# pashtari/factorizer

Measured on AMD Instinct MI355X. Metric: volumes/sec fwd+bwd, Swin Factorizer 128^3, higher is better.
Workload: dtype f32

## Files before the change

factorizer_amd/_native.py:

```python
from __future__ import annotations

import ctypes
import os
import threading

import torch

_HERE = os.path.dirname(os.path.abspath(__file__))
LIB_PATH = os.environ.get("FZ_LIB_PATH") or os.path.join(_HERE, "libfactorizer_hip.so")

FZ_OK = 0
FZ_E_UNSUPPORTED = -2
ABI_VERSION = 7
SOLVER_ID = {"mu": 0, "hals": 1, "cd": 2, "smu": 3}
STORE_F32, STORE_BF16 = 0, 1
PRODUCTS_DEFAULT, PRODUCTS_SPLIT_BF16, PRODUCTS_FP32_MFMA = 0, 1, 2
_products = threading.local()


def products() -> int:
    return getattr(_products, "value", PRODUCTS_DEFAULT)


class use_products:
# ... 56 lines not shown
    "fz_abi_version": ([], _i),
    "fz_set_tile_order": ([_i], _i),
    "fz_last_error_string": ([], _c.c_char_p),
    "fz_launch_count": ([], _i64),
    "fz_swm_fwd": ([_vp, _vp] + [_i] * 10 + [_c.POINTER(_i), _i, _i, _i, _vp], _i),
    "fz_swm_inv": ([_vp, _vp] + [_i] * 10 + [_c.POINTER(_i), _i, _vp, _i, _vp], _i),
    "fz_nmf_fwd": ([_vp] * 6 + [_i64] + [_i] * 5 + [_f, _i, _vp], _i),
    "fz_nmf_bwd": ([_vp] * 7 + [_i64] + [_i] * 6 + [_f, _i, _vp], _i),
    "fz_nmf_supported": ([_i] * 5, _i),
}


class NativeError(RuntimeError):
    pass


def declared_symbols():
    return sorted(_SIGS)


def lib():
    global _lib
    if _lib is not None:
        return _lib
    with _lock:
        if _lib is not None:
            return _lib
        if not os.path.exists(LIB_PATH):
            raise NativeError(
                f"{LIB_PATH} not found: build it with `python -m factorizer_amd.build` "
                "(hipcc --offload-arch=gfx950). Device tensors have no fallback path.")
        h = ctypes.CDLL(LIB_PATH)
        try:
            h.fz_abi_version.restype = ctypes.c_int
            abi = int(h.fz_abi_version())
        except AttributeError:
            abi = None
        if abi != ABI_VERSION:
            raise NativeError(f"{LIB_PATH} has ABI revision {abi}, this binding is written against {ABI_VERSION} "
                              "(include/factorizer_hip.h: FZ_ABI_VERSION): rebuild with `python -m factorizer_amd.build`")
        for name, (args, res) in _SIGS.items():
            fn = getattr(h, name)
            fn.argtypes = args
            fn.restype = res
        _lib = h
    return _lib


def launch_count() -> int:
    return int(lib().fz_launch_count())


def check(rc: int, what: str):
    if rc != FZ_OK:
        msg = lib().fz_last_error_string().decode()
        raise NativeError(f"{what} failed (code {rc}): {msg}")


def stream_ptr(t: torch.Tensor) -> int:
    return torch.cuda.current_stream(t.device).cuda_stream


def ptr(t):
    return None if t is None else t.data_ptr()


def shifts_array(shifts):
    flat = [int(v) for s in shifts for v in s]
    return (_i * len(flat))(*flat)


_fp = _c.POINTER(_c.c_float)


class GemmDesc(_c.Structure):
    _fields_ = [("x", _vp * 4), ("nsrc", _i), ("src_mode", _i), ("c0", _i), ("Cin", _i), ("Vin", _i64),
                ("Di", _i), ("Hi", _i), ("Wi", _i), ("w", _vp), ("w_t", _i), ("ldw", _i), ("M", _i), ("K", _i),
                ("bias", _vp), ("ln", _i), ("ln_g", _vp), ("ln_b", _vp), ("ln_eps", _f), ("stats_out", _vp),
                ("bact", _i), ("bmul", _vp), ("bmul_kind", _i), ("eact", _i), ("res", _vp), ("emul", _vp), ("emul_kind", _i), ("y", _vp),
                ("Ncol", _i64), ("Ho", _i), ("Wo", _i), ("B", _i), ("loader", _i), ("epilogue", _i), ("lnb_x", _vp), ("lnb_stats", _vp), ("lnb_g", _vp),
                ("lnb_gadd", _vp), ("lnb_part", _vp), ("act_dtype", _i), ("products", _i), ("tune", _i)]


class MlpDesc(_c.Structure):
    _fields_ = [("mode", _i), ("inp", _vp), ("w1", _vp), ("w2", _vp), ("b1", _vp), ("b2", _vp), ("ln_g", _vp),
                ("ln_b", _vp), ("ln_eps", _f), ("stats", _vp), ("z1", _vp), ("gz1", _vp), ("x1", _vp), ("out", _vp),
                ("part", _vp), ("B", _i), ("C", _i), ("H", _i), ("V", _i64), ("act_dtype", _i), ("wpart", _vp),
                ("gw1", _vp), ("gb1", _vp), ("gw2", _vp), ("gb2", _vp), ("gln", _vp), ("glp", _vp), ("products", _i),
                ("pre_in", _vp), ("pre_w", _vp), ("pre_b", _vp), ("pre_res", _vp), ("pre_out", _vp),
                ("post_w", _vp), ("post_b", _vp), ("post_out", _vp), ("post_m", _i)]


class MlpDropout(_c.Structure):
    _fields_ = [("m0", _vp), ("m1", _vp), ("m2", _vp), ("s0", _f), ("s1", _f), ("s2", _f)]


class BlockPrologue(_c.Structure):
    _fields_ = [("ln_g", _vp), ("ln_b", _vp), ("ln_eps", _f), ("w", _vp), ("t", _vp), ("stats", _vp)]


class GemmDwDesc(_c.Structure):
    _fields_ = [("g", _vp), ("q", _vp), ("w", _vp), ("ln", _i), ("stats", _vp), ("ln_g", _vp), ("ln_b", _vp), ("gadd", _vp),
                ("y", _vp), ("gln", _vp), ("wpart", _vp), ("gw", _vp), ("gb", _vp), ("B", _i), ("C", _i), ("V", _i64),
                ("act_dtype", _i), ("ldgw", _i), ("ldw", _i), ("drop_m", _vp), ("drop_s", _f)]


class WgradDesc(_c.Structure):
    _fields_ = [("p", _vp), ("M", _i), ("pmul", _vp), ("pmul_kind", _i), ("q", _vp * 4), ("nsrc", _i),
                ("src_mode", _i), ("c0", _i), ("Cin", _i), ("K", _i), ("Vq", _i64), ("D", _i), ("H", _i),
                ("W", _i), ("N", _i64), ("Ho", _i), ("Wo", _i), ("stats", _vp), ("qact", _i), ("ln_g", _vp),
                ("ln_b", _vp), ("gw", _vp), ("gbias", _vp), ("accumulate", _i), ("B", _i), ("loader", _i),
                ("act_dtype", _i), ("products", _i)]


class VolGeom(_c.Structure):
    _fields_ = [("nd", _i), ("size", _i * 3), ("start", _i * 3), ("end", _i * 3), ("pad", _i * 3), ("out", _i * 3)]


class RespaceGeom(_c.Structure):
    _fields_ = [("nd", _i), ("src_size", _i * 3), ("src_axis", _i * 3), ("flip", _i * 3), ("res_size", _i * 3), ("pad", _i * 3),
                ("out", _i * 3), ("orig_size", _i * 3), ("box_start", _i * 3), ("scale", _c.c_double * 3),
                ("inv_scale", _c.c_double * 3)]


_SIGS.update({
    "fz_gcorr_supported": ([_i] * 5, _i),
    "fz_gcorr": ([_vp] * 5 + [_i] * 11 + [_f, _vp], _i),
    "fz_gcorr_wgrad_workspace_bytes": ([_i] * 10, _i64),
    "fz_gcorr_wgrad": ([_vp] * 4 + [_i] * 11 + [_vp], _i),
    "fz_gcorr_act": ([_vp] * 5 + [_i] * 11 + [_f, _i, _vp], _i),
    "fz_gcorr_wgrad_act": ([_vp] * 4 + [_i] * 12 + [_vp], _i),
    "fz_gcorr_mu_bwd": ([_vp] * 8 + [_i] * 11 + [_f, _i, _vp], _i),
    "fz_gnmf_supported": ([_i, _i64, _i, _i, _i], _i),
    "fz_gnmf_workspace_bytes": ([_i64, _i, _i64, _i, _i, _i], _i64),
    "fz_gnmf_launches": ([_i, _i, _i], _i),
    "fz_gnmf_fwd": ([_vp] * 6 + [_i64, _i, _i64, _i, _i, _i, _f, _vp, _vp], _i),
    "fz_gnmf_bwd": ([_vp] * 7 + [_i64, _i, _i64, _i, _i, _i, _i, _f, _vp, _vp], _i),
    "fz_gnmfx_supported": ([_i, _i64, _i, _i, _i], _i),
    "fz_gnmfx_workspace_bytes": ([_i64, _i, _i64, _i, _i, _i], _i64),
    "fz_gnmfx_launches": ([_i, _i64, _i, _i, _i, _i], _i),
    "fz_gnmfx_fwd": ([_vp] * 6 + [_i64, _i, _i64, _i, _i, _i, _f, _vp, _vp], _i),
    "fz_gnmfx_bwd": ([_vp] * 7 + [_i64, _i, _i64, _i, _i, _i, _i, _f, _vp, _vp], _i),
    "fz_nmf_cf_supported": ([_i] * 11, _i),
    "fz_nmf_cf_fwd": ([_vp] * 4 + [_i] * 5 + [_c.POINTER(_i)] + [_i] * 5 + [_f, _i, _vp], _i),
    "fz_nmf_cf_bwd": ([_vp] * 5 + [_i] * 5 + [_c.POINTER(_i)] + [_i] * 7 + [_f, _i, _vp], _i),
    "fz_nmf_cf_factors_supported": ([_i] * 12 + [_c.POINTER(_i)], _i),
    "fz_nmf_cf_fwd_store_factors": ([_vp] * 5 + [_i] * 5 + [_c.POINTER(_i)] + [_i] * 3 + [_f, _i, _vp], _i),
    "fz_nmf_cf_fwd_from_factors": ([_vp] * 6 + [_i] * 5 + [_c.POINTER(_i)] * 2 + [_i] * 4 + [_f, _i, _vp], _i),
    "fz_nmf_cf_bwd_factors_supported": ([_i] * 14 + [_c.POINTER(_i)], _i),
    "fz_nmf_cf_bwd_store_factors": ([_vp] * 5 + [_i] * 5 + [_c.POINTER(_i)] + [_i] * 3 + [_f, _i, _vp], _i),
    "fz_nmf_cf_bwd_from_factors": ([_vp] * 6 + [_i] * 5 + [_c.POINTER(_i)] * 2 + [_i] * 3 + [_f, _i, _vp], _i),
    "fz_nmf_pcf_supported": ([_i] * 11, _i),
    "fz_nmf_pcf_fwd": ([_vp] * 4 + [_i] * 8 + [_c.POINTER(_i)] + [_i] * 5 + [_f, _i, _vp], _i),
    "fz_nmf_pcf_bwd": ([_vp] * 5 + [_i] * 8 + [_c.POINTER(_i)] + [_i] * 7 + [_f, _i, _vp], _i),
    "fz_nmf_pcf_bwd_prefers_separate": ([_i] * 4, _i),
    "fz_act_add": ([_vp, _vp, _i64, _i, _vp], _i),
    "fz_mlp_pre_supported": ([_i, _i, _i64, _i], _i),
    "fz_mlp_drop_supported": ([_i, _i, _i64, _i], _i),
    "fz_mlp_chain_drop": ([_c.POINTER(MlpDesc), _c.POINTER(MlpDropout), _vp], _i),
    "fz_conv3_prologue_supported": ([_i] * 4, _i),
    "fz_conv3_fwd2": ([_vp] * 4 + [_i] * 8 + [_c.POINTER(BlockPrologue), _vp], _i),
    "fz_upcat2": ([_vp, _vp, _vp, _i, _vp, _vp, _vp] + [_i] * 7 + [_c.POINTER(BlockPrologue), _vp], _i),
    "fz_gemm": ([_c.POINTER(GemmDesc), _vp], _i),
    "fz_gemm_plan": ([_c.POINTER(GemmDesc), _c.c_char_p, _i], _i),
    "fz_gemm_bx_enable": ([_i], _i),
    "fz_gemm_lnbwd_partials": ([_c.POINTER(GemmDesc)], _i64),
    "fz_reduce_rows": ([_vp, _i64, _i, _vp, _vp, _vp], _i),
    "fz_adamw_step": ([_vp, _vp, _vp, _vp, _i64, _f, _f, _f, _f, _f, _i, _f, _vp], _i),
    "fz_sw_gather": ([_vp, _vp] + [_i] * 10 + [_vp], _i),
    "fz_sw_accumulate": ([_vp] * 6 + [_f] + [_i] * 10 + [_vp], _i),
    "fz_sw_finalize": ([_vp, _vp, _i, _i64, _vp], _i),
    "fz_sw_gather2": ([_vp, _vp] + [_i] * 11 + [_vp], _i),
    "fz_sw_accumulate2": ([_vp] * 6 + [_f] + [_i] * 11 + [_vp], _i),
    "fz_sw_finalize2": ([_vp, _vp, _vp, _i, _i64, _i, _vp], _i),
    "fz_mlp_supported": ([_i, _i, _i64], _i),
    "fz_mlp_partials": ([_i, _i64], _i64),
    "fz_mlp_wgrad_rows": ([_i, _i64], _i),
    "fz_gemm_dw_rows": ([_i, _i64], _i),
    "fz_gemm_dw_workspace_bytes": ([_i, _i64], _i64),
    "fz_gemm_dw": ([_c.POINTER(GemmDwDesc), _vp], _i),
    "fz_mlp_wgrad_workspace_bytes": ([_i, _i64], _i64),
    "fz_mlp_chain": ([_c.POINTER(MlpDesc), _vp], _i),
    "fz_head_bwd_rows": ([], _i),
    "fz_head_bwd_workspace_bytes": ([], _i64),
    "fz_head_bwd": ([_vp, _vp, _vp, _vp, _vp, _i, _i, _i, _i64, _i, _vp], _i),
    "fz_head_fwd": ([_vp, _vp, _vp, _vp, _i, _i, _i, _i64, _i, _vp], _i),
    "fz_upcat_supported": ([_i] * 5, _i),
    "fz_upcat_compose": ([_vp, _vp, _i, _vp, _vp, _vp, _vp, _vp, _i, _i, _i, _vp], _i),
    "fz_upcat_wgrads": ([_vp, _vp, _vp, _i, _vp, _vp, _vp, _vp, _i, _vp, _i, _i, _i, _vp], _i),
    "fz_upcat": ([_vp, _vp, _vp, _i, _vp, _vp, _vp] + [_i] * 7 + [_vp], _i),
    "fz_upcat_bwd_supported": ([_i] * 6, _i),
    "fz_upcat_bwd_workspace_bytes": ([_i] * 4, _i64),
    "fz_upcat_bwd": ([_vp, _vp, _vp, _vp, _i, _vp, _vp, _vp, _vp, _vp, _i, _vp, _vp] + [_i] * 7 + [_vp], _i),
    "fz_wgrad": ([_c.POINTER(WgradDesc), _vp, _vp], _i),
    "fz_wgrad_group": ([_c.POINTER(_c.POINTER(WgradDesc)), _c.POINTER(_vp), _i, _vp], _i),
    "fz_wgrad_workspace_bytes": ([_c.POINTER(WgradDesc)], _i64),
    "fz_conv3_fwd": ([_vp] * 4 + [_i] * 8 + [_vp], _i),
    "fz_conv3_wgrad_chunks": ([_i] * 4, _i),
    "fz_conv3_wgrad_partials": ([_vp] * 4 + [_i] * 8 + [_vp], _i),
    "fz_chunk_reduce": ([_vp, _i, _i64, _vp, _i, _vp], _i),
    "fz_chunk_reduce_ld": ([_vp, _i, _i64, _i64, _vp, _i, _vp], _i),
    "fz_finish_defer": ([_i], _i),
    "fz_finish_pending": ([], _i),
    "fz_finish_flush": ([_vp], _i),
    "fz_finish_flush_all": ([_vp], _i),
    "fz_dice_bce_chunks": ([_i64], _i),
    "fz_dice_bce_sums": ([_vp, _vp, _vp, _i, _i64, _vp], _i),
    "fz_dice_bce_grad": ([_vp, _vp, _vp, _vp, _i, _i64, _f, _f, _vp, _vp], _i),
    "fz_dice_ce_sums": ([_vp, _vp, _vp, _i, _i, _i64, _vp], _i),
    "fz_dice_ce_grad": ([_vp, _vp, _vp, _vp, _i, _i, _i64, _f, _f, _vp, _vp], _i),
    "fz_dice_ce_finish": ([_vp, _i, _i, _i64, _f, _vp, _vp, _vp], _i),
    "fz_dice_bce_ds_sums": ([_vp, _vp, _vp, _i] + [_i] * 6 + [_i, _vp], _i),
    "fz_dice_bce_ds_grad": ([_vp, _vp, _vp, _vp, _i] + [_i] * 6 + [_i, _f, _f, _vp, _vp], _i),
    "fz_dice_ce_ds_sums": ([_vp, _vp, _vp, _i, _i] + [_i] * 6 + [_i, _vp], _i),
    "fz_dice_ce_ds_grad": ([_vp, _vp, _vp, _vp, _i, _i] + [_i] * 6 + [_i, _f, _f, _vp, _vp], _i),
    "fz_rowsum_chunks": ([_i64], _i),
    "fz_rowsum": ([_vp, _vp, _vp, _i, _i, _i64, _i, _vp], _i),
    "fz_ln_fwd": ([_vp] * 5 + [_i, _i, _i64, _f, _i, _vp], _i),
    "fz_ln_bwd": ([_vp] * 8 + [_i, _i, _i64, _i, _vp], _i),
    "fz_ln_bwd_workspace_bytes": ([_i], _i64),
    "fz_ln_bwd_workspace_bytes2": ([_i, _i, _i64], _i64),
    "fz_dropout_bits_words": ([_i, _i, _i64], _i64),
    "fz_dropout_keep_bits": ([_vp, _i, _i, _i, _i64, _f, _vp, _vp], _i),
    "fz_dropout_apply": ([_i, _vp, _f, _vp, _vp, _vp, _i, _i, _i64, _i, _vp], _i),
    "fz_seg_counts_chunks": ([_i64], _i),
    "fz_seg_counts_workspace_bytes": ([_i, _i64], _i64),
    "fz_seg_counts": ([_vp, _i, _vp, _i, _f, _vp, _vp, _vp, _i, _i64, _vp], _i),
    "fz_mask_edges": ([_vp, _vp, _vp, _i, _i, _i, _i, _i, _vp], _i),
    "fz_edge_min_dist2_splits": ([_i64, _i64], _i),
    "fz_edge_min_dist2_workspace_bytes": ([_i64, _i64], _i64),
    "fz_edge_min_dist2": ([_vp, _i64, _vp, _i64, _f, _f, _f, _vp, _vp, _vp], _i),
    "fz_aug_record_floats": ([], _i),
    "fz_aug_resample": ([_vp, _vp, _i, _i, _vp, _vp, _i, _vp, _vp, _vp] + [_i] * 6 + [_vp], _i),
    "fz_aug_smooth": ([_vp, _vp, _i, _i, _vp, _vp] + [_i] * 6 + [_vp], _i),
    "fz_aug_noise_field": ([_vp, _vp, _i, _i, _i64, _vp], _i),
    "fz_aug_source_words": ([], _i),
    "fz_aug_crop_resample": ([_vp, _vp, _i, _i, _vp, _i, _vp, _vp, _vp] + [_i] * 6 + [_vp], _i),
    "fz_vol_kind_ok": ([_i, _i], _i),
    "fz_vol_bbox": ([_vp, _i, _i, _i, _i, _i, _i, _vp, _vp], _i),
    "fz_vol_workspace_bytes": ([_i, _c.POINTER(VolGeom)], _i64),
    "fz_vol_stats": ([_vp, _i, _i, _c.POINTER(VolGeom), _i, _i, _vp, _vp], _i),
    "fz_vol_write": ([_vp, _i, _vp, _i, _i, _vp, _i, _i, _c.POINTER(_i), _c.POINTER(_i), _i, _vp, _c.POINTER(VolGeom), _i, _i,
# ... 16 lines not shown
```

factorizer_amd/csrc/gemm_dw.hip:

```cpp
#include "gemm_bx.h"
#include "gemm_shared.h"
#include "finish.h"

namespace fz {


template <typename AT>
struct DwArgsT {
  const AT* g;
  const AT* q;
  const float* w;
  int ldw;
  const float* stats;
  const float* ln_g;
  const AT* gadd;
  AT* y;
  float* wpart;
  int64_t V;
  int B;
};

template <bool LNB, typename AT, typename... DropX>
__global__ __launch_bounds__(256, 2) void gemm_dw_kernel(DwArgsT<AT> p, int ntiles, DropX... dx) {
  constexpr bool DROP = sizeof...(DropX) > 0;
  const DropArgs dr = drop_of(dx...);
  constexpr int NACC = 2;
  constexpr int kWave = 64 * kTS;
  constexpr bool BXB = sizeof(AT) == 2;
  extern __shared__ __attribute__((aligned(16))) float fz_lds_dw[];
  float* As = fz_lds_dw;
  float* tB = As + 1536;
  float* red = tB + 32;
  float* R = red + 256;
  const int lane = threadIdx.x & 63, wave = threadIdx.x >> 6;
  const int j = lane & 31, h = lane >> 5;
  const int l16 = lane & 15, k4 = lane >> 4;
  float* Gb = R + wave * kWave;
  float* Qb = Gb + 32 * kTS;
  const int tiles_per_sample = (int)((p.V + 128 * NACC - 1) / (128 * NACC));

  if constexpr (BXB) {
    if (threadIdx.x < 128) {
      const int l = threadIdx.x & 63, g = threadIdx.x >> 6;
      float a8[8];
#pragma unroll
      for (int e = 0; e < 8; ++e) a8[e] = p.w[(int64_t)(2 * (8 * g + e) + (l >> 5)) * p.ldw + (l & 31)];
      bx8 t3[3];
      bx_split<3>(a8, t3);
      bx8* dst = reinterpret_cast<bx8*>(As) + (g * 3) * 64 + l;
      dst[0] = t3[0]; dst[64] = t3[1]; dst[128] = t3[2];
    }
  } else {
  for (int idx = threadIdx.x; idx < 1024; idx += 256) {
    const int l = idx & 63, a = idx >> 6;
    As[idx] = p.w[(int64_t)(2 * a + (l >> 5)) * p.ldw + (l & 31)];
  }
  }
  if (LNB && threadIdx.x < 32) tB[threadIdx.x] = p.ln_g[threadIdx.x];

  f32x4 dW[2][2];
#pragma unroll
  for (int a = 0; a < 2; ++a)
#pragma unroll
    for (int b2 = 0; b2 < 2; ++b2)
#pragma unroll
      for (int v = 0; v < 4; ++v) dW[a][b2][v] = 0.f;
  f32x16 dWx;
#pragma unroll
  for (int r = 0; r < 16; ++r) dWx[r] = 0.f;
  float db[2] = {0.f, 0.f};
  float gln = 0.f;

  int tile = blockIdx.x;
  float bv[16][NACC];
  auto fetch_tile = [&](int t) {
    const int bt = t / tiles_per_sample;
    const int64_t ct = ((int64_t)(t % tiles_per_sample) * 4 + wave) * (32 * NACC) + NACC * j;
    const unsigned lo = (unsigned)h * (unsigned)p.V + (unsigned)(ct < p.V ? ct : 0);
    const AT* xb = p.g + (int64_t)bt * 32 * p.V;
#pragma unroll
    for (int s = 0; s < 16; ++s) vload<NACC>(xb + (int64_t)(2 * s) * p.V + lo, bv[s]);
  };
  fetch_tile(tile);
  __syncthreads();

  for (; tile < ntiles; tile += gridDim.x) {
    asm volatile("" ::: "memory");
    const int b = tile / tiles_per_sample;
    const int64_t col_off = ((int64_t)(tile % tiles_per_sample) * 4 + wave) * (32 * NACC) + NACC * j;
    const bool col_ok = col_off < p.V;
    const int64_t nc = col_ok ? col_off : 0;
    const unsigned lane_row = (unsigned)(4 * h) * (unsigned)p.V + (unsigned)nc;
    const unsigned lane_par = (unsigned)h * (unsigned)p.V + (unsigned)nc;
    const int64_t sample = (int64_t)b * 32 * p.V;
    if constexpr (DROP) {
#pragma unroll
      for (int s = 0; s < 16; ++s) {
        const uint32_t dk = drop_bits(dr, 0, b, 32, 2 * s + h, nc);
        bv[s][0] = drop_f(dr, 0, dk, 0, bv[s][0]);
        bv[s][1] = drop_f(dr, 0, dk, 1, bv[s][1]);
      }
    }

    float mu[NACC] = {0.f, 0.f}, rs[NACC] = {1.f, 1.f};
    if (LNB) {
      const float* sp = p.stats + (int64_t)b * 2 * p.V;
      vload<NACC>(sp + nc, mu);
      vload<NACC>(sp + p.V + nc, rs);
    }
#pragma unroll
    for (int hf = 0; hf < 2; ++hf) {
      float xv[8][NACC];
#pragma unroll
      for (int s8 = 0; s8 < 8; ++s8) vload<NACC>(p.q + sample + (int64_t)(2 * (hf * 8 + s8)) * p.V + lane_par, xv[s8]);
#pragma unroll
      for (int s8 = 0; s8 < 8; ++s8)
        *reinterpret_cast<float2*>(Qb + (2 * (hf * 8 + s8) + h) * kTS + 2 * j) =
            make_float2(col_ok ? (xv[s8][0] - mu[0]) * rs[0] : 0.f, col_ok ? (xv[s8][1] - mu[1]) * rs[1] : 0.f);
      __builtin_amdgcn_sched_barrier(0);
    }
#pragma unroll
    for (int s = 0; s < 16; ++s)
      *reinterpret_cast<float2*>(Gb + (2 * s + h) * kTS + 2 * j) = make_float2(col_ok ? bv[s][0] : 0.f, col_ok ? bv[s][1] : 0.f);

    f32x16 acc[NACC];
#pragma unroll
    for (int q = 0; q < NACC; ++q)
#pragma unroll
      for (int r = 0; r < 16; ++r) acc[q][r] = 0.f;
    if constexpr (BXB) {
#pragma unroll
      for (int g = 0; g < 2; ++g) {
        bx8 bop[NACC][1];
#pragma unroll
        for (int q = 0; q < NACC; ++q) {
          float x8[8];
#pragma unroll
          for (int e = 0; e < 8; ++e) x8[e] = bv[8 * g + e][q];
          bx_split<1>(x8, bop[q]);
        }
#pragma unroll
        for (int t = 2; t >= 0; --t) {
          const bx8 aw = reinterpret_cast<const bx8*>(As)[(g * 3 + t) * 64 + lane];
#pragma unroll
          for (int q = 0; q < NACC; ++q) acc[q] = __builtin_amdgcn_mfma_f32_32x32x16_bf16(aw, bop[q][0], acc[q], 0, 0, 0);
        }
      }
    } else {
#pragma unroll
    for (int s = 0; s < 16; ++s) {
      const float av = As[s * 64 + lane];
#pragma unroll
      for (int q = 0; q < NACC; ++q) acc[q] = __builtin_amdgcn_mfma_f32_32x32x2f32(av, bv[s][q], acc[q], 0, 0, 0);
    }
    }
    fetch_tile(tile + gridDim.x < ntiles ? tile + gridDim.x : tile);

    if constexpr (BXB) {
      const int rowo = (lane & 31) * kTS + 8 * (lane >> 5);
#pragma unroll
      for (int gk = 0; gk < 4; ++gk) {
        float g8[8], q8[8];
#pragma unroll
        for (int e2 = 0; e2 < 4; ++e2) {
          const float2 gv = *reinterpret_cast<const float2*>(Gb + rowo + 16 * gk + 2 * e2);
          const float2 qv = *reinterpret_cast<const float2*>(Qb + rowo + 16 * gk + 2 * e2);
          g8[2 * e2] = gv.x; g8[2 * e2 + 1] = gv.y;
          q8[2 * e2] = qv.x; q8[2 * e2 + 1] = qv.y;
        }
        bx8 ga[1];
        bx_split<1>(g8, ga);
        constexpr int NTQ = LNB ? 3 : 1;
        bx8 qb[NTQ];
        bx_split<NTQ>(q8, qb);
#pragma unroll
        for (int t = NTQ - 1; t >= 0; --t) dWx = __builtin_amdgcn_mfma_f32_32x32x16_bf16(ga[0], qb[t], dWx, 0, 0, 0);
        db[0] += ((g8[0] + g8[1]) + (g8[2] + g8[3])) + ((g8[4] + g8[5]) + (g8[6] + g8[7]));
        asm volatile("" : "+v"(db[0]));
        __builtin_amdgcn_sched_barrier(0);
      }
    } else
#pragma unroll
    for (int tc = 0; tc < 2; ++tc) {
      float a0[8], a1[8], b0[8], b1[8];
#pragma unroll
      for (int u = 0; u < 8; ++u) {
        const int t = tc * 8 + u;
        a0[u] = Gb[l16 * kTS + 4 * t + k4];
        a1[u] = Gb[(16 + l16) * kTS + 4 * t + k4];
        b0[u] = Qb[l16 * kTS + 4 * t + k4];
        b1[u] = Qb[(16 + l16) * kTS + 4 * t + k4];
      }
// ... 46 lines not shown
        }
#pragma unroll
        for (int i = 0; i < 8; ++i) {
          const int r = r8 * 8 + i;
          const int rbase = (r & 3) + 8 * (r >> 2);
          const int row = rbase + 4 * h;
          const float gc = tB[row];
          const float2 xh = *reinterpret_cast<const float2*>(Qb + row * kTS + 2 * j);
          float v[NACC];
          v[0] = rs[0] * (acc[0][r] * gc - m1[0] - xh.x * m2[0]) + ga[i][0];
          v[1] = rs[1] * (acc[1][r] * gc - m1[1] - xh.y * m2[1]) + ga[i][1];
          if (col_ok) vstore<NACC>(p.y + sample + (int64_t)rbase * p.V + lane_row, v);
          float sg = col_ok ? acc[0][r] * xh.x + acc[1][r] * xh.y : 0.f;
          float sb = col_ok ? acc[0][r] + acc[1][r] : 0.f;
          sg = half_sum32(sg);
          sb = half_sum32(sb);
          if ((lane & 31) == 31) {
            red[wave * 64 + row] = sg;
            red[wave * 64 + 32 + row] = sb;
          }
          __builtin_amdgcn_sched_barrier(0);
        }
      }
      __syncthreads();
      if (threadIdx.x < 64) {
        const int e = threadIdx.x;
        gln += (red[e] + red[64 + e]) + (red[128 + e] + red[192 + e]);
      }
      __syncthreads();
    }
  }

  float* row = p.wpart + (int64_t)blockIdx.x * kDwRow;
  __syncthreads();
  if constexpr (BXB) {
#pragma unroll
    for (int r = 0; r < 16; ++r) R[(wave * 16 + r) * 64 + lane] = dWx[r];
  } else {
#pragma unroll
  for (int a = 0; a < 2; ++a)
#pragma unroll
    for (int b2 = 0; b2 < 2; ++b2)
#pragma unroll
      for (int v = 0; v < 4; ++v) R[(wave * 16 + (a * 2 + b2) * 4 + v) * 64 + lane] = dW[a][b2][v];
  }
  __syncthreads();
  for (int e = threadIdx.x; e < 1024; e += 256) {
    const int idx = e >> 6, l = e & 63;
    const float t = (R[e] + R[1024 + e]) + (R[2048 + e] + R[3072 + e]);
    if constexpr (BXB) {
      row[((idx & 3) + 8 * (idx >> 2) + 4 * (l >> 5)) * 32 + (l & 31)] = t;
    } else {
      const int a = idx >> 3, b2 = (idx >> 2) & 1, v = idx & 3;
      row[(16 * a + 4 * (l >> 4) + v) * 32 + 16 * b2 + (l & 15)] = t;
    }
  }
  __syncthreads();
  R[(wave * 2 + 0) * 64 + lane] = db[0];
  R[(wave * 2 + 1) * 64 + lane] = db[1];
  __syncthreads();
  if (threadIdx.x < 32) {
    const int e = threadIdx.x, slot = e >> 4, i16 = e & 15;
    float t = 0.f;
    if constexpr (BXB) {
      for (int w = 0; w < 4; ++w) t += R[(w * 2) * 64 + e] + R[(w * 2) * 64 + 32 + e];
    } else {
      for (int w = 0; w < 4; ++w)
        for (int kk = 0; kk < 4; ++kk) t += R[(w * 2 + slot) * 64 + kk * 16 + i16];
    }
    row[1024 + e] = t;
  }
  if (threadIdx.x < 64) row[1024 + 32 + threadIdx.x] = gln;
}


}

using namespace fz;

static int knob_gemm_dw_wgs() { return knob_pos(FZ_KNOB("FZ_GEMM_DW_WGS"), 512); }

extern "C" int fz_gemm_dw_rows(int B, int64_t V);
template <typename AT>
static int gemm_dw_launch(const fz_gemm_dw_desc* d, fz_stream_t stream) {
  DwArgsT<AT> a;
  a.g = (const AT*)d->g; a.q = (const AT*)d->q; a.w = d->w; a.ldw = d->ldw > 0 ? d->ldw : 32; a.stats = d->stats; a.ln_g = d->ln_g; a.gadd = (const AT*)d->gadd;
  a.y = (AT*)d->y; a.wpart = (float*)d->wpart; a.V = d->V; a.B = d->B;
  const int ntiles = (int)fz_mlp_partials(d->B, d->V);
  const int rows = fz_gemm_dw_rows(d->B, d->V);
  constexpr int lds = (1536 + 32 + 256 + 4 * 64 * kTS) * (int)sizeof(float);
  hipStream_t st = (hipStream_t)stream;
  if (d->drop_m) {
    auto kern = gemm_dw_kernel<false, AT, DropArgs>;
    FZ_HIP_OK(hipFuncSetAttribute(reinterpret_cast<const void*>(kern), hipFuncAttributeMaxDynamicSharedMemorySize, lds));
    hipLaunchKernelGGL(kern, dim3((unsigned)rows), dim3(256), lds, st, a, ntiles, drop_args(d->drop_m, nullptr, nullptr, d->drop_s, 1.f, 1.f, d->V));
  } else if (d->ln) {
    auto kern = gemm_dw_kernel<true, AT>;
    FZ_HIP_OK(hipFuncSetAttribute(reinterpret_cast<const void*>(kern), hipFuncAttributeMaxDynamicSharedMemorySize, lds));
    hipLaunchKernelGGL(kern, dim3((unsigned)rows), dim3(256), lds, st, a, ntiles);
  } else {
    auto kern = gemm_dw_kernel<false, AT>;
    FZ_HIP_OK(hipFuncSetAttribute(reinterpret_cast<const void*>(kern), hipFuncAttributeMaxDynamicSharedMemorySize, lds));
    hipLaunchKernelGGL(kern, dim3((unsigned)rows), dim3(256), lds, st, a, ntiles);
  }
  FZ_LAUNCH_CHECK();
  FinishJob fj = finish_job(FK_DW, kDwRow / 16);
  fj.u.dw = FinDw{(const float*)d->wpart, d->ln ? d->ln_g : (const float*)nullptr, d->ln_b, d->gw, d->gb, d->ln ? d->gln : (float*)nullptr,
                  rows, d->ldgw > 0 ? d->ldgw : 32};
  return finish_run(&fj, 1, st);
}

extern "C" int fz_gemm_dw_rows(int B, int64_t V) {
  const int64_t nt = fz_mlp_partials(B, V);
  const int wgs = knob_gemm_dw_wgs();
  return (int)(nt < wgs ? nt : wgs);
}
extern "C" int64_t fz_gemm_dw_workspace_bytes(int B, int64_t V) {
  return (int64_t)fz_gemm_dw_rows(B, V) * kDwRow * (int64_t)sizeof(float);
}

extern "C" int fz_gemm_dw(const fz_gemm_dw_desc* d, fz_stream_t stream) {
  if (!d) return fail(FZ_E_ARG, "fz_gemm_dw: null descriptor");
  if (!d->g || !d->q || !d->w || !d->y || !d->wpart || !d->gw) return fail(FZ_E_ARG, "fz_gemm_dw: null pointer");
  if (d->ln && (!d->stats || !d->ln_g || !d->ln_b || !d->gln)) return fail(FZ_E_ARG, "fz_gemm_dw: the LayerNorm form needs stats, gamma, beta, gln");
  if (!d->ln && d->gadd) return fail(FZ_E_UNSUPPORTED, "fz_gemm_dw: gadd only with the LayerNorm backward");
  if (d->drop_m && d->ln) return fail(FZ_E_UNSUPPORTED, "fz_gemm_dw: dropout on g only without the LayerNorm backward");
  if (!drop_scale_ok(d->drop_m, d->drop_s)) return fail(FZ_E_ARG, "fz_gemm_dw: the dropout scale 1 / (1 - p) must be >= 1 and finite");
  if (d->C != 32) return fail(FZ_E_UNSUPPORTED, "fz_gemm_dw: needs C == 32");
  if (d->ldgw != 0 && d->ldgw < 32) return fail(FZ_E_ARG, "fz_gemm_dw: ldgw must be 0 (= 32) or >= 32");
  if (d->ldw != 0 && d->ldw < 32) return fail(FZ_E_ARG, "fz_gemm_dw: ldw must be 0 (= 32) or >= 32");
  if (d->B < 1 || d->V < 1 || d->V % 4 != 0 || d->V > ((int64_t)1 << 27)) return fail(FZ_E_UNSUPPORTED, "fz_gemm_dw: needs B >= 1, V % 4 == 0, V <= 2^27");
  if (d->act_dtype == FZ_STORE_F32) return gemm_dw_launch<float>(d, stream);
  if (d->act_dtype == FZ_STORE_BF16) return gemm_dw_launch<bf16>(d, stream);
  return fail(FZ_E_ARG, "fz_gemm_dw: act_dtype must be FZ_STORE_F32 or FZ_STORE_BF16");
}
```

factorizer_amd/csrc/mlp_chain.h:

```cpp
#pragma once
#include "gemm_bx.h"
#include "gemm_shared.h"

namespace fz {

template <typename AT>
struct ChainArgsT {
  const float* wB;
  int wB_t, ldwB;
  const float* biasB;
  AT* side;
  const AT* preA;
  const float* preW;
  const float* preB;
  const AT* preRes;
  AT* preOut;
  const float* postW;
  const float* postB;
  AT* postOut;
  int postM;
  int stagger;
};

__device__ __forceinline__ void chain_stagger(int stagger) {
  const int n = stagger * (int)(blockIdx.x >> 8);
  for (int i = 0; i < n; ++i) __builtin_amdgcn_s_sleep(127);
}

constexpr int chain64_lds_floats(bool p512, bool pre) {
  return 2 * (p512 ? 12288 : 8192) + (pre ? 6144 + 64 : 0) + 128 + 64 + (p512 ? 2 : 1) * 512;
}
constexpr int chain_wg_lds_floats(bool bx, bool wgb) {
  return 2 * (bx ? 3072 : 2048) + 32 + 256 + 4 * (wgb ? 3072 : 48 * kTS);
}

template <typename... KArgs, typename... Args>
static int launch_lds(void (*kern)(KArgs...), dim3 grid, dim3 block, int lds_floats, hipStream_t st, Args... args) {
  const int lds = lds_floats * (int)sizeof(float);
  FZ_HIP_OK(hipFuncSetAttribute(reinterpret_cast<const void*>(kern), hipFuncAttributeMaxDynamicSharedMemorySize, lds));
  hipLaunchKernelGGL(kern, grid, block, lds, st, args...);
  FZ_LAUNCH_CHECK();
  return FZ_OK;
}

static int knob_chain64_p512() { return knob_pos(FZ_KNOB("FZ_CHAIN64_P512"), 1) == 1; }
static int knob_chain_fwd_bx() { const auto& k = FZ_KNOB("FZ_CHAIN_FWD_BX"); return k.set ? k.val : 1; }
static int knob_mlp_wgs(int dflt) { return knob_pos(FZ_KNOB("FZ_MLP_WGS"), dflt); }

template <typename AT>
int chain32_launch(const fz_mlp_desc* d, const fz_mlp_dropout* drop, const GemmArgsT<AT>& a, const ChainArgsT<AT>& c, fz_stream_t stream);
template <typename AT>
int chain64_launch(const fz_mlp_desc* d, const GemmArgsT<AT>& a, const ChainArgsT<AT>& c, fz_stream_t stream);
template <typename AT>
int chain_wg_launch(const fz_mlp_desc* d, const GemmArgsT<AT>& a, const ChainArgsT<AT>& c, fz_stream_t stream);

}
```

factorizer_amd/csrc/mlp_chain.hip:

```cpp
#include "mlp_chain.h"

using namespace fz;

static int mlp_nacc() { return 2; }

extern "C" int64_t fz_mlp_partials(int B, int64_t V) {
  const int64_t tw = 128 * mlp_nacc();
  return ((V + tw - 1) / tw) * (int64_t)B;
}

extern "C" int fz_mlp_pre_supported(int C, int H, int64_t V, int products) {
  if (!(V > 0 && (V % 4) == 0 && V <= ((int64_t)1 << 27) && products_split(products))) return 0;
  if (C == 32 && H == 64) return knob_chain_fwd_bx() ? 1 : 0;
  if (C == 64 && H == 128) return (((V + 255) / 256) % 2 == 0 && knob_chain64_p512()) ? 1 : 0;
  return 0;
}

extern "C" int fz_mlp_supported(int C, int H, int64_t V) {
  const bool shape = (C == 32 && (H == 64 || H == 128)) || (C == 64 && H == 128);
  return (shape && V > 0 && (V % 4) == 0 && V <= ((int64_t)1 << 27)) ? 1 : 0;
}

extern "C" int fz_mlp_drop_supported(int C, int H, int64_t V, int products) {
  return (C == 32 && H == 64 && fz_mlp_supported(C, H, V) && fz_mlp_pre_supported(C, H, V, products) && products_split(products)
          && knob_chain_fwd_bx()) ? 1 : 0;
}

template <typename AT>
static void forward_args(const fz_mlp_desc* d, int ldw, int ldwB, GemmArgsT<AT>& a, ChainArgsT<AT>& c) {
  a.w = d->w1; a.w_t = 0; a.ldw = ldw;
  a.bias = d->b1; a.ln = 1; a.ln_g = d->ln_g; a.ln_b = d->ln_b; a.ln_eps = d->ln_eps; a.stats_out = d->stats;
  a.res = (const AT*)d->in; a.y = (AT*)d->out;
  c.wB = d->w2; c.wB_t = 0; c.ldwB = ldwB; c.biasB = d->b2; c.side = (AT*)d->z1;
  if (d->pre_in) {
    c.preA = (const AT*)d->pre_in; c.preW = d->pre_w; c.preB = d->pre_b; c.preRes = (const AT*)d->pre_res; c.preOut = (AT*)d->pre_out;
    if (d->C == 64) a.res = (const AT*)d->pre_out;
    else { c.postW = d->post_w; c.postB = d->post_b; c.postOut = (AT*)d->post_out; c.postM = d->post_m; }
  }
}
template <typename AT>
static void backward_args(const fz_mlp_desc* d, int ldw, int ldwB, AT* side, GemmArgsT<AT>& a, ChainArgsT<AT>& c) {
  a.w = d->w2; a.w_t = 1; a.ldw = ldw;
  a.emul = (const AT*)d->z1; a.y = (AT*)d->out;
  a.lnb_x = (const AT*)d->x1; a.lnb_stats = d->stats; a.lnb_g = d->ln_g; a.lnb_gadd = (const AT*)d->in; a.lnb_part = d->part;
  c.wB = d->w1; c.wB_t = 1; c.ldwB = ldwB; c.side = side;
}

static int mlp_check(const fz_mlp_desc* d, const fz_mlp_dropout* dd, bool drop) {
  if (!fz_mlp_supported(d->C, d->H, d->V)) return fail(FZ_E_UNSUPPORTED, "fz_mlp_chain: needs (C, H) in {(32, 64), (32, 128), (64, 128)}, V % 4 == 0");
  if (drop) {
    if (!fz_mlp_drop_supported(d->C, d->H, d->V, d->products) || d->mode != 0 || !d->pre_in)
      return fail(FZ_E_UNSUPPORTED, "fz_mlp_chain: dropout needs (C, H) = (32, 64), split-bf16 products, mode 0 with pre_in (fz_mlp_drop_supported)");
    if (!drop_scale_ok(dd->m0, dd->s0) || !drop_scale_ok(dd->m1, dd->s1) || !drop_scale_ok(dd->m2, dd->s2))
      return fail(FZ_E_ARG, "fz_mlp_chain: a dropout scale 1 / (1 - p) must be >= 1 and finite");
  }
  if (d->C == 64 && d->mode == 2) return fail(FZ_E_UNSUPPORTED, "fz_mlp_chain: the fused weight gradients need C == 32, H == 64");
  if (d->B < 0) return fail(FZ_E_SHAPE, "fz_mlp_chain: negative batch");
  const bool pre = d->pre_in != nullptr;
  if (pre && (d->mode != 0 || !d->pre_w || !d->pre_res || !d->pre_out))
    return fail(FZ_E_ARG, "fz_mlp_chain: pre_in needs mode 0, pre_w, pre_res, pre_out (see fz_mlp_pre_supported)");
  if (pre && !fz_mlp_pre_supported(d->C, d->H, d->V, d->products))
    return fail(FZ_E_UNSUPPORTED, "fz_mlp_chain: the fused out-projection runs on split-bf16 products only (fz_mlp_pre_supported)");
  if (d->post_out && (!pre || d->C != 32 || !d->post_w || d->post_m < 1 || d->post_m > 4))
    return fail(FZ_E_ARG, "fz_mlp_chain: post_out needs pre_in, C == 32, post_w and 1 <= post_m <= 4");
  if ((!d->in && !pre) || !d->w1 || !d->w2 || !d->out || !d->z1 || !d->stats)
    return fail(FZ_E_ARG, "fz_mlp_chain: null pointer");
  if (d->mode == 0 && (!d->ln_g || !d->ln_b)) return fail(FZ_E_ARG, "fz_mlp_chain: forward needs the LayerNorm affine");
  if (d->mode == 1 && (!d->gz1 || !d->x1 || !d->ln_g || !d->part)) return fail(FZ_E_ARG, "fz_mlp_chain: backward needs gz1, x1, gamma, part");
  if (d->mode == 2 && (!d->x1 || !d->ln_g || !d->ln_b || !d->gln || !d->wpart || !d->gw1 || !d->gb1 || !d->gw2 || !d->gb2))
    return fail(FZ_E_ARG, "fz_mlp_chain: backward with weight gradients needs x1, gamma, beta, gln, wpart, gw1, gb1, gw2, gb2");
  if (d->mode == 2 && d->H == 128 && !d->glp) return fail(FZ_E_ARG, "fz_mlp_chain: the fused weight gradients at H == 128 need the glp buffer");
  if (d->mode < 0 || d->mode > 2) return fail(FZ_E_ARG, "fz_mlp_chain: bad mode");
  return FZ_OK;
}

template <typename AT>
static int mlp_launch(const fz_mlp_desc* d, const fz_mlp_dropout* dd, fz_stream_t stream) {
  const bool drop = dd && (dd->m0 || dd->m1 || dd->m2);
  const int rc = mlp_check(d, dd, drop);
  if (rc != FZ_OK) return rc;
  if (d->B == 0) {
    if (d->mode == 2) {
      hipStream_t s0 = (hipStream_t)stream;
      FZ_HIP_OK(hipMemsetAsync(d->gw1, 0, sizeof(float) * d->H * 32, s0));
      FZ_HIP_OK(hipMemsetAsync(d->gw2, 0, sizeof(float) * d->H * 32, s0));
      FZ_HIP_OK(hipMemsetAsync(d->gb1, 0, sizeof(float) * d->H, s0));
      FZ_HIP_OK(hipMemsetAsync(d->gb2, 0, sizeof(float) * 32, s0));
      FZ_HIP_OK(hipMemsetAsync(d->gln, 0, sizeof(float) * 64, s0));
    }
    return FZ_OK;
  }
  GemmArgsT<AT> a = {};
  ChainArgsT<AT> c = {};
  a.x[0] = (const AT*)d->in; a.nsrc = 1; a.c0 = d->C; a.Cin = d->C; a.Vin = d->V; a.M = d->H; a.K = d->C; a.Ncol = d->V; a.B = d->B;
  if (d->mode == 0) forward_args(d, d->C, d->H, a, c);
  else backward_args(d, d->H, d->C, d->mode == 1 ? (AT*)d->gz1 : (AT*)nullptr, a, c);
  if (d->C == 64) return chain64_launch(d, a, c, stream);
  if (d->mode == 2) return chain_wg_launch(d, a, c, stream);
  return chain32_launch(d, drop ? dd : nullptr, a, c, stream);
}

extern "C" int fz_mlp_chain(const fz_mlp_desc* d, fz_stream_t stream) {
  if (!d) return fail(FZ_E_ARG, "fz_mlp_chain: null descriptor");
  if (d->act_dtype == FZ_STORE_F32) return mlp_launch<float>(d, nullptr, stream);
  if (d->act_dtype == FZ_STORE_BF16) return mlp_launch<bf16>(d, nullptr, stream);
  return fail(FZ_E_ARG, "fz_mlp_chain: act_dtype must be FZ_STORE_F32 or FZ_STORE_BF16");
}

extern "C" int fz_mlp_chain_drop(const fz_mlp_desc* d, const fz_mlp_dropout* drop, fz_stream_t stream) {
  if (!d || !drop) return fail(FZ_E_ARG, "fz_mlp_chain_drop: null descriptor");
  if (d->act_dtype == FZ_STORE_F32) return mlp_launch<float>(d, drop, stream);
  if (d->act_dtype == FZ_STORE_BF16) return mlp_launch<bf16>(d, drop, stream);
  return fail(FZ_E_ARG, "fz_mlp_chain_drop: act_dtype must be FZ_STORE_F32 or FZ_STORE_BF16");
}
```

factorizer_amd/csrc/mlp_chain32.hip:

```cpp
#include "mlp_chain.h"

namespace fz {

template <bool BWD, int NACC, int HB, typename AT = float, bool BX = false, bool PRE = false, typename... DropX>
__global__ __launch_bounds__(256, (NACC == 2 && HB == 2 && !BWD && !BX) ? 3 : 2) void gemm_chain_kernel(GemmArgsT<AT> p, ChainArgsT<AT> c, int ntiles, DropX... dx) {
  constexpr bool DROP = sizeof...(DropX) > 0;
  const DropArgs dr = drop_of(dx...);
  static_assert(!DROP || (PRE && !BWD && NACC == 2), "dropout: the forward chain with the out-projection in front");
  constexpr int NW = 4;
  constexpr int HID = 32 * HB, N1 = BX ? 1536 * HB : 16 * HB * 64;
  static_assert(!BX || (!BWD && NACC == 2), "the split-bf16 form is the forward chain");
  static_assert(!PRE || (BX && HB == 2), "the out-projection in front of the chain: split-bf16 forward, hidden 64");
  __shared__ __attribute__((aligned(16))) float As1[N1];
  __shared__ __attribute__((aligned(16))) float As2[N1];
  __shared__ __attribute__((aligned(16))) float As0[PRE ? 1536 : 4];
  __shared__ float tW[HID];
  __shared__ float tB[32];
  __shared__ float tB0[32];
  __shared__ float tP[PRE ? 4 * 32 + 4 : 1];
  __shared__ float red[256];
  __shared__ __attribute__((aligned(16))) float stash[NW][32][32 * NACC];
  const int lane = threadIdx.x & 63, wave = threadIdx.x >> 6;
  const int j = lane & 31, h = lane >> 5;
  const int tiles_per_sample = (int)((p.Ncol + 32 * NW * NACC - 1) / (32 * NW * NACC));
  chain_stagger(c.stagger);

  if constexpr (BX) {
    for (int it = threadIdx.x; it < (PRE ? 4 * HB + 2 : 4 * HB) * 64; it += 64 * NW) {
      float wv[8];
      const int l = it & 63;
      __bf16* dst;
      if (PRE && it >= 4 * HB * 64) {
        const int g = (it - 4 * HB * 64) >> 6;
#pragma unroll
        for (int e = 0; e < 8; ++e) wv[e] = c.preW[(l & 31) * 32 + 2 * (8 * g + e) + (l >> 5)];
        dst = reinterpret_cast<__bf16*>(As0) + (g * 3 * 64 + l) * 8;
      } else if (it < 2 * HB * 64) {
        const int rb = (it >> 6) % HB, g = it / (64 * HB);
#pragma unroll
        for (int e = 0; e < 8; ++e) {
          const int r = 8 * g + e;
          const int kk = PRE ? (r & 3) + 8 * (r >> 2) + 4 * (l >> 5) : 2 * r + (l >> 5);
          wv[e] = weight_at(p, rb * 32 + (l & 31), kk) * p.ln_g[kk];
        }
        dst = reinterpret_cast<__bf16*>(As1) + ((g * HB + rb) * 3 * 64 + l) * 8;
      } else {
        const int g = (it - 2 * HB * 64) >> 6;
#pragma unroll
        for (int e = 0; e < 8; ++e) {
          const int s2 = 8 * g + e, r = s2 & 15, rb = s2 >> 4;
          const int kk = rb * 32 + (r & 3) + 8 * (r >> 2) + 4 * (l >> 5), m = l & 31;
          wv[e] = c.wB_t ? c.wB[(int64_t)kk * c.ldwB + m] : c.wB[(int64_t)m * c.ldwB + kk];
        }
        dst = reinterpret_cast<__bf16*>(As2) + (g * 3 * 64 + l) * 8;
      }
      bx8 t3[3];
      bx_split<3>(wv, t3);
#pragma unroll
      for (int i = 0; i < 3; ++i) *reinterpret_cast<bx8*>(dst + i * 64 * 8) = t3[i];
    }
  } else
  for (int base = threadIdx.x; base < 2 * N1; base += 256 * 8) {
    float tmp[8];
#pragma unroll
    for (int uu = 0; uu < 8; ++uu) {
      const int idx = base + uu * 256;
      float wv;
      if (idx < N1) {
        const int l = idx & 63, rb = (idx >> 6) % HB, a = idx / (64 * HB);
        const int m = rb * 32 + (l & 31), k = 2 * a + (l >> 5);
        wv = weight_at(p, m, k);
        if (!BWD) wv *= p.ln_g[k];
      } else {
        const int i2 = idx - N1;
        const int l = i2 & 63, s2 = i2 >> 6;
        const int r = s2 & 15, rb = s2 >> 4;
        const int k = rb * 32 + (r & 3) + 8 * (r >> 2) + 4 * (l >> 5), m = l & 31;
        wv = c.wB_t ? c.wB[(int64_t)k * c.ldwB + m] : c.wB[(int64_t)m * c.ldwB + k];
      }
      tmp[uu] = wv;
    }
#pragma unroll
    for (int uu = 0; uu < 8; ++uu) {
      const int idx = base + uu * 256;
      if (idx < N1) As1[idx] = tmp[uu]; else As2[idx - N1] = tmp[uu];
    }
  }
  if (BWD) {
    if (threadIdx.x < 32) tB[threadIdx.x] = p.lnb_g[threadIdx.x];
  } else {
    for (int r = threadIdx.x; r < HID; r += blockDim.x) {
      float t = 0.f;
      for (int k = 0; k < 32; ++k) t += weight_at(p, r, k) * p.ln_b[k];
      tW[r] = t + (p.bias ? p.bias[r] : 0.f);
      if (r < 32) tB[r] = c.biasB ? c.biasB[r] : 0.f;
      if (PRE && r < 32) tB0[r] = c.preB ? c.preB[r] : 0.f;
    }
    if constexpr (PRE) {
      if (c.postOut != nullptr && threadIdx.x < 4 * 32 + 4) {
        const int i = threadIdx.x;
        if (i < 128) tP[i] = (i >> 5) < c.postM ? c.postW[i] : 0.f;
        else tP[i] = ((i - 128) < c.postM && c.postB) ? c.postB[i - 128] : 0.f;
      }
    }
  }

  int tile = blockIdx.x;
  float bv[16][NACC];
  float xr[PRE ? 16 : 1][NACC];
  auto fetch_tile = [&](int t) {
    const int bt = t / tiles_per_sample;
    const int64_t ct = ((int64_t)(t % tiles_per_sample) * NW + wave) * (32 * NACC) + NACC * j;
    const unsigned lo = (unsigned)h * (unsigned)p.Ncol + (unsigned)(ct < p.Ncol ? ct : 0);
    const AT* xb = (PRE ? c.preA : p.x[0]) + (int64_t)bt * 32 * p.Ncol;
#pragma unroll
    for (int s = 0; s < 16; ++s) vload<NACC>(xb + (int64_t)(2 * s) * p.Ncol + lo, bv[s]);
    if constexpr (PRE) {
      const unsigned lr = (unsigned)(4 * h) * (unsigned)p.Ncol + (unsigned)(ct < p.Ncol ? ct : 0);
      const AT* rb0 = c.preRes + (int64_t)bt * 32 * p.Ncol;
#pragma unroll
      for (int r = 0; r < 16; ++r) vload<NACC>(rb0 + (int64_t)((r & 3) + 8 * (r >> 2)) * p.Ncol + lr, xr[PRE ? r : 0]);
    }
  };
  fetch_tile(tile);
  __syncthreads();

  for (; tile < ntiles; tile += gridDim.x) {
    asm volatile("" ::: "memory");
    const int b = tile / tiles_per_sample;
    const int64_t col_off = ((int64_t)(tile % tiles_per_sample) * NW + wave) * (32 * NACC) + NACC * j;
    const bool col_ok = col_off < p.Ncol;
    const int64_t nc = col_ok ? col_off : 0;
    const unsigned lane_row = (unsigned)(4 * h) * (unsigned)p.Ncol + (unsigned)nc;
    if constexpr (PRE) {
      f32x16 acc0[NACC];
#pragma unroll
      for (int q = 0; q < NACC; ++q)
#pragma unroll
        for (int r = 0; r < 16; ++r) acc0[q][r] = 0.f;
#pragma unroll
      for (int g = 0; g < 2; ++g) {
        bx8 aop[3];
#pragma unroll
        for (int i = 0; i < 3; ++i)
          aop[i] = *reinterpret_cast<const bx8*>(reinterpret_cast<const __bf16*>(As0) + ((g * 3 + i) * 64 + lane) * 8);
#pragma unroll
        for (int q = 0; q < NACC; ++q) {
          float x8[8];
#pragma unroll
          for (int e = 0; e < 8; ++e) x8[e] = bv[8 * g + e][q];
          bx8 bop[3];
          bx_split<3>(x8, bop);
          bx_mfma<3, 3>(acc0[q], aop, bop);
        }
      }
#pragma unroll
      for (int r = 0; r < 16; ++r) {
        const int rbase = (r & 3) + 8 * (r >> 2);
        const int row = rbase + 4 * h;
        const float add = tB0[row];
        uint32_t dk = 0;
        if constexpr (DROP) dk = drop_bits(dr, 0, b, 32, row, nc);
#pragma unroll
        for (int q = 0; q < NACC; ++q) {
          float v;
          if constexpr (DROP) v = drop_f(dr, 0, dk, q, acc0[q][r] + add) + xr[PRE ? r : 0][q];
          else v = acc0[q][r] + add + xr[PRE ? r : 0][q];
          if constexpr (sizeof(AT) == 2) v = (float)(AT)v;
          bv[r][q] = v;
        }
        vstore<NACC>(&stash[wave][row][NACC * j], bv[r]);
        if (col_ok) vstore<NACC>(c.preOut + ((int64_t)b * 32 + rbase) * p.Ncol + lane_row, bv[r]);
      }
    } else {
#pragma unroll
    for (int s = 0; s < 16; ++s) vstore<NACC>(&stash[wave][2 * s + h][NACC * j], bv[s]);
    }

    if (!BWD) {
      float mu[NACC], rs[NACC];
#pragma unroll
      for (int e = 0; e < NACC; ++e) {
        float t = 0.f;
#pragma unroll
        for (int s = 0; s < 16; ++s) t += bv[s][e];
        t += __shfl_xor(t, 32, 64);
        mu[e] = t / 32.0f;
      }
#pragma unroll
      for (int e = 0; e < NACC; ++e) {
        float t = 0.f;
#pragma unroll
        for (int s = 0; s < 16; ++s) {
          const float d = bv[s][e] - mu[e];
          t += d * d;
        }
        t += __shfl_xor(t, 32, 64);
        rs[e] = 1.0f / sqrtf(t / 32.0f + p.ln_eps);
      }
#pragma unroll
      for (int s = 0; s < 16; ++s)
#pragma unroll
        for (int e = 0; e < NACC; ++e) bv[s][e] = (bv[s][e] - mu[e]) * rs[e];
      if (p.stats_out != nullptr && h == 0 && col_ok) {
        float* so = p.stats_out + (int64_t)b * 2 * p.Vin;
        vstore<NACC>(so + col_off, mu);
        vstore<NACC>(so + p.Vin + col_off, rs);
      }
    }

    f32x16 acc1[HB][NACC];
#pragma unroll
    for (int rb = 0; rb < HB; ++rb)
#pragma unroll
      for (int q = 0; q < NACC; ++q)
#pragma unroll
        for (int r = 0; r < 16; ++r) acc1[rb][q][r] = 0.f;
// ... 82 lines not shown
        __builtin_amdgcn_sched_barrier(0);
      }
    }

    f32x16 acc2[NACC];
#pragma unroll
    for (int q = 0; q < NACC; ++q)
#pragma unroll
      for (int r = 0; r < 16; ++r) acc2[q][r] = 0.f;
    if constexpr (BX) {
#pragma unroll
      for (int g = 0; g < 2 * HB; ++g) {
        bx8 aop[3];
#pragma unroll
        for (int i = 0; i < 3; ++i)
          aop[i] = *reinterpret_cast<const bx8*>(reinterpret_cast<const __bf16*>(As2) + ((g * 3 + i) * 64 + lane) * 8);
#pragma unroll
        for (int q = 0; q < NACC; ++q) {
          float x8[8];
#pragma unroll
          for (int e = 0; e < 8; ++e) x8[e] = acc1[g >> 1][q][8 * (g & 1) + e];
          bx8 bop[3];
          bx_split<3>(x8, bop);
          bx_mfma<3, 3>(acc2[q], aop, bop);
        }
      }
    } else {
#pragma unroll
    for (int rb = 0; rb < HB; ++rb)
#pragma unroll
      for (int r = 0; r < 16; ++r) {
        const float av = As2[(rb * 16 + r) * 64 + lane];
#pragma unroll
        for (int q = 0; q < NACC; ++q) acc2[q] = __builtin_amdgcn_mfma_f32_32x32x2f32(av, acc1[rb][q][r], acc2[q], 0, 0, 0);
      }
    }

    if (BWD) {
      lnbwd_block<NACC, true, true>(p, acc2, b, col_off, col_ok, lane, wave, red, tile, tB, &stash[wave][0][0]);
      __syncthreads();
    } else if (col_ok) {
      const bool post = PRE && c.postOut != nullptr;
      float pl[4][NACC] = {};
#pragma unroll
      for (int r = 0; r < 16; ++r) {
        const int rbase = (r & 3) + 8 * (r >> 2);
        const int row = rbase + 4 * h;
        const int64_t ob = ((int64_t)b * 32 + rbase) * p.Ncol;
        const float add = tB[row];
        float e[NACC], v[NACC];
        vload<NACC>(&stash[wave][row][NACC * j], e);
        if constexpr (DROP) {
          const uint32_t dk = drop_bits(dr, 2, b, 32, row, nc);
#pragma unroll
          for (int q = 0; q < NACC; ++q) v[q] = drop_f(dr, 2, dk, q, acc2[q][r] + add) + e[q];
        } else {
#pragma unroll
        for (int q = 0; q < NACC; ++q) v[q] = acc2[q][r] + add + e[q];
        }
        vstore<NACC>(p.y + ob + lane_row, v);
        if (PRE && post) {
#pragma unroll
          for (int q = 0; q < NACC; ++q) {
            const float vs = sizeof(AT) == 2 ? (float)(AT)v[q] : v[q];
#pragma unroll
            for (int o = 0; o < 4; ++o) pl[o][q] += tP[o * 32 + row] * vs;
          }
        }
      }
      if (PRE && post) {
#pragma unroll
        for (int o = 0; o < 4; ++o) {
          float v[NACC];
#pragma unroll
          for (int q = 0; q < NACC; ++q) v[q] = pl[o][q] + __shfl_xor(pl[o][q], 32, 64) + tP[128 + o];
          if (h == 0 && o < c.postM) vstore<NACC>(c.postOut + ((int64_t)b * c.postM + o) * p.Ncol + nc, v);
        }
      }
    }
  }
}

template <typename AT>
int chain32_launch(const fz_mlp_desc* d, const fz_mlp_dropout* drop, const GemmArgsT<AT>& a, const ChainArgsT<AT>& c, fz_stream_t stream) {
  hipStream_t st = (hipStream_t)stream;
  const int ntiles = (int)fz_mlp_partials(d->B, d->V);
  const bool bwd = d->mode != 0, pre = d->pre_in != nullptr;
  const bool bx = !bwd && d->H == 64 && products_split(d->products) && knob_chain_fwd_bx();
  const int wgs = knob_mlp_wgs(d->H == 128 || bx ? 512 : 768);
  const dim3 grid((unsigned)(ntiles < wgs ? ntiles : wgs)), block(256);
  if (bwd) {
    if (d->H == 128) hipLaunchKernelGGL((gemm_chain_kernel<true, 2, 4>), grid, block, 0, st, a, c, ntiles);
    else hipLaunchKernelGGL((gemm_chain_kernel<true, 2, 2>), grid, block, 0, st, a, c, ntiles);
  } else if (d->H == 128) hipLaunchKernelGGL((gemm_chain_kernel<false, 2, 4>), grid, block, 0, st, a, c, ntiles);
  else if (!bx) hipLaunchKernelGGL((gemm_chain_kernel<false, 2, 2>), grid, block, 0, st, a, c, ntiles);
  else if (!pre) hipLaunchKernelGGL((gemm_chain_kernel<false, 2, 2, AT, true>), grid, block, 0, st, a, c, ntiles);
  else if (!drop) hipLaunchKernelGGL((gemm_chain_kernel<false, 2, 2, AT, true, true>), grid, block, 0, st, a, c, ntiles);
  else
    hipLaunchKernelGGL((gemm_chain_kernel<false, 2, 2, AT, true, true, DropArgs>), grid, block, 0, st, a, c, ntiles,
                       drop_args(drop->m0, drop->m1, drop->m2, drop->s0, drop->s1, drop->s2, d->V));
  FZ_LAUNCH_CHECK();
  return FZ_OK;
}
template int chain32_launch<float>(const fz_mlp_desc*, const fz_mlp_dropout*, const GemmArgsT<float>&, const ChainArgsT<float>&, fz_stream_t);
template int chain32_launch<bf16>(const fz_mlp_desc*, const fz_mlp_dropout*, const GemmArgsT<bf16>&, const ChainArgsT<bf16>&, fz_stream_t);

}
```

factorizer_amd/csrc/nmf_cf.h:

```cpp
#pragma once
#include <cstdlib>

#include "fz_common.h"
#include "nmf_core.h"
#include "nmf_gram.h"

namespace fz {

struct CfGeom {
  int B, C, D, H, W;
  int h;
  int G0, G1, G2;
  int s0, s1, s2;
  int accumulate;
  int divisor;
  float gscale_div;
  int64_t plane;
  int ps0, ps1, ps2;
};

enum { CF_PLAIN = 0, CF_STORE_FACTORS = 1, CF_FROM_FACTORS = 2 };
constexpr int CFG_COFAC = 88;

struct CfWave {
  using F = float;
  int lane;
  __device__ __forceinline__ int col(int j) const {
    const int jp = j >> 2, e = j & 3;
    return (((jp * 4 + (lane >> 4)) * 8 + ((lane >> 1) & 7)) * 8) + (lane & 1) * 4 + e;
  }
  __device__ __forceinline__ float sum(float v) const { return wave_sum(v); }
  __device__ __forceinline__ void sum8(float (&v)[8]) const { wave_sum8(v, lane); }
  __device__ __forceinline__ void st_priv(float* base, int idx, float v) const { base[idx * 64 + lane] = v; }
  __device__ __forceinline__ float ld_priv(const float* base, int idx) const { return base[idx * 64 + lane]; }
  __device__ __forceinline__ void st_uni(float* base, int idx, float v) const {
    if (lane == 0) base[idx] = v;
  }
  __device__ __forceinline__ float ld_uni(const float* base, int idx) const { return base[idx]; }
  __device__ __forceinline__ float ld_uni_global(const float* p, int idx) const { return p[idx]; }
  __device__ __forceinline__ float ld_v0(const float* v0, int j, int r, int R) const { return v0[col(j) * R + r]; }
  __device__ __forceinline__ float keep_col(int, float v) const { return v; }
  __device__ __forceinline__ void fence() const { __builtin_amdgcn_fence(__ATOMIC_ACQ_REL, "wavefront"); }
  static constexpr bool kDistRows = true;
  __device__ __forceinline__ float sum8_dist(const float (&v)[8]) const { return wave_sum8_dist(v, lane); }
  __device__ __forceinline__ float grp_take(float d, int m) const {
    return __int_as_float(__builtin_amdgcn_readlane(__float_as_int(d), 8 * m));
  }
  __device__ __forceinline__ bool grp_below(int n) const { return (lane >> 3) < n; }
  __device__ __forceinline__ void st_grp(float* base, int i0, int stride, float d) const {
    if ((lane & 7) == 0) base[i0 + (lane >> 3) * stride] = d;
  }
  __device__ __forceinline__ float ld_grp_global(const float* p, int i0, int stride) const { return p[i0 + (lane >> 3) * stride]; }
  __device__ __forceinline__ float ld_grp(const float* base, int i0, int stride) const { return base[i0 + (lane >> 3) * stride]; }
  __device__ __forceinline__ float grp_sum(float d) const { return wave_group_sum(d); }
  __device__ __forceinline__ float mask_rows(float d, int mreal) const { return (lane >> 3) < mreal ? d : 0.f; }
  __device__ __forceinline__ float pick_call(int c, float tot, float mine) const { return (lane & 7) == c ? tot : mine; }
  __device__ __forceinline__ void k_unrotate(float* scratch, float mine, float (&Kd)[8]) const {
    const int g = lane >> 3;
    scratch[g * 8 + ((g + lane) & 7)] = mine;
    fence();
    const float4 a = *reinterpret_cast<const float4*>(scratch + g * 8), b = *reinterpret_cast<const float4*>(scratch + g * 8 + 4);
    Kd[0] = a.x; Kd[1] = a.y; Kd[2] = a.z; Kd[3] = a.w; Kd[4] = b.x; Kd[5] = b.y; Kd[6] = b.z; Kd[7] = b.w;
    fence();
  }
};

struct CfAddr {
  int64_t base;
  int64_t off[2];
  int64_t V;
};

__device__ __forceinline__ void cf_decode(const CfGeom& q, int64_t mat, int lane, CfAddr& a) {
  unsigned t = (unsigned)mat;
  const int g2 = (int)(t % (unsigned)q.G2); t /= (unsigned)q.G2;
  const int g1 = (int)(t % (unsigned)q.G1); t /= (unsigned)q.G1;
  const int g0 = (int)(t % (unsigned)q.G0); t /= (unsigned)q.G0;
  const int hh = (int)(t % (unsigned)q.h);
  const int b = (int)(t / (unsigned)q.h);
  const int p1 = (lane >> 1) & 7, half = lane & 1;
  int z1 = g1 * 8 + p1 - q.s1; if (z1 < 0) z1 += q.H;
  int z2 = g2 * 8 + half * 4 - q.s2; if (z2 < 0) z2 += q.W;
  a.V = q.plane;
  a.base = ((int64_t)b * q.C + (int64_t)hh * 8) * a.V;
#pragma unroll
// ... 117 lines not shown
  z0 = id.g0 * 8 + (row >> 3) - q.s0; if (z0 < 0) z0 += q.D;
  z1 = id.g1 * 8 + (row & 7) - q.s1; if (z1 < 0) z1 += q.H;
  z2 = id.gq * WPB * 8 + chunk * 4 - q.s2; if (z2 < 0) z2 += q.W;
}

template <int WPB>
__device__ __forceinline__ void cf_tile_decode(const CfGeom& q, const CfTileId& id, int tid, int64_t& base, int64_t& V,
                                               unsigned (&off)[2], int (&lidx)[2], unsigned (&off2)[2]) {
  using TL = CfTile<WPB>;
  V = q.plane;
  base = ((int64_t)id.b * q.C + (int64_t)id.hh * 8) * V;
#pragma unroll
  for (int k = 0; k < 2; ++k) {
    int row, chunk, z0, z1, z2;
    cf_chunk_voxel<WPB>(q, id, tid, k, row, chunk, z0, z1, z2);
    off[k] = (unsigned)((z0 * q.H + z1) * q.W + z2);
    int z2b = z2 + 2; if (z2b >= q.W) z2b -= q.W;
    off2[k] = (unsigned)((z0 * q.H + z1) * q.W + z2b);
    lidx[k] = TL::at(row, chunk);
  }
}

template <int WPB>
__device__ __forceinline__ unsigned cf_prev_patch(const CfGeom& q, const CfTileId& id, int tid, int k) {
  int row, chunk, z0, z1, z2;
  cf_chunk_voxel<WPB>(q, id, tid, k, row, chunk, z0, z1, z2);
  z0 += q.ps0; if (z0 >= q.D) z0 -= q.D;
  z1 += q.ps1; if (z1 >= q.H) z1 -= q.H;
  z2 += q.ps2; if (z2 >= q.W) z2 -= q.W;
  return (unsigned)(((z0 >> 3) * q.G1 + (z1 >> 3)) * q.G2 + (z2 >> 3));
}

template <typename AT>
__device__ __forceinline__ float4 cf_first_window(float u, const float4& v) {
  float p0 = u * v.x, p1 = u * v.y, p2 = u * v.z, p3 = u * v.w;
  asm("" : "+v"(p0), "+v"(p1), "+v"(p2), "+v"(p3));
  const f32v4 f = {0.0f + p0, 0.0f + p1, 0.0f + p2, 0.0f + p3};
  if constexpr (sizeof(AT) == 2) {
    const f32v4 r = __builtin_convertvector(__builtin_convertvector(f, bf16v4), f32v4);
    return make_float4(r[0], r[1], r[2], r[3]);
  }
  return make_float4(f[0], f[1], f[2], f[3]);
}

template <int WPB>
__device__ __forceinline__ int cf_owner_lidx(int lane, int wave, int jp) {
  return CfTile<WPB>::at((jp * 4 + (lane >> 4)) * 8 + ((lane >> 1) & 7), wave * 2 + (lane & 1));
}

template <int WPB>
__device__ __forceinline__ void cf_to_owner(float* S, const int (&lidx)[2], int own0, int own1, float (&x)[8][8]) {
  using TL = CfTile<WPB>;
#pragma unroll
  for (int s = 0; s < 4; ++s) {
#pragma unroll
    for (int c = 0; c < 2; ++c)
#pragma unroll
      for (int k = 0; k < 2; ++k)
        *reinterpret_cast<float4*>(S + c * 64 * TL::LW + lidx[k]) =
            make_float4(x[2 * s + c][k * 4 + 0], x[2 * s + c][k * 4 + 1], x[2 * s + c][k * 4 + 2], x[2 * s + c][k * 4 + 3]);
    __syncthreads();
#pragma unroll
    for (int c = 0; c < 2; ++c) {
      const float4 a0 = *reinterpret_cast<const float4*>(S + c * 64 * TL::LW + own0);
      const float4 a1 = *reinterpret_cast<const float4*>(S + c * 64 * TL::LW + own1);
      x[2 * s + c][0] = a0.x; x[2 * s + c][1] = a0.y; x[2 * s + c][2] = a0.z; x[2 * s + c][3] = a0.w;
      x[2 * s + c][4] = a1.x; x[2 * s + c][5] = a1.y; x[2 * s + c][6] = a1.z; x[2 * s + c][7] = a1.w;
    }
    __syncthreads();
  }
}


struct CfLaunch {
  CfGeom q;
  int64_t nmat;
  int xr;
  hipStream_t st;
};

template <typename AT>
int cf_fwd_launch(const AT* t, const float* u0, const float* v0, AT* out, float* vfac, float* ufac, const CfLaunch& a, int form,
                  int R, int T, int solver, float eps);
template <typename AT>
int cf_bwd_launch(const AT* t, const float* u0, const float* v0, const AT* ga, AT* gt, const CfLaunch& a, int relu_gate, int R,
                  int T, int G, int solver, float eps);
template <typename AT>
int cf_bwd_gram_launch(const AT* t, const float* v0, const AT* ga, AT* gt, const CfLaunch& a, int T, int G, float eps);
template <typename AT>
int cf_bwd_gram_factors_launch(const AT* t, const float* v0, const AT* ga, AT* gt, float* gcfac, float* cofac, const CfLaunch& a,
                               int form, int T, int G, float eps);

}
```

factorizer_amd/csrc/nmf_cf.hip:

```cpp
#include "nmf_cf.h"

namespace fz {

static void cf_norm_shift(const int* shift, int D, int H, int W, int (&s)[3]) {
  const int S[3] = {D, H, W};
  for (int i = 0; i < 3; ++i) { s[i] = shift[i] % S[i]; if (s[i] < 0) s[i] += S[i]; }
}

static int cf_geom(CfGeom& q, int B, int C, int D, int H, int W, const int* shift, const int* prev_shift, int accumulate,
                   int divisor) {
  if (B < 0 || C < 8 || (C % 8) || D < 8 || H < 8 || W < 8 || (D % 8) || (H % 8) || (W % 8))
    return fail(FZ_E_SHAPE, "fz_nmf_cf: needs C % 8 == 0 and spatial dims multiples of 8");
  if (!shift) return fail(FZ_E_ARG, "fz_nmf_cf: shift is null");
  if ((int64_t)D * H * W >= ((int64_t)1 << 30)) return fail(FZ_E_UNSUPPORTED, "fz_nmf_cf: 2^30 or more voxels per channel plane");
  q.B = B; q.C = C; q.D = D; q.H = H; q.W = W; q.h = C / 8; q.G0 = D / 8; q.G1 = H / 8; q.G2 = W / 8;
  int s[3], ps[3] = {0, 0, 0};
  cf_norm_shift(shift, D, H, W, s);
  if (s[2] % 2) return fail(FZ_E_UNSUPPORTED, "fz_nmf_cf: W-axis shift must be even");
  if (prev_shift) cf_norm_shift(prev_shift, D, H, W, ps);
  q.s0 = s[0]; q.s1 = s[1]; q.s2 = s[2];
  q.ps0 = ps[0]; q.ps1 = ps[1]; q.ps2 = ps[2];
  q.accumulate = accumulate; q.divisor = divisor; q.gscale_div = 1.0f;
  q.plane = (int64_t)D * H * W;
#ifdef FZ_PROBE_PLANE_PAD
// ... 41 lines not shown
    using AT = decltype(at);
    CfLaunch a;
    const int rc = cf_prepare(a, B, C, D, H, W, shift, nullptr, accumulate, divisor, stream, [&](const CfGeom&) {
      if (!t || !u0 || !v0 || !out) return fail(FZ_E_ARG, "fz_nmf_cf_fwd: null pointer");
      if (R < 1 || R > 2) return fail(FZ_E_UNSUPPORTED, "fz_nmf_cf_fwd: rank 1..2");
      if (solver < FZ_SOLVER_MU || solver > FZ_SOLVER_SMU) return fail(FZ_E_ARG, "fz_nmf_cf_fwd: bad solver");
      return (int)FZ_OK;
    });
    if (rc != FZ_OK || a.nmat == 0) return rc;
    return cf_fwd_launch<AT>((const AT*)t, u0, v0, (AT*)out, nullptr, nullptr, a, CF_PLAIN, R, T, solver, eps);
  });
}

extern "C" int fz_nmf_cf_bwd(const void* t, const float* u0, const float* v0, const void* ga, void* gt, int B,
                             int C, int D, int H, int W, const int* shift, int accumulate, int nshift,
                             int relu_gate, int R, int T, int Tgrad, int solver, float eps, int act_dtype,
                             fz_stream_t stream) {
  return cf_with_dtype(act_dtype, "fz_nmf_cf_bwd: bad act_dtype", [&](auto at) {
    using AT = decltype(at);
    CfLaunch a;
    const int rc = cf_prepare(a, B, C, D, H, W, shift, nullptr, accumulate, 1, stream, [&](const CfGeom&) {
      if (!t || !u0 || !v0 || !ga || !gt) return fail(FZ_E_ARG, "fz_nmf_cf_bwd: null pointer");
      if (R < 1 || R > 2) return fail(FZ_E_UNSUPPORTED, "fz_nmf_cf_bwd: rank 1..2");
      if (solver < FZ_SOLVER_MU || solver > FZ_SOLVER_SMU) return fail(FZ_E_ARG, "fz_nmf_cf_bwd: bad solver");
      return (int)FZ_OK;
    });
    if (rc != FZ_OK || a.nmat == 0) return rc;
    a.q.gscale_div = (float)(nshift > 1 ? nshift : 1);
    const int G = Tgrad < 0 ? 0 : (Tgrad > T ? T : Tgrad);
    return cf_bwd_launch<AT>((const AT*)t, u0, v0, (const AT*)ga, (AT*)gt, a, relu_gate, R, T, G, solver, eps);
  });
}

extern "C" int fz_nmf_cf_factors_supported(int C, int D, int H, int W, int d, int pd, int ph, int pw, int R, int T, int Tgrad,
                                           int nshift, const int* shifts) {
  if (!fz_nmf_cf_supported(C, D, H, W, d, pd, ph, pw, R, T, Tgrad)) return 0;
  if (R != 1 || nshift != 2 || !shifts || (W % 64)) return 0;
  for (int w = 0; w < 2; ++w) {
    int s[3];
    cf_norm_shift(shifts + 3 * w, D, H, W, s);
    if (s[2] % 4) return 0;
  }
  return 1;
}

static int cf_fwd_factors(const void* t, const float* u0, const float* v0, void* out, float* vfac, float* ufac, int B, int C,
                          int D, int H, int W, const int* shift, const int* prev_shift, int form, int divisor, int R, int T,
                          int solver, float eps, int act_dtype, fz_stream_t stream, const char* null_msg, const char* dtype_msg) {
  return cf_with_dtype(act_dtype, dtype_msg, [&](auto at) {
    using AT = decltype(at);
    CfLaunch a;
    const int rc = cf_prepare(a, B, C, D, H, W, shift, prev_shift, form == CF_FROM_FACTORS, divisor, stream, [&](const CfGeom& q) {
      if (!t || !u0 || !v0 || !vfac || !ufac || (form == CF_FROM_FACTORS && (!out || !prev_shift))) return fail(FZ_E_ARG, null_msg);
      if (R != 1) return fail(FZ_E_UNSUPPORTED, "fz_nmf_cf_fwd factor forms: rank 1 only");
      if (W % 64) return fail(FZ_E_UNSUPPORTED, "fz_nmf_cf_fwd factor forms: W must be a multiple of 64");
      if (solver < FZ_SOLVER_MU || solver > FZ_SOLVER_SMU) return fail(FZ_E_ARG, "fz_nmf_cf_fwd factor forms: bad solver");
      if (divisor < 1) return fail(FZ_E_ARG, "fz_nmf_cf_fwd factor forms: divisor < 1");
      if ((q.s2 % 4) || (q.ps2 % 4)) return fail(FZ_E_UNSUPPORTED, "fz_nmf_cf_fwd factor forms: W-axis shift must be a multiple of 4");
      return (int)FZ_OK;
    });
    if (rc != FZ_OK || a.nmat == 0) return rc;
    return cf_fwd_launch<AT>((const AT*)t, u0, v0, (AT*)out, vfac, ufac, a, form, R, T, solver, eps);
  });
}

extern "C" int fz_nmf_cf_fwd_store_factors(const void* t, const float* u0, const float* v0, float* vfac, float* ufac, int B,
                                           int C, int D, int H, int W, const int* shift, int R, int T, int solver, float eps,
                                           int act_dtype, fz_stream_t stream) {
  return cf_fwd_factors(t, u0, v0, nullptr, vfac, ufac, B, C, D, H, W, shift, nullptr, CF_STORE_FACTORS, 1, R, T, solver, eps,
                        act_dtype, stream, "fz_nmf_cf_fwd_store_factors: null pointer (t, u0, v0, vfac or ufac)",
                        "fz_nmf_cf_fwd_store_factors: bad act_dtype");
}

extern "C" int fz_nmf_cf_fwd_from_factors(const void* t, const float* u0, const float* v0, const float* vfac,
                                          const float* ufac, void* out, int B, int C, int D, int H, int W, const int* shift,
                                          const int* prev_shift, int divisor, int R, int T, int solver, float eps, int act_dtype,
                                          fz_stream_t stream) {
  return cf_fwd_factors(t, u0, v0, out, const_cast<float*>(vfac), const_cast<float*>(ufac), B, C, D, H, W, shift, prev_shift,
                        CF_FROM_FACTORS, divisor, R, T, solver, eps, act_dtype, stream,
                        "fz_nmf_cf_fwd_from_factors: null pointer (t, u0, v0, vfac, ufac, out or prev_shift)",
                        "fz_nmf_cf_fwd_from_factors: bad act_dtype");
}

extern "C" int fz_nmf_cf_bwd_factors_supported(int C, int D, int H, int W, int d, int pd, int ph, int pw, int R, int T, int Tgrad,
                                               int solver, int relu_gate, int nshift, const int* shifts) {
  if (FZ_KNOB("FZ_CF_BWD_FACTORS").set && FZ_KNOB("FZ_CF_BWD_FACTORS").val == 0) return 0;
  if (!fz_nmf_cf_factors_supported(C, D, H, W, d, pd, ph, pw, R, T, Tgrad, nshift, shifts)) return 0;
  if (solver != FZ_SOLVER_HALS || !relu_gate) return 0;
  if (T < 1 || Tgrad < T) return 0;
  if ((C / 8) * (int64_t)(D / 8) * (H / 8) * (W / 8) >= ((int64_t)1 << 31)) return 0;
  const int lds = (CfTile<4>::STAGE_FLOATS + 4 * gram_hist_floats(T - 1) + 4 * 8 * CFG_COFAC) * (int)sizeof(float);
  return lds <= 64 * 1024 ? 1 : 0;
}

static int cf_bwd_factors(const void* t, const float* v0, const void* ga, void* gt, float* gcfac, float* cofac, int B, int C,
                          int D, int H, int W, const int* shift, const int* prev_shift, int form, int nshift, int T, int Tgrad,
                          float eps, int act_dtype, fz_stream_t stream, const char* null_msg, const char* dtype_msg) {
  return cf_with_dtype(act_dtype, dtype_msg, [&](auto at) {
    using AT = decltype(at);
    CfLaunch a;
    int rc = cf_prepare(a, B, C, D, H, W, shift, prev_shift, form == CF_FROM_FACTORS, 1, stream, [&](const CfGeom& q) {
      if (!t || !v0 || !ga || !gcfac || !cofac || (form == CF_FROM_FACTORS && (!gt || !prev_shift))) return fail(FZ_E_ARG, null_msg);
      if (W % 64) return fail(FZ_E_UNSUPPORTED, "fz_nmf_cf_bwd factor forms: W must be a multiple of 64");
      if (nshift != 2) return fail(FZ_E_UNSUPPORTED, "fz_nmf_cf_bwd factor forms: exactly two windows");
      if (T < 1 || Tgrad < T) return fail(FZ_E_UNSUPPORTED, "fz_nmf_cf_bwd factor forms: every iteration graded (1 <= T <= Tgrad)");
      if ((q.s2 % 4) || (q.ps2 % 4)) return fail(FZ_E_UNSUPPORTED, "fz_nmf_cf_bwd factor forms: W-axis shift must be a multiple of 4");
      return (int)FZ_OK;
    });
    if (rc != FZ_OK || a.nmat == 0) return rc;
    a.q.gscale_div = (float)nshift;
    rc = cf_bwd_gram_factors_launch<AT>((const AT*)t, v0, (const AT*)ga, (AT*)gt, gcfac, cofac, a, form, T, T, eps);
    if (rc == FZ_E_UNSUPPORTED) return fail(rc, "fz_nmf_cf_bwd factor forms: history exceeds the LDS budget");
    return rc;
  });
}

extern "C" int fz_nmf_cf_bwd_store_factors(const void* t, const float* v0, const void* ga, float* gcfac, float* cofac, int B,
                                           int C, int D, int H, int W, const int* shift, int nshift, int T, int Tgrad,
                                           float eps, int act_dtype, fz_stream_t stream) {
  return cf_bwd_factors(t, v0, ga, nullptr, gcfac, cofac, B, C, D, H, W, shift, nullptr, CF_STORE_FACTORS, nshift, T, Tgrad, eps,
                        act_dtype, stream, "fz_nmf_cf_bwd_store_factors: null pointer (t, v0, ga, gcfac or cofac)",
                        "fz_nmf_cf_bwd_store_factors: bad act_dtype");
}

extern "C" int fz_nmf_cf_bwd_from_factors(const void* t, const float* v0, const void* ga, const float* gcfac,
                                          const float* cofac, void* gt, int B, int C, int D, int H, int W, const int* shift,
                                          const int* prev_shift, int nshift, int T, int Tgrad, float eps, int act_dtype,
                                          fz_stream_t stream) {
  return cf_bwd_factors(t, v0, ga, gt, const_cast<float*>(gcfac), const_cast<float*>(cofac), B, C, D, H, W, shift, prev_shift,
                        CF_FROM_FACTORS, nshift, T, Tgrad, eps, act_dtype, stream,
                        "fz_nmf_cf_bwd_from_factors: null pointer (t, v0, ga, gcfac, cofac, gt or prev_shift)",
                        "fz_nmf_cf_bwd_from_factors: bad act_dtype");
}
```

factorizer_amd/csrc/nmf_cf_fwd.hip:

```cpp
#include "nmf_cf.h"

namespace fz {

template <int R, int SOLVER, typename AT>
__global__ __launch_bounds__(1024) void nmf_cf_fwd_kernel(const AT* __restrict__ t, const float* __restrict__ u0,
                                                          const float* __restrict__ v0, AT* __restrict__ out,
                                                          CfGeom q, int64_t nmat, int T, float eps, int xcd_remap) {
  const int lane = threadIdx.x & 63;
  const int64_t mat = cf_logical_block(xcd_remap) * (blockDim.x >> 6) + (threadIdx.x >> 6);
  if (mat >= nmat) return;
  CfWave w{lane};
  CfAddr a;
  cf_decode(q, mat, lane, a);
  float x[8][8], u[8][R], v[8][R];
  cf_load(t, a, x);
  nmf_forward_wave<8, 8, R, SOLVER>(w, u0, v0, x, u, v, 8, T, eps);
  const float dv = (float)q.divisor;
  const bool dv_pow2 = cf_pow2(dv);
#pragma unroll
  for (int dd = 0; dd < 8; ++dd)
#pragma unroll
    for (int jp = 0; jp < 2; ++jp) {
      AT* p = out + a.base + dd * a.V + a.off[jp];
      float4 o;
// ... 74 lines not shown
#pragma unroll
    for (int dd = 0; dd < 8; ++dd)
#pragma unroll
      for (int k = 0; k < 2; ++k) old[dd][k] = cf_ld4<HALF>(out + base + dd * V, off[k], off2[k]);
  }
#pragma unroll
  for (int s = 0; s < 4; ++s) {
#pragma unroll
    for (int c = 0; c < 2; ++c) {
      *reinterpret_cast<float4*>(S + c * 64 * TL::LW + own0) =
          make_float4(x[2 * s + c][0], x[2 * s + c][1], x[2 * s + c][2], x[2 * s + c][3]);
      *reinterpret_cast<float4*>(S + c * 64 * TL::LW + own1) =
          make_float4(x[2 * s + c][4], x[2 * s + c][5], x[2 * s + c][6], x[2 * s + c][7]);
    }
    __syncthreads();
#pragma unroll
    for (int c = 0; c < 2; ++c)
#pragma unroll
      for (int k = 0; k < 2; ++k) {
        const float4 z = *reinterpret_cast<const float4*>(S + c * 64 * TL::LW + lidx[k]);
        float4 o;
        if constexpr (FORM == CF_FROM_FACTORS) {
          o = cf_first_window<AT>(pu[k][2 * s + c], pv[k]);
          o.x += z.x; o.y += z.y; o.z += z.z; o.w += z.w;
        } else if (q.accumulate) {
          o = old[2 * s + c][k];
          o.x += z.x; o.y += z.y; o.z += z.z; o.w += z.w;
        } else {
          o = make_float4(0.0f + z.x, 0.0f + z.y, 0.0f + z.z, 0.0f + z.w);
        }
        if (q.divisor > 1) o = cf_divide4(o, dv, dv_pow2);
        cf_st4<HALF>(out + base + (2 * s + c) * V, off[k], off2[k], o);
      }
    __syncthreads();
  }
}

template <int R, int SOLVER, int WPB, bool HALF, typename AT, int FORM>
__global__ __launch_bounds__(WPB * 64, (WPB == 8 || R >= 2) ? 2 : 4) void nmf_cf_fwd_tile_kernel(const AT* __restrict__ t,
                                                                   const float* __restrict__ u0,
                                                                   const float* __restrict__ v0,
                                                                   AT* __restrict__ out, float* vfac, float* ufac,
                                                                   CfGeom q, int T, float eps, int xcd_remap) {
  extern __shared__ __attribute__((aligned(16))) float fz_lds_tile[];
  cf_fwd_tile_body<R, SOLVER, WPB, HALF, AT, FORM>(t, u0, v0, out, vfac, ufac, q, cf_tile_id<WPB>(q, cf_logical_block(xcd_remap)), T, eps,
                                                   fz_lds_tile);
}

template <typename AT>
int cf_fwd_launch(const AT* t, const float* u0, const float* v0, AT* out, float* vfac, float* ufac, const CfLaunch& a, int form,
                  int R, int T, int solver, float eps) {
  const CfGeom& q = a.q;
  const int tile = FZ_KNOB("FZ_CF_TILE").set ? FZ_KNOB("FZ_CF_TILE").val : 1;
  const bool half = (q.s2 % 4) != 0;
  const int twpb = (q.G2 % 8) == 0 ? 8 : ((q.G2 % 4) == 0 ? 4 : 1);
#define FZ_CF_TILE(RR, WW, HH, FF, SS)                                                                                  \
  hipLaunchKernelGGL((nmf_cf_fwd_tile_kernel<RR, SS, WW, HH, AT, FF>), dim3((unsigned)(a.nmat / WW)), dim3(64 * WW),    \
                     CfTile<WW>::STAGE_FLOATS * (int)sizeof(float), a.st, t, u0, v0, out, vfac, ufac, q, T, eps, a.xr)
#define FZ_CF_TILE_W(RR, SS)                                                                                            \
  do {                                                                                                                  \
    if (half) { if (twpb == 8) FZ_CF_TILE(RR, 8, true, CF_PLAIN, SS); else if (twpb == 4) FZ_CF_TILE(RR, 4, true, CF_PLAIN, SS); else FZ_CF_TILE(RR, 1, true, CF_PLAIN, SS); } \
    else FZ_CF_TILE(RR, 8, false, CF_PLAIN, SS);                                                                        \
  } while (0)
  if (form == CF_STORE_FACTORS) {
    FZ_SOLVER_CASES(FZ_CF_TILE, 1, 8, false, CF_STORE_FACTORS);
  } else if (form == CF_FROM_FACTORS) {
    FZ_SOLVER_CASES(FZ_CF_TILE, 1, 8, false, CF_FROM_FACTORS);
  } else if (half || (tile && (q.G2 % 8) == 0)) {
    if (R == 1) { FZ_SOLVER_CASES(FZ_CF_TILE_W, 1); }
    else { FZ_SOLVER_CASES(FZ_CF_TILE_W, 2); }
  } else {
    const int wpb = q.G2 < 16 ? q.G2 : 16;
    dim3 grid((unsigned)((a.nmat + wpb - 1) / wpb)), block(64 * wpb);
#define FZ_CF_FWD(RR, SS) hipLaunchKernelGGL((nmf_cf_fwd_kernel<RR, SS, AT>), grid, block, 0, a.st, t, u0, v0, out, q, a.nmat, T, eps, a.xr)
    if (R == 1) { FZ_SOLVER_CASES(FZ_CF_FWD, 1); }
    else { FZ_SOLVER_CASES(FZ_CF_FWD, 2); }
  }
  FZ_LAUNCH_CHECK();
  return FZ_OK;
}
template int cf_fwd_launch<float>(const float*, const float*, const float*, float*, float*, float*, const CfLaunch&, int, int, int, int, float);
template int cf_fwd_launch<bf16>(const bf16*, const float*, const float*, bf16*, float*, float*, const CfLaunch&, int, int, int, int, float);

}
```

factorizer_amd/functional.py:

```python
from __future__ import annotations

import ctypes
import math
import os

import torch

from . import _native as N


def _dev_guard(t: torch.Tensor):
    return torch.cuda.device(t.device)


class KernelTimer:

    def __init__(self, only=None):
        self.records = []
        self.only = None if only is None else set(only)

    def launch(self, name, nbytes, fn, cols=0, flops=0):
        if self.only is not None and name not in self.only:
            return fn()
        s = torch.cuda.Event(enable_timing=True)
# ... 279 lines not shown
    return gx


class GNMFFn(torch.autograd.Function):

    @staticmethod
    def forward(ctx, x, u0, v0, T, G, solver, eps, fam):
        x, u0, v0 = x.contiguous(), u0.contiguous(), v0.contiguous()
        y, _, _ = _gnmf_fwd_raw(x, u0, v0, T, solver, eps, fam=fam)
        ctx.save_for_backward(x, u0, v0)
        ctx.cfg = (T, G, solver, eps, fam)
        return y

    @staticmethod
    def backward(ctx, gy):
        x, u0, v0 = ctx.saved_tensors
        T, G, solver, eps, fam = ctx.cfg
        if G <= 0:
            return (torch.zeros_like(x), *[None] * 7)
        return (_gnmf_bwd_raw(x, u0, v0, gy.contiguous(), None, None, T, G, solver, eps, fam), *[None] * 7)


class GNMFDecomposeFn(torch.autograd.Function):
    @staticmethod
    def forward(ctx, x, u0, v0, T, G, solver, eps, fam):
        x, u0, v0 = x.contiguous(), u0.contiguous(), v0.contiguous()
        _, u, v = _gnmf_fwd_raw(x, u0, v0, T, solver, eps, want_uv=True, fam=fam)
        ctx.save_for_backward(x, u0, v0)
        ctx.cfg = (T, G, solver, eps, fam)
        return u, v

    @staticmethod
    def backward(ctx, gu, gv):
        x, u0, v0 = ctx.saved_tensors
        T, G, solver, eps, fam = ctx.cfg
        if G <= 0:
            return (torch.zeros_like(x), *[None] * 7)
        gx = _gnmf_bwd_raw(x, u0, v0, None, gu.contiguous(), gv.contiguous(), T, G, solver, eps, fam)
        return (gx, *[None] * 7)


def gnmf(x, u0, v0, T, G, solver, eps=1e-16):
    return GNMFFn.apply(x, u0, v0, T, G, solver, eps, "gnmf")


def gnmf_decompose(x, u0, v0, T, G, solver, eps=1e-16):
    return GNMFDecomposeFn.apply(x, u0, v0, T, G, solver, eps, "gnmf")


def gnmfx(x, u0, v0, T, G, solver, eps=1e-16):
    return GNMFFn.apply(x, u0, v0, T, G, solver, eps, "gnmfx")


def gnmfx_decompose(x, u0, v0, T, G, solver, eps=1e-16):
    return GNMFDecomposeFn.apply(x, u0, v0, T, G, solver, eps, "gnmfx")


def nmf_cf_supported(geo: Geometry, R, T, G) -> bool:
    if len(geo.spatial) != 3 or any(s[2] % 2 for s in geo.shifts):
        return False
    return bool(N.lib().fz_nmf_cf_supported(geo.C, *geo.spatial, geo.d, *geo.patch, int(R), int(T), int(G)))


def nmf_cf_factors_supported(geo: Geometry, R, T, G) -> bool:
    if len(geo.spatial) != 3:
        return False
    k = (int(R), int(T), int(G))
    ok = geo._factors_ok.get(k)
    if ok is None:
        ok = geo._factors_ok[k] = bool(N.lib().fz_nmf_cf_factors_supported(geo.C, *geo.spatial, geo.d, *geo.patch, *k,
                                                                          geo.nshift, geo._carr))
    return ok


def nmf_cf_bwd_factors_supported(geo: Geometry, R, T, G, solver, relu_gate) -> bool:
    if len(geo.spatial) != 3:
        return False
    k = ("bwd", int(R), int(T), int(G), solver, bool(relu_gate))
    ok = geo._factors_ok.get(k)
    if ok is None:
        ok = geo._factors_ok[k] = bool(N.lib().fz_nmf_cf_bwd_factors_supported(
            geo.C, *geo.spatial, geo.d, *geo.patch, *k[1:4], N.SOLVER_ID[solver], int(k[5]), geo.nshift, geo._carr))
    return ok


def nmf_pcf_supported(geo: Geometry, R, T, G) -> bool:
    if os.environ.get("FZ_NMF_PCF", "1") == "0":
        return False
    return bool(N.lib().fz_nmf_pcf_supported(geo.C, *geo.s3, geo.d, *geo.p3, int(R), int(T), int(G)))


def nmf_core_supported(geo: Geometry, R, T, G) -> bool:
    return nmf_cf_supported(geo, R, T, G) or nmf_pcf_supported(geo, R, T, G)


def _core_launches(t, geo: Geometry, ad):
    lib, cols, tail = N.lib(), t.numel() // geo.C, (ad, N.stream_ptr(t))

    def launch(name, key, nbytes, *args):
        fn = getattr(lib, name)
        N.check(_timed(key, nbytes, cols=cols, fn=lambda: fn(*args, *tail)), name)

    return launch, f"{geo.C}x" + "x".join(str(v) for v in geo.spatial), [(N._i * 3)(*s) for s in geo.shifts3]


class FactCoreFn(torch.autograd.Function):

    @staticmethod
    def forward(ctx, t, u0, v0, geo, T, G, solver, eps, relu_gate):
        t = t.contiguous()
        u0, v0 = u0.contiguous(), v0.contiguous()
        B = t.shape[0]
        out = torch.empty_like(t)
        R = u0.shape[1]
        nt = t.element_size() * t.numel()
        hot = nmf_cf_supported(geo, R, T, G)
        launch, sp, shifts = _core_launches(t, geo, N.act_dtype(t))
        key = ("nmf_cf_fwd_" if hot else "nmf_pcf_fwd_") + sp
        lead = (t.data_ptr(), u0.data_ptr(), v0.data_ptr())
        dims = (B, geo.C, *geo.spatial) if hot else (B, geo.C, *geo.s3, *geo.p3)
        cfg = (R, T, N.SOLVER_ID[solver], eps)
        with _dev_guard(t):
            if hot and nmf_cf_factors_supported(geo, R, T, G):
                vfac = torch.empty((B, geo.h, *geo.spatial), device=t.device, dtype=torch.float32)
                ufac = torch.empty((B * geo.h * geo.G, 8), device=t.device, dtype=torch.float32)
                fac = (vfac.data_ptr(), ufac.data_ptr())
                nf = 4 * (t.numel() // 8)
                N.set_tile_order(0)
                launch("fz_nmf_cf_fwd_store_factors", key, nt + nf, *lead, *fac, *dims, shifts[0], *cfg)
                N.set_tile_order(1)
                launch("fz_nmf_cf_fwd_from_factors", key, 2 * nt + nf, *lead, *fac, out.data_ptr(), *dims, shifts[1], shifts[0], 2,
                       *cfg)
            else:
                name = "fz_nmf_cf_fwd" if hot else "fz_nmf_pcf_fwd"
                for w, arr in enumerate(shifts):
                    N.set_tile_order(w & 1)
                    launch(name, key, (3 if w else 2) * nt, *lead, out.data_ptr(), *dims, arr, int(w > 0),
                           geo.nshift if w == geo.nshift - 1 else 1, *cfg)
            N.set_tile_order(0)
        ctx.save_for_backward(t, u0, v0)
        ctx.cfg = (geo, T, G, solver, eps, relu_gate)
        return out

    @staticmethod
    def backward(ctx, ga):
        t, u0, v0 = ctx.saved_tensors
        geo, T, G, solver, eps, relu_gate = ctx.cfg
        if G <= 0:
            return (torch.zeros_like(t),) + (None,) * 8
        ga = ga.contiguous()
        if ga.dtype != t.dtype:
            ga = ga.to(t.dtype)
        gt = torch.empty_like(t)
        B = t.shape[0]
        R = u0.shape[1]
        nt = t.element_size() * t.numel()
        ad = N.act_dtype(t)
        hot = nmf_cf_supported(geo, R, T, G)
        launch, sp, shifts = _core_launches(t, geo, ad)
        key = ("nmf_cf_bwd_" if hot else "nmf_pcf_bwd_") + sp
        dims = (B, geo.C, *geo.spatial) if hot else (B, geo.C, *geo.s3, *geo.p3)
        with _dev_guard(t):
            if hot and nmf_cf_bwd_factors_supported(geo, R, T, G, solver, relu_gate):
                gcfac = torch.empty((B, geo.h, *geo.spatial), device=t.device, dtype=torch.float32)
                cofac = torch.empty((B * geo.h * geo.G, 88), device=t.device, dtype=torch.float32)
                lead = (t.data_ptr(), v0.data_ptr(), ga.data_ptr(), gcfac.data_ptr(), cofac.data_ptr())
# ... 487 lines not shown
```

factorizer_amd/pointwise.py:

```python
from __future__ import annotations

import collections
import ctypes
import functools
import os
import threading as _threading
import weakref

import torch
import torch.nn.functional as F

from . import _native as N
from . import gradbuf as _GB
from . import functional as Fn

ACT = {"none": 0, "relu": 1, "gelu": 2}
LOAD_PLAIN, LOAD_S2D, LOAD_K3, LOAD_S2D_2D, LOAD_K3_2D = 0, 1, 2, 3, 4
EPI_PLAIN, EPI_D2S, EPI_LNBWD, EPI_D2S_2D = 0, 1, 2, 3
QL_S2D_2D, QL_K3_2D = LOAD_S2D_2D, LOAD_K3_2D
_D2S_FINE = {EPI_D2S: 8, EPI_D2S_2D: 4}


_p = N.ptr

# ... 64 lines not shown
    d.act_dtype = N.act_dtype(p)
    nb = N.lib().fz_wgrad_workspace_bytes(ctypes.byref(d))
    if nb < 0:
        raise N.NativeError("fz_wgrad_workspace_bytes failed")
    ws = torch.empty(max(nb // 4, 1), dtype=torch.float32, device=p.device)
    nbytes = p.element_size() * (p.numel() + sum(t.numel() for t in qs))
    return d, ws, f"{name}_{M}x{K}", nbytes, B * max(Vq, Ncols), 2 * B * Ncols * M * K


def _wgrad(p, qs, gw, **kw):
    d, ws, key, nbytes, cols, flops = _wgrad_desc(p, qs, gw, **kw)
    with torch.cuda.device(p.device), _finish_scope(ws, gw, kw.get("gbias")):
        rc = Fn._timed(key, nbytes, lambda: N.lib().fz_wgrad(ctypes.byref(d), ws.data_ptr(), N.stream_ptr(p)),
                       cols=cols, flops=flops)
    N.check(rc, "fz_wgrad")
    return gw


_WGRAD_GROUP = os.environ.get("FZ_WGRAD_GROUP", "1") != "0"


def _wgrad_group(problems, name):
    plans = [_wgrad_desc(p, qs, gw, **kw) for p, qs, gw, kw in problems]
    n = len(plans)
    descs = (ctypes.POINTER(N.WgradDesc) * n)(*[ctypes.pointer(pl[0]) for pl in plans])
    wss = (ctypes.c_void_p * n)(*[pl[1].data_ptr() for pl in plans])
    t0 = problems[0][0]
    held = [pl[1] for pl in plans] + [pr[2] for pr in problems] + [pr[3].get("gbias") for pr in problems]
    with torch.cuda.device(t0.device), _finish_scope(*held):
        rc = Fn._timed(name, sum(pl[3] for pl in plans),
                       lambda: N.lib().fz_wgrad_group(descs, wss, n, N.stream_ptr(t0)),
                       cols=max(pl[4] for pl in plans), flops=sum(pl[5] for pl in plans))
    N.check(rc, "fz_wgrad_group")


def _ln_backward(gl, x, stats, ln_w, gadd=None):
    B, C = x.shape[:2]
    V = _vox(x)
    gx = torch.empty_like(x)
    gpar = torch.empty(2 * C, dtype=torch.float32, device=x.device)
    ws = torch.empty(max(N.lib().fz_ln_bwd_workspace_bytes2(B, C, V) // 4, 1), dtype=torch.float32, device=x.device)
    with torch.cuda.device(x.device), _finish_scope(ws, gpar):
        rc = Fn._timed(f"ln_bwd_{C}", 3 * x.element_size() * x.numel(), lambda: N.lib().fz_ln_bwd(
            gl.data_ptr(), x.data_ptr(), stats.data_ptr(), ln_w.data_ptr(), _p(gadd), gx.data_ptr(), _p(gpar), _p(ws),
            B, C, V, N.act_dtype(x), N.stream_ptr(x)), cols=B * V)
    N.check(rc, "fz_ln_bwd")
    return gx, gpar[:C], gpar[C:]


def _reduce_affine_rows(part, rows, C, like):
    gpar = torch.empty(2 * C, dtype=torch.float32, device=like.device)
    tmp = torch.empty((64, 2 * C), dtype=torch.float32, device=like.device)
    with _finish_scope(part, gpar, tmp):
        rc = N.lib().fz_reduce_rows(part.data_ptr(), rows, 2 * C, gpar.data_ptr(), tmp.data_ptr(), N.stream_ptr(like))
    N.check(rc, "fz_reduce_rows")
    return gpar[:C], gpar[C:]


def _dgrad_lnbwd(gz, w2, x, stats, ln_w, gadd):
    B, C = x.shape[:2]
    V = _vox(x)
    Mz = gz.shape[1]
    fused64 = C == 64 and Mz == 64 and gadd is not None and V % 4 == 0 and os.environ.get("FZ_LNBWD64", "1") != "0"
    if not fused64 and (C != 32 or Mz > 64 or Mz % 2):
        gl = torch.empty_like(x)
        _gemm([gz], w2, gl, B=B, Cin=Mz, Vin=V, M=C, K=Mz, Ncol=V, w_t=True, ldw=C, name="linear_dgrad")
        return _ln_backward(gl, x, stats, ln_w, gadd=gadd)
    gx = torch.empty_like(x)
    d, *timed = _gemm_desc([gz], w2, gx, B=B, Cin=Mz, Vin=V, M=C, K=Mz, Ncol=V, w_t=True, ldw=C, epilogue=EPI_LNBWD,
                           lnb=(x, stats, ln_w, gadd), name="dgrad_lnbwd")
    rows = N.lib().fz_gemm_lnbwd_partials(ctypes.byref(d))
    part = torch.empty((rows, 2 * C), dtype=torch.float32, device=x.device)
    d.lnb_part = part.data_ptr()
    with torch.cuda.device(x.device):
        _gemm_launch(gz, d, *timed)
        ggamma, gbeta = _reduce_affine_rows(part, rows, C, x)
    return gx, ggamma, gbeta


def _dw_fused_ok(C, V):
    return C == 32 and V % 4 == 0 and V <= (1 << 27) and os.environ.get("FZ_DW_FUSED", "1") != "0"


def _gemm_dw(g, w2, q, ln=None, stats=None, gadd=None, want_bias=False, name="dgrad_wgrad", gw_out=None, gb_out=None, drop=None):
    B, C = q.shape[:2]
    V = _vox(q)
    dev = q.device
    y = torch.empty_like(q)
    gw = _GB.out_like(w2, (C, C), torch.float32) if gw_out is None else gw_out
    gb = (gb_out if gb_out is not None else torch.empty(C, dtype=torch.float32, device=dev)) if want_bias else None
    wpart = torch.empty(N.lib().fz_gemm_dw_workspace_bytes(B, V) // 4, dtype=torch.float32, device=dev)
    d = N.GemmDwDesc()
    d.g, d.q, d.w, d.y = g.data_ptr(), q.data_ptr(), w2.data_ptr(), y.data_ptr()
    d.wpart, d.gw, d.gb = wpart.data_ptr(), gw.data_ptr(), _p(gb)
    d.B, d.C, d.V, d.act_dtype = B, C, V, N.act_dtype(q)
    d.ldgw = gw.stride(0)
    d.ldw = w2.stride(0)
    if drop is not None:
        d.drop_m, d.drop_s = drop[0].data_ptr(), _drop_scale(drop[1])
    gpar = None
    if ln is not None:
        gpar = torch.empty(64, dtype=torch.float32, device=dev)
        d.ln, d.stats, d.ln_g, d.ln_b, d.gadd, d.gln = 1, stats.data_ptr(), ln[0].data_ptr(), ln[1].data_ptr(), _p(gadd), gpar.data_ptr()
    nbytes = q.element_size() * (3 * q.numel() + (gadd.numel() if gadd is not None else 0))
    with torch.cuda.device(dev), _finish_scope(wpart, gw, gb, gpar):
        rc = Fn._timed(f"{name}_{C}", nbytes, lambda: N.lib().fz_gemm_dw(ctypes.byref(d), N.stream_ptr(q)),
                       cols=B * V, flops=4 * B * V * C * C)
        N.check(rc, "fz_gemm_dw")
    if ln is not None:
        return y, gw, gb, gpar[:32], gpar[32:]
    return y, gw, gb, None, None


def _drop_scale(p):
    return 1.0 / (1.0 - float(ctypes.c_float(p).value))


def _mlp_dropout(drop):
    bits, ps = drop
    dd = N.MlpDropout()
    for s in range(3):
        if bits[s] is not None:
            setattr(dd, f"m{s}", bits[s].data_ptr())
            setattr(dd, f"s{s}", _drop_scale(ps[s]))
    return dd


def _mlp_drop_ok(C, Hd, V):
    return (_outproj_mlp_ok(C, Hd, V)
            and bool(N.lib().fz_mlp_drop_supported(C, Hd, V, N.products())))


def _mlp_chain_ok(C, Hd, V):
    return os.environ.get("FZ_MLP_CHAIN", "1") != "0" and bool(N.lib().fz_mlp_supported(C, Hd, V))


def _mlp_desc(mode, like, w12, w22, *, B, C, Hd, V, inp=None, b1=None, b2=None, ln_w=None, ln_b=None, eps=0.0, stats=None, z1=None,
              x1=None, out=None):
    d = N.MlpDesc()
    d.products = N.products()
    d.mode, d.inp, d.w1, d.w2, d.b1, d.b2 = mode, _p(inp), w12.data_ptr(), w22.data_ptr(), _p(b1), _p(b2)
    d.ln_g, d.ln_b, d.ln_eps = _p(ln_w), _p(ln_b), float(eps)
    d.stats, d.z1, d.x1, d.out = _p(stats), _p(z1), _p(x1), _p(out)
    d.B, d.C, d.H, d.V = B, C, Hd, V
    d.act_dtype = N.act_dtype(like)
    return d


def _mlp_chain_fwd(timed, like, ln_w, ln_b, eps, w12, b1, w22, b2, inp=None, pre=None, head=None, drop=None):
    B, C = like.shape[:2]
    V = _vox(like)
    Hd = w12.shape[0]
    new = lambda ch: torch.empty((B, ch, *like.shape[2:]), dtype=like.dtype, device=like.device)
    z1, st, x2 = new(Hd), _ln_stats(B, V, like.device), torch.empty_like(like)
    d = _mlp_desc(0, like, w12, w22, B=B, C=C, Hd=Hd, V=V, inp=inp, b1=b1, b2=b2, ln_w=ln_w, ln_b=ln_b, eps=eps, stats=st, z1=z1, out=x2)
    x1 = logits = None
    if pre is not None:
        a, wout2, bout, x = pre
        x1 = torch.empty_like(like)
        d.pre_in, d.pre_w, d.pre_b, d.pre_res, d.pre_out = a.data_ptr(), wout2.data_ptr(), _p(bout), x.data_ptr(), x1.data_ptr()
    if head is not None:
        hw, hb = head
        logits = new(hw.shape[0])
        d.post_w, d.post_b, d.post_out, d.post_m = hw.data_ptr(), _p(hb), logits.data_ptr(), hw.shape[0]
    dd = _mlp_dropout(drop) if drop is not None else None
    key, nbytes, flops = timed
    with torch.cuda.device(like.device):
        rc = Fn._timed(key, nbytes,
                       lambda: (N.lib().fz_mlp_chain(ctypes.byref(d), N.stream_ptr(like)) if dd is None
                                else N.lib().fz_mlp_chain_drop(ctypes.byref(d), ctypes.byref(dd), N.stream_ptr(like))),
                       cols=B * V, flops=flops)
    N.check(rc, "fz_mlp_chain")
    return x1, x2, z1, st, logits


def _mlp_fwd_chain(x1, ln_w, ln_b, eps, w12, b1, w22, b2):
    B, C = x1.shape[:2]
    V = _vox(x1)
    Hd = w12.shape[0]
    timed = (f"mlp_chain_fwd_{C}", x1.element_size() * (2 * x1.numel() + B * Hd * V), 4 * B * V * C * Hd)
    _, x2, z1, st, _ = _mlp_chain_fwd(timed, x1, ln_w, ln_b, eps, w12, b1, w22, b2, inp=x1)
    return x2, z1, st


_OUTPROJ_MLP = os.environ.get("FZ_OUTPROJ_MLP", "1") != "0"


def _outproj_mlp_ok(C, Hd, V):
    return _OUTPROJ_MLP and _mlp_chain_ok(C, Hd, V) and bool(N.lib().fz_mlp_pre_supported(C, Hd, V, N.products()))


def _outproj_mlp_fwd_chain(a, wout2, bout, x, ln_w, ln_b, eps, w12, b1, w22, b2, head=None, drop=None):
    B, C = a.shape[:2]
    V = _vox(a)
    Hd = w12.shape[0]
    nlogits = B * head[0].shape[0] * V if head is not None else 0
    timed = (f"outproj_mlp_chain_fwd_{C}", a.element_size() * (4 * a.numel() + B * Hd * V + nlogits), 4 * B * V * C * Hd + 2 * B * V * C * C)
    x1, x2, z1, st, logits = _mlp_chain_fwd(timed, a, ln_w, ln_b, eps, w12, b1, w22, b2, pre=(a, wout2, bout, x), head=head, drop=drop)
    if head is not None:
        return x1, x2, z1, st, logits
    return x1, x2, z1, st


def _mlp_bwd_chain(g2, z1, w12, w22, x1, st, ln_w):
    B, C = x1.shape[:2]
    V = _vox(x1)
    Hd = w12.shape[0]
    gz1 = torch.empty_like(z1)
    gx1 = torch.empty_like(x1)
    rows = N.lib().fz_mlp_partials(B, V)
    part = torch.empty((rows, 2 * C), dtype=torch.float32, device=x1.device)
    d = _mlp_desc(1, x1, w12, w22, B=B, C=C, Hd=Hd, V=V, inp=g2, ln_w=ln_w, stats=st, z1=z1, x1=x1, out=gx1)
    d.gz1, d.part = gz1.data_ptr(), part.data_ptr()
    with torch.cuda.device(x1.device):
        rc = Fn._timed(f"mlp_chain_bwd_{C}", x1.element_size() * (3 * x1.numel() + 2 * z1.numel()),
                       lambda: N.lib().fz_mlp_chain(ctypes.byref(d), N.stream_ptr(x1)), cols=B * V, flops=4 * B * V * C * Hd)
        N.check(rc, "fz_mlp_chain")
        ggamma, gbeta = _reduce_affine_rows(part, rows, C, x1)
    return gz1, gx1, ggamma, gbeta


def _mlp_wgrad_fused_ok(C, Hd, V):
    return _mlp_chain_ok(C, Hd, V) and C == 32 and Hd in (64, 128) and os.environ.get("FZ_MLP_FUSED_WGRAD", "1") != "0"


def _mlp_bwd_chain_wgrad(g2, z1, w12, w22, x1, st, ln_w, ln_b):
    B, C = x1.shape[:2]
    V = _vox(x1)
    Hd = w12.shape[0]
    dev = x1.device
    gx1 = torch.empty_like(x1)
    gpar = torch.empty(64, dtype=torch.float32, device=dev)
    wpart = torch.empty(N.lib().fz_mlp_wgrad_workspace_bytes(B, V) // 4, dtype=torch.float32, device=dev)
    gw1 = _GB.out_like(w12, (Hd, C), torch.float32)
    gw2 = _GB.out_like(w22, (C, Hd), torch.float32)
    gb1 = torch.empty(Hd, dtype=torch.float32, device=dev)
    gb2 = torch.empty(C, dtype=torch.float32, device=dev)
    glp = torch.empty(x1.shape, dtype=torch.float32, device=dev) if Hd == 128 else None
    d = _mlp_desc(2, x1, w12, w22, B=B, C=C, Hd=Hd, V=V, inp=g2, ln_w=ln_w, ln_b=ln_b, stats=st, z1=z1, x1=x1, out=gx1)
    d.gln, d.wpart, d.glp = gpar.data_ptr(), wpart.data_ptr(), _p(glp)
    d.gw1, d.gb1, d.gw2, d.gb2 = gw1.data_ptr(), gb1.data_ptr(), gw2.data_ptr(), gb2.data_ptr()
    nbytes = x1.element_size() * (3 * x1.numel() + z1.numel()) + (0 if Hd == 64 else x1.element_size() * 2 * x1.numel() + 8 * x1.numel())
    with torch.cuda.device(dev), _finish_scope(wpart, gpar, gw1, gb1, gw2, gb2):
        rc = Fn._timed(f"mlp_chain_bwd_wgrad_{C}" + ("" if Hd == 64 else f"x{Hd}"), nbytes,
                       lambda: N.lib().fz_mlp_chain(ctypes.byref(d), N.stream_ptr(x1)), cols=B * V, flops=8 * B * V * C * Hd)
        N.check(rc, "fz_mlp_chain")
    return gx1, gpar[:32], gpar[32:], gw1, gb1, gw2, gb2


_SIDE = {}


def _side_stream(dev, ncols):
    lim = int(os.environ.get("FZ_SIDE_WGRAD", "0"))
    if lim <= 0 or ncols > lim:
        return None
    key = (dev.type, dev.index)
    if key not in _SIDE:
        _SIDE[key] = torch.cuda.Stream(device=dev)
    return _SIDE[key]


class _LateJoin:
    enabled = False
    keep = []
    owed = []
    devices = set()
    queued = False
    verified = 0


def _end_of_backward():
    _LateJoin.queued = False
    join_wgrad_streams()


def reset_late_join():
    d = _LateJoin
    if d.devices:
        wait_wgrad_streams()
    d.owed.clear()
# ... 852 lines not shown
        tls.cur = self
        return self

    def __exit__(self, *exc):
        BlockPrologue._tls.cur = self.prev

    @staticmethod
    def take(x):
        cur = getattr(BlockPrologue._tls, "cur", None)
        if cur is not None and cur.x is x:
            return cur.t, cur.st
        return None


def cat_linear(x1, x2, w, b=None):
    if _native_ok(x1, x2, w, b) and x1.shape[1] % 2 == 0 and x2.shape[1] % 2 == 0:
        return CatLinearFn.apply(x1, x2, w, b)
    _warn_composed("cat+Linear", x1, x2, w, b)
    return linear_cf(torch.cat([x1, x2], dim=1), w, b)


def _block_dropout_bits(x, C, Hd, drop):
    B, V = x.shape[0], _vox(x)
    seed = Fn.dropout_seed(x.device)
    return tuple(None if p == 0 else Fn.dropout_keep_bits(seed, s, B, ch, V, p) for s, (ch, p) in enumerate(zip((C, Hd, C), drop)))


def _block_tail_fwd(a, wout2, bout, x, ln_w, ln_b, eps, w12, b1, w22, b2, drop=None, bits=(None, None, None)):
    B, C = x.shape[:2]
    V = _vox(x)
    Hd = w12.shape[0]
    new = lambda ch: torch.empty((B, ch, *x.shape[2:]), dtype=x.dtype, device=x.device)
    (p0, p1, p2), (m0, m1, m2) = drop or (0, 0, 0), bits
    if m0 is not None:
        o = new(C)
        _gemm([a], wout2, o, B=B, Cin=C, Vin=V, M=C, K=C, Ncol=V, bias=bout, name="linear")
        x1 = Fn.dropout_apply(N.DROP_RES, m0, p0, o, x)
        del o
    else:
        x1 = new(C)
        _gemm([a], wout2, x1, B=B, Cin=C, Vin=V, M=C, K=C, Ncol=V, bias=bout, res=x, name="act_linear_res")
    z1 = new(Hd)
    st2 = _ln_stats(B, V, x.device)
    _gemm([x1], w12, z1, B=B, Cin=C, Vin=V, M=Hd, K=C, Ncol=V, bias=b1, ln=(ln_w, ln_b, eps), stats_out=st2, name="ln_linear")
    h, bact = (Fn.dropout_apply(N.DROP_GELU, m1, p1, z1), ACT["none"]) if m1 is not None else (z1, ACT["gelu"])
    if m2 is not None:
        o = new(C)
        _gemm([h], w22, o, B=B, Cin=Hd, Vin=V, M=C, K=Hd, Ncol=V, bias=b2, bact=bact, name="linear")
        x2 = Fn.dropout_apply(N.DROP_RES, m2, p2, o, x1)
        del o
    else:
        x2 = new(C)
        _gemm([h], w22, x2, B=B, Cin=Hd, Vin=V, M=C, K=Hd, Ncol=V, bias=b2, bact=bact, res=x1, name="act_linear_res")
    return x1, x2, z1, st2


class FactorizerBlockFn(torch.autograd.Function):

    _fz_acts = (0, 4, 5, 14, 15, 16, 17, 18)

    @staticmethod
    @_fwd
    def forward(ctx, x, n1w, n1b, win, u0, v0, wout, bout, n2w, n2b, w1, b1, w2, b2, cfg, head_w=None, head_b=None,
                t_pre=None, st_pre=None):
        x = x.contiguous()
        B, C = x.shape[:2]
        V = _vox(x)
        sp = x.shape[2:]
        geo, T, G, solver, neps = cfg["geo"], cfg["T"], cfg["G"], cfg["solver"], cfg["nmf_eps"]
        win2, wout2 = win.reshape(C, C), wout.reshape(C, C)
        Hd = w1.shape[0]
        w12, w22 = w1.reshape(Hd, C), w2.reshape(C, Hd)
        u0c, v0c = u0.contiguous(), v0.contiguous()
        new = lambda ch: torch.empty((B, ch, *sp), dtype=x.dtype, device=x.device)
        drop = cfg.get("drop")
        bits = _block_dropout_bits(x, C, Hd, drop) if drop is not None else (None, None, None)
        if t_pre is not None:
            t, st1 = t_pre, st_pre
        else:
            t = new(C)
            st1 = _ln_stats(B, V, x.device)
            _gemm([x], win2, t, B=B, Cin=C, Vin=V, M=C, K=C, Ncol=V, ln=(n1w, n1b, cfg["eps1"]), stats_out=st1,
                  eact=ACT["relu"], name="ln_linear")
        m = None
        if cfg["core"]:
            a = Fn.FactCoreFn.forward(_Ctx(), t, u0c, v0c, geo, T, G, solver, neps, True)
        else:
            m = Fn._swm_fwd_raw(t, geo)
            ym, _, _ = Fn._nmf_fwd_raw(m, u0c, v0c, T, solver, neps)
            a = Fn._swm_inv_raw(ym, geo, average=True)
            del ym
        logits = None
        tail = (a, wout2, bout, x, n2w, n2b, cfg["eps2"], w12, b1, w22, b2)
        if (_mlp_drop_ok if drop is not None else _outproj_mlp_ok)(C, Hd, V) and a.is_contiguous():
            head = (head_w.reshape(head_w.shape[0], C), head_b) if head_w is not None and drop is None else None
            x1, x2, z1, st2, *logits = _outproj_mlp_fwd_chain(*tail, head=head, drop=(bits, drop) if drop is not None else None)
            logits = logits[0] if logits else None
        elif drop is None and _mlp_chain_ok(C, Hd, V):
            x1 = new(C)
            _gemm([a], wout2, x1, B=B, Cin=C, Vin=V, M=C, K=C, Ncol=V, bias=bout, res=x, name="act_linear_res")
            x2, z1, st2 = _mlp_fwd_chain(x1, n2w, n2b, cfg["eps2"], w12, b1, w22, b2)
        else:
            x1, x2, z1, st2 = _block_tail_fwd(*tail, drop, bits)
        ctx.save_for_backward(x, st1, t, a, x1, st2, z1, m, n1w, n1b, win2, u0c, v0c, wout2, n2w, n2b, w12, w22, *bits)
        ctx.cfg = cfg
        ctx.shapes = (win.shape, wout.shape, w1.shape, w2.shape)
        ctx.prm = tuple(weakref.ref(t) for t in (win, wout, bout, w1, b1, w2, b2))
        if head_w is not None:
            if logits is None:
                raise RuntimeError("FactorizerBlockFn: head fusion asked for a configuration outside fz_mlp_pre_supported "
                                   "(callers check block_head_fusable first)")
            ctx.mark_non_differentiable(logits)
            ctx.set_materialize_grads(False)
            return x2, logits
        return x2

    @staticmethod
    @_bwd
    def backward(ctx, g2, _g_logits=None):
        x, st1, t, a, x1, st2, z1, m, n1w, n1b, win2, u0c, v0c, wout2, n2w, n2b, w12, w22, *bits = ctx.saved_tensors
        cfg = ctx.cfg
        drop = cfg.get("drop")
        if g2 is None:
            g2 = torch.zeros_like(x)
        g2 = g2.contiguous()
        B, C = x.shape[:2]
        V = _vox(x)
        Hd = w12.shape[0]
        dev, dt = x.device, x.dtype
        geo, T, G, solver, neps = cfg["geo"], cfg["T"], cfg["G"], cfg["solver"], cfg["nmf_eps"]
        cur = torch.cuda.current_stream(dev)
        side = _side_stream(dev, B * V)
        keep = []

        pending = []

        def wgrad(*args, **kw):
            if _WGRAD_GROUP:
                kw.pop("name", None)
                pending.append((args[0], args[1], args[2], kw))
                return args[2]
            if side is None:
                return _wgrad(*args, **kw)
            side.wait_stream(cur)
            keep.extend(t for t in (args[0], *args[1], kw.get("stats")) if t is not None)
            with torch.cuda.stream(side):
                return _wgrad(*args, **kw)

        chain = _mlp_chain_ok(C, Hd, V) and drop is None
        (p0, p1, p2), (m0, m1, m2) = drop or (0, 0, 0), bits
        if drop is None and _mlp_wgrad_fused_ok(C, Hd, V):
            gx1, gg2, gbt2, gw1, gb1, gw2, gb2 = _mlp_bwd_chain_wgrad(g2, z1, w12, w22, x1, st2, n2w, n2b)
        else:
            gelu = ACT["gelu" if m1 is None else "none"]
            gf = Fn.dropout_apply(N.DROP_RES, m2, p2, g2) if m2 is not None else g2
            gw2 = _GB.out_like(w22)
            gb2 = torch.empty(C, dtype=torch.float32, device=dev)
            if chain:
                gz1, gx1, gg2, gbt2 = _mlp_bwd_chain(g2, z1, w12, w22, x1, st2, n2w)
            else:
                gz1 = torch.empty_like(z1)
                _gemm([gf], w22, gz1, B=B, Cin=C, Vin=V, M=Hd, K=C, Ncol=V, w_t=True, ldw=Hd, emul=(z1 if m1 is None else None),
                      emul_kind=gelu, name="linear_dgrad")
                if m1 is not None:
                    gz1 = Fn.dropout_apply(N.DROP_GELU_BWD, m1, p1, gz1, z1)
            h = Fn.dropout_apply(N.DROP_GELU, m1, p1, z1) if m1 is not None else z1
            wgrad(gf, [h], gw2, B=B, M=C, Cin=Hd, K=Hd, Vq=V, Ncols=V, gbias=gb2, qact=gelu, name="wgrad_linear")
            del h, gf
            if not chain:
                gx1, gg2, gbt2 = _dgrad_lnbwd(gz1, w12, x1, st2, n2w, g2)
            gw1 = _GB.out_like(w12)
            gb1 = torch.empty(Hd, dtype=torch.float32, device=dev)
            wgrad(gz1, [x1], gw1, B=B, M=Hd, Cin=C, K=C, Vq=V, Ncols=V, gbias=gb1, stats=st2, ln=(n2w, n2b),
                  name="wgrad_ln_linear")
            del gz1
        go, go_drop = gx1, None
        if m0 is not None:
            if _dw_fused_ok(C, V):
                go_drop = (m0, p0)
            else:
                go = Fn.dropout_apply(N.DROP_RES, m0, p0, gx1)
        dw = _dw_fused_ok(C, V)
        if dw:
            ga, gwo, gbo, _, _ = _gemm_dw(go, wout2, a, want_bias=True, name="dgrad_wgrad", drop=go_drop)
        else:
            ga = torch.empty_like(a)
            _gemm([go], wout2, ga, B=B, Cin=C, Vin=V, M=C, K=C, Ncol=V, w_t=True, ldw=C, name="linear_dgrad")
            gwo = _GB.out_like(wout2)
            gbo = torch.empty(C, dtype=torch.float32, device=dev)
            wgrad(go, [a], gwo, B=B, M=C, Cin=C, K=C, Vq=V, Ncols=V, gbias=gbo, name="wgrad_linear")
        del go
        if G <= 0:
            gt = torch.zeros_like(t)
        elif cfg["core"]:
            c2 = _Ctx()
            c2.saved_tensors = (t, u0c, v0c)
            c2.cfg = (geo, T, G, solver, neps, True)
            gt = Fn.FactCoreFn.backward(c2, ga)[0]
        else:
            gym = Fn._swm_fwd_raw(ga, geo, div=geo.nshift)
            gm = Fn._nmf_bwd_raw(m, u0c, v0c, gym, None, None, T, G, solver, neps)
            del gym
            gt = Fn._swm_inv_raw(gm, geo, average=False, gate=m)
            del gm
        del ga
        if dw:
            gx, gwi, _, gg1, gbt1 = _gemm_dw(gt, win2, x, ln=(n1w, n1b), stats=st1, gadd=gx1, name="dgrad_lnbwd_wgrad")
        else:
            gx, gg1, gbt1 = _dgrad_lnbwd(gt, win2, x, st1, n1w, gx1)
            gwi = _GB.out_like(win2)
            wgrad(gt, [x], gwi, B=B, M=C, Cin=C, K=C, Vq=V, Ncols=V, stats=st1, ln=(n1w, n1b), name="wgrad_ln_linear")
        if pending:
            if side is None:
                _wgrad_group(pending, f"wgrad_block_{C}x{Hd}")
            else:
                side.wait_stream(cur)
                for pr in pending:
                    keep.extend(t for t in (pr[0], *pr[1], pr[3].get("stats"), pr[3].get("pmul")) if t is not None)
                with torch.cuda.stream(side):
                    _wgrad_group(pending, f"wgrad_block_{C}x{Hd}")
            pending.clear()
        if side is not None:
            if _LateJoin.enabled:
                _LateJoin.keep.extend(keep)
                _LateJoin.devices.add((dev.type, dev.index))
                _LateJoin.owed.extend(zip(ctx.prm, (t.data_ptr() for t in (gwi, gwo, gbo, gw1, gb1, gw2, gb2))))
                if not _LateJoin.queued:
                    _LateJoin.queued = True
                    torch.autograd.Variable._execution_engine.queue_callback(_end_of_backward)
            else:
                cur.wait_stream(side)
            keep.clear()
        s_in, s_out, s_1, s_2 = ctx.shapes
        return (gx, gg1, gbt1, gwi.reshape(s_in), None, None, gwo.reshape(s_out), gbo, gg2, gbt2,
                gw1.reshape(s_1), gb1, gw2.reshape(s_2), gb2, None, None, None, None, None)[:len(ctx.needs_input_grad)]


_head_fusion = _threading.local()


class HeadFusion:

    def __init__(self, block, head_params):
        self.block, self.head_params, self.logits = block, head_params, None

    def __enter__(self):
        self.prev = getattr(_head_fusion, "slot", None)
        _head_fusion.slot = self
        return self

    def __exit__(self, *exc):
        _head_fusion.slot = self.prev


def head_fusion_slot():
    return getattr(_head_fusion, "slot", None)


def block_head_fusable(C, Hd, V, head_w, x):
    return (C == 32 and _outproj_mlp_ok(C, Hd, V) and head_w is not None and head_w.dtype == torch.float32 and head_w.numel() == head_w.shape[0] * C
            and 1 <= head_w.shape[0] <= 4 and x.is_cuda and _HEAD_BWD)


class HeadOfBlockFn(torch.autograd.Function):

    _fz_acts = (0, 3)

    @staticmethod
# ... 28 lines not shown
```

include/factorizer_hip.h:

```cpp
#ifndef FACTORIZER_HIP_H
#define FACTORIZER_HIP_H

#include <stdint.h>

#ifdef __cplusplus
extern "C" {
#endif

#define FZ_OK 0
#define FZ_E_SHAPE (-1)
#define FZ_E_UNSUPPORTED (-2)
#define FZ_E_HIP (-3)
#define FZ_E_ARG (-4)

#define FZ_STORE_F32 0
#define FZ_STORE_BF16 1

#define FZ_SOLVER_MU 0
#define FZ_SOLVER_HALS 1
#define FZ_SOLVER_CD 2
#define FZ_SOLVER_SMU 3

typedef void* fz_stream_t;

int fz_version(void);
#define FZ_ABI_VERSION 7
int fz_abi_version(void);
int fz_set_tile_order(int descending);
int fz_finish_defer(int on);
int fz_finish_pending(void);
int fz_finish_flush(fz_stream_t stream);
int fz_finish_flush_all(fz_stream_t waiter);
const char* fz_last_error_string(void);
int64_t fz_launch_count(void);

int fz_swm_fwd(const void* x, void* y, int B, int C, int D, int H, int W, int d, int pd,
               int ph, int pw, int nshift, const int* shifts, int elem_bytes, int relu,
               int div, fz_stream_t stream);

int fz_swm_inv(const void* y, void* x, int B, int C, int D, int H, int W, int d, int pd,
               int ph, int pw, int nshift, const int* shifts, int average, const void* gate,
               int act_dtype, fz_stream_t stream);

int fz_nmf_fwd(const void* x, const float* u0, const float* v0, void* y, float* u_out,
               float* v_out, int64_t nmat, int M, int N, int R, int T, int solver, float eps,
               int act_dtype, fz_stream_t stream);

int fz_nmf_bwd(const void* x, const float* u0, const float* v0, const void* gy,
               const float* gu, const float* gv, void* gx, int64_t nmat, int M, int N, int R,
               int T, int Tgrad, int solver, float eps, int act_dtype, fz_stream_t stream);

int fz_nmf_supported(int M, int N, int R, int T, int Tgrad);

int fz_gnmf_supported(int M, int64_t N, int R, int T, int Tgrad);
int64_t fz_gnmf_workspace_bytes(int64_t nmat, int M, int64_t N, int R, int T, int backward);
int fz_gnmf_launches(int T, int Tgrad, int backward);
int fz_gnmf_fwd(const float* x, const float* u0, const float* v0, float* y, float* u_out, float* v_out,
                int64_t nmat, int M, int64_t N, int R, int T, int solver, float eps, void* workspace,
                fz_stream_t stream);
int fz_gnmf_bwd(const float* x, const float* u0, const float* v0, const float* gy, const float* gu,
                const float* gv, float* gx, int64_t nmat, int M, int64_t N, int R, int T, int Tgrad, int solver,
                float eps, void* workspace, fz_stream_t stream);

int fz_gnmfx_supported(int M, int64_t N, int R, int T, int Tgrad);
int64_t fz_gnmfx_workspace_bytes(int64_t nmat, int M, int64_t N, int R, int T, int backward);
int fz_gnmfx_launches(int M, int64_t N, int R, int T, int Tgrad, int backward);
int fz_gnmfx_fwd(const float* x, const float* u0, const float* v0, float* y, float* u_out, float* v_out,
                 int64_t nmat, int M, int64_t N, int R, int T, int solver, float eps, void* workspace,
                 fz_stream_t stream);
int fz_gnmfx_bwd(const float* x, const float* u0, const float* v0, const float* gy, const float* gu,
                 const float* gv, float* gx, int64_t nmat, int M, int64_t N, int R, int T, int Tgrad, int solver,
                 float eps, void* workspace, fz_stream_t stream);

int fz_nmf_cf_supported(int C, int D, int H, int W, int d, int pd, int ph, int pw, int R, int T, int Tgrad);
int fz_nmf_cf_fwd(const void* t, const float* u0, const float* v0, void* out, int B, int C, int D,
                  int H, int W, const int* shift, int accumulate, int divisor, int R, int T,
                  int solver, float eps, int act_dtype, fz_stream_t stream);
int fz_nmf_cf_bwd(const void* t, const float* u0, const float* v0, const void* ga, void* gt, int B,
                  int C, int D, int H, int W, const int* shift, int accumulate, int nshift,
                  int relu_gate, int R, int T, int Tgrad, int solver, float eps, int act_dtype,
                  fz_stream_t stream);

int fz_nmf_cf_factors_supported(int C, int D, int H, int W, int d, int pd, int ph, int pw, int R, int T, int Tgrad,
                                int nshift, const int* shifts);
int fz_nmf_cf_fwd_store_factors(const void* t, const float* u0, const float* v0, float* vfac, float* ufac, int B,
                                int C, int D, int H, int W, const int* shift, int R, int T, int solver, float eps,
                                int act_dtype, fz_stream_t stream);
int fz_nmf_cf_fwd_from_factors(const void* t, const float* u0, const float* v0, const float* vfac, const float* ufac,
                               void* out, int B, int C, int D, int H, int W, const int* shift, const int* prev_shift,
                               int divisor, int R, int T, int solver, float eps, int act_dtype, fz_stream_t stream);

int fz_nmf_cf_bwd_factors_supported(int C, int D, int H, int W, int d, int pd, int ph, int pw, int R, int T, int Tgrad,
                                    int solver, int relu_gate, int nshift, const int* shifts);
int fz_nmf_cf_bwd_store_factors(const void* t, const float* v0, const void* ga, float* gcfac, float* cofac, int B, int C,
                                int D, int H, int W, const int* shift, int nshift, int T, int Tgrad, float eps,
                                int act_dtype, fz_stream_t stream);
int fz_nmf_cf_bwd_from_factors(const void* t, const float* v0, const void* ga, const float* gcfac, const float* cofac,
                               void* gt, int B, int C, int D, int H, int W, const int* shift, const int* prev_shift,
                               int nshift, int T, int Tgrad, float eps, int act_dtype, fz_stream_t stream);

int fz_nmf_pcf_supported(int C, int D, int H, int W, int d, int pd, int ph, int pw, int R, int T, int Tgrad);
int fz_nmf_pcf_fwd(const void* t, const float* u0, const float* v0, void* out, int B, int C, int D, int H, int W,
                   int pd, int ph, int pw, const int* shift, int accumulate, int divisor, int R, int T, int solver,
                   float eps, int act_dtype, fz_stream_t stream);
int fz_nmf_pcf_bwd(const void* t, const float* u0, const float* v0, const void* ga, void* gt, int B, int C, int D,
                   int H, int W, int pd, int ph, int pw, const int* shift, int accumulate, int nshift, int relu_gate,
                   int R, int T, int Tgrad, int solver, float eps, int act_dtype, fz_stream_t stream);
int fz_nmf_pcf_bwd_prefers_separate(int pd, int ph, int pw, int act_dtype);
int fz_act_add(void* dst, const void* src, int64_t n, int act_dtype, fz_stream_t stream);

#define FZ_LOAD_PLAIN 0
#define FZ_LOAD_S2D 1
#define FZ_LOAD_K3 2
#define FZ_EPI_PLAIN 0
#define FZ_EPI_D2S 1
#define FZ_EPI_LNBWD 2
#define FZ_LOAD_S2D_2D 3
#define FZ_LOAD_K3_2D 4
#define FZ_EPI_D2S_2D 3
#define FZ_ACT_NONE 0
#define FZ_ACT_RELU 1
#define FZ_ACT_GELU 2

#define FZ_PRODUCTS_DEFAULT 0
#define FZ_PRODUCTS_SPLIT_BF16 1
#define FZ_PRODUCTS_FP32_MFMA 2

typedef struct fz_gemm_desc {
  const void* x[4];
  int nsrc;
  int src_mode;
  int c0;
  int Cin;
  int64_t Vin;
  int Di, Hi, Wi;
  const float* w;
  int w_t, ldw;
  int M, K;
  const float* bias;
  int ln;
  const float* ln_g;
  const float* ln_b;
  float ln_eps;
  float* stats_out;
  int bact;
  const void* bmul;
  int bmul_kind;
  int eact;
  const void* res;
  const void* emul;
  int emul_kind;
  void* y;
  int64_t Ncol;
  int Ho, Wo;
  int B;
  int loader, epilogue;
  const void* lnb_x;
  const float* lnb_stats;
  const float* lnb_g;
  const void* lnb_gadd;
  float* lnb_part;
  int act_dtype;
  int products;
  int tune;
} fz_gemm_desc;

int64_t fz_gemm_lnbwd_partials(const fz_gemm_desc* desc);
int fz_reduce_rows(const float* part, int64_t rows, int n, float* out, float* tmp, fz_stream_t stream);

int fz_gemm(const fz_gemm_desc* desc, fz_stream_t stream);
int fz_gemm_plan(const fz_gemm_desc* desc, char* form, int cap);
int fz_gemm_bx_enable(int on);

typedef struct fz_mlp_desc {
  int mode;
  const void* in;
  const float* w1;
  const float* w2;
  const float* b1;
  const float* b2;
  const float* ln_g;
  const float* ln_b;
  float ln_eps;
  float* stats;
  void* z1;
  void* gz1;
  const void* x1;
  void* out;
  float* part;
  int B, C, H;
  int64_t V;
  int act_dtype;
  void* wpart;
  float* gw1;
  float* gb1;
  float* gw2;
  float* gb2;
  float* gln;
  float* glp;
  int products;
  const void* pre_in;
  const float* pre_w;
  const float* pre_b;
  const void* pre_res;
  void* pre_out;
  const float* post_w;
  const float* post_b;
  void* post_out;
  int post_m;
} fz_mlp_desc;
typedef struct fz_mlp_dropout {
  const uint32_t* m0;
  const uint32_t* m1;
  const uint32_t* m2;
  float s0, s1, s2;
} fz_mlp_dropout;

typedef struct fz_gemm_dw_desc {
  const void* g;
  const void* q;
  const float* w;
  int ln;
  const float* stats;
  const float* ln_g;
  const float* ln_b;
  const void* gadd;
  void* y;
  float* gln;
  void* wpart;
  float* gw;
  float* gb;
  int B, C;
  int64_t V;
  int act_dtype;
  int ldgw;
  int ldw;
  const uint32_t* drop_m;
  float drop_s;
} fz_gemm_dw_desc;
int fz_gemm_dw_rows(int B, int64_t V);
int64_t fz_gemm_dw_workspace_bytes(int B, int64_t V);
int fz_gemm_dw(const fz_gemm_dw_desc* desc, fz_stream_t stream);

int fz_head_bwd_rows(void);
int64_t fz_head_bwd_workspace_bytes(void);
int fz_head_bwd(const void* gy, const void* x, const float* w, void* gx, float* part, int B, int M, int C, int64_t V,
                int act_dtype, fz_stream_t stream);
int fz_head_fwd(const void* x, const float* w, const float* bias, void* y, int B, int M, int C, int64_t V, int act_dtype,
                fz_stream_t stream);

int fz_upcat_compose(const float* w_t, const float* w_b, int ldb, const float* b_t, const float* b_ad, float* wc, float* wbt, float* bias,
                     int Cd, int O, int M, fz_stream_t stream);
int fz_upcat_wgrads(const float* gt, const float* w_t, const float* w_b, int ldb, const float* gb_ad, const float* b_t, float* gw_t,
                    float* gw_b, int ldg, float* gb_t, int Cd, int O, int M, fz_stream_t stream);
int fz_upcat_supported(int C, int Cd, int D, int H, int W);
int fz_upcat(const void* skip, const void* deep, const float* wa, int lda, const float* wbt, const float* bias, void* out,
             int B, int C, int Cd, int D, int H, int W, int act_dtype, fz_stream_t stream);
int fz_upcat_bwd_supported(int C1, int Cd, int D, int H, int W, int act_dtype);
int64_t fz_upcat_bwd_workspace_bytes(int B, int D, int H, int W);
int fz_upcat_bwd(const void* g, const void* skip, const void* deep, const float* wa, int lda, const float* wc, void* g_skip,
                 void* g_deep, void* workspace, float* gw_a, int ldg, float* gb, float* gt, int B, int C1, int Cd, int D, int H,
                 int W, int act_dtype, fz_stream_t stream);
typedef struct fz_block_prologue {
  const float* ln_g;
  const float* ln_b;
  float ln_eps;
  const float* w;
  void* t;
  float* stats;
} fz_block_prologue;
int fz_upcat2(const void* skip, const void* deep, const float* wa, int lda, const float* wbt, const float* bias, void* out,
              int B, int C, int Cd, int D, int H, int W, int act_dtype, const fz_block_prologue* pro, fz_stream_t stream);

int fz_mlp_supported(int C, int H, int64_t V);
int fz_mlp_pre_supported(int C, int H, int64_t V, int products);
int fz_mlp_drop_supported(int C, int H, int64_t V, int products);
int64_t fz_mlp_partials(int B, int64_t V);
int fz_mlp_wgrad_rows(int B, int64_t V);
int64_t fz_mlp_wgrad_workspace_bytes(int B, int64_t V);
int fz_mlp_chain(const fz_mlp_desc* desc, fz_stream_t stream);
int fz_mlp_chain_drop(const fz_mlp_desc* desc, const fz_mlp_dropout* drop, fz_stream_t stream);

#define FZ_QL_PLAIN 0
#define FZ_QL_S2D 1
#define FZ_QL_K3 2
#define FZ_QL_S2D_2D 3
#define FZ_QL_K3_2D 4

typedef struct fz_wgrad_desc {
  const void* p;
  int M;
  const void* pmul;
  int pmul_kind;
  const void* q[4];
  int nsrc, src_mode, c0;
  int Cin;
  int K;
  int64_t Vq;
  int D, H, W;
  int64_t N;
  int Ho, Wo;
  const float* stats;
  int qact;
  const float* ln_g;
  const float* ln_b;
  float* gw;
  float* gbias;
  int accumulate;
  int B;
  int loader;
  int act_dtype;
  int products;
} fz_wgrad_desc;

int64_t fz_wgrad_workspace_bytes(const fz_wgrad_desc* desc);
int fz_wgrad(const fz_wgrad_desc* desc, void* workspace, fz_stream_t stream);
int fz_wgrad_group(const fz_wgrad_desc* const* descs, void* const* workspaces, int n, fz_stream_t stream);

int fz_ln_fwd(const void* x , const float* gamma, const float* beta, void* y ,
              float* stats, int B, int C, int64_t V, float eps, int act_dtype, fz_stream_t stream);
int64_t fz_ln_bwd_workspace_bytes(int C);
int64_t fz_ln_bwd_workspace_bytes2(int B, int C, int64_t V);
int fz_ln_bwd(const void* gl, const void* x, const float* stats, const float* gamma,
              const void* gadd, void* gx , float* gparams, void* workspace,
              int B, int C, int64_t V, int act_dtype, fz_stream_t stream);

// ... 162 lines not shown
```

Measured before the change: 133.3.

## Feed out-projection GEMMs directly from NMF core factors instead of materialized tensor

Result: faster. 135.9, median of 6 (+1.9%).

```diff
diff --git a/factorizer_amd/_native.py b/factorizer_amd/_native.py
--- a/factorizer_amd/_native.py
+++ b/factorizer_amd/_native.py
@@ -162,6 +162,19 @@
                 ("lnb_gadd", _vp), ("lnb_part", _vp), ("act_dtype", _i), ("products", _i), ("tune", _i)]
 
 
+class OutprojFac(_c.Structure):
+    _fields_ = [("v", _vp * 2), ("u", _vp * 2), ("dims", _i * 3), ("heads", _i), ("shift", _i * 6)]
+
+
+def outproj_fac(fac, geo):
+    d = OutprojFac()
+    d.v[0], d.u[0], d.v[1], d.u[1] = (t.data_ptr() for t in fac)
+    d.dims[:] = list(geo.spatial)
+    d.heads = geo.h
+    d.shift[:] = [int(v) for s in geo.shifts3 for v in s]
+    return d
+
+
 class MlpDesc(_c.Structure):
     _fields_ = [("mode", _i), ("inp", _vp), ("w1", _vp), ("w2", _vp), ("b1", _vp), ("b2", _vp), ("ln_g", _vp),
                 ("ln_b", _vp), ("ln_eps", _f), ("stats", _vp), ("z1", _vp), ("gz1", _vp), ("x1", _vp), ("out", _vp),
@@ -225,6 +238,8 @@
     "fz_nmf_cf_fwd": ([_vp] * 4 + [_i] * 5 + [_c.POINTER(_i)] + [_i] * 5 + [_f, _i, _vp], _i),
     "fz_nmf_cf_bwd": ([_vp] * 5 + [_i] * 5 + [_c.POINTER(_i)] + [_i] * 7 + [_f, _i, _vp], _i),
     "fz_nmf_cf_factors_supported": ([_i] * 12 + [_c.POINTER(_i)], _i),
+    "fz_nmf_cf_factors_to_tensor": ([_vp] * 5 + [_i] * 5 + [_c.POINTER(_i)] * 2 + [_i, _vp], _i),
+    "fz_outproj_factors_supported": ([_i] * 13 + [_c.POINTER(_i)] + [_i] * 3, _i),
     "fz_nmf_cf_fwd_store_factors": ([_vp] * 5 + [_i] * 5 + [_c.POINTER(_i)] + [_i] * 3 + [_f, _i, _vp], _i),
     "fz_nmf_cf_fwd_from_factors": ([_vp] * 6 + [_i] * 5 + [_c.POINTER(_i)] * 2 + [_i] * 4 + [_f, _i, _vp], _i),
     "fz_nmf_cf_bwd_factors_supported": ([_i] * 14 + [_c.POINTER(_i)], _i),
@@ -238,6 +253,8 @@
     "fz_mlp_pre_supported": ([_i, _i, _i64, _i], _i),
     "fz_mlp_drop_supported": ([_i, _i, _i64, _i], _i),
     "fz_mlp_chain_drop": ([_c.POINTER(MlpDesc), _c.POINTER(MlpDropout), _vp], _i),
+    "fz_mlp_chain_fac": ([_c.POINTER(MlpDesc), _c.POINTER(OutprojFac), _vp], _i),
+    "fz_gemm_dw_fac": ([_c.POINTER(GemmDwDesc), _c.POINTER(OutprojFac), _vp], _i),
     "fz_conv3_prologue_supported": ([_i] * 4, _i),
     "fz_conv3_fwd2": ([_vp] * 4 + [_i] * 8 + [_c.POINTER(BlockPrologue), _vp], _i),
     "fz_upcat2": ([_vp, _vp, _vp, _i, _vp, _vp, _vp] + [_i] * 7 + [_c.POINTER(BlockPrologue), _vp], _i),
diff --git a/factorizer_amd/csrc/cf_patch.h b/factorizer_amd/csrc/cf_patch.h
--- /dev/null
+++ b/factorizer_amd/csrc/cf_patch.h
@@ -0,0 +1,26 @@
+#pragma once
+
+#if defined(__HIPCC__)
+#define FZ_CF_HD __host__ __device__ inline __attribute__((always_inline))
+#else
+#define FZ_CF_HD inline
+#endif
+
+namespace fz {
+
+FZ_CF_HD unsigned cf_voxel_patch(int d, int h, int w, int D, int H, int W, int s0, int s1, int s2) {
+  d += s0; if (d >= D) d -= D;
+  h += s1; if (h >= H) h -= H;
+  w += s2; if (w >= W) w -= W;
+  return (unsigned)(((d >> 3) * (H >> 3) + (h >> 3)) * (W >> 3) + (w >> 3));
+}
+
+#if defined(__HIPCC__)
+__device__ inline __attribute__((always_inline)) float cf_two_window_value(float u0, float v0, float u1, float v1) {
+  float p0 = u0 * v0, p1 = u1 * v1;
+  asm("" : "+v"(p0), "+v"(p1));
+  return ((0.0f + p0) + p1) * 0.5f;
+}
+#endif
+
+}
diff --git a/factorizer_amd/csrc/gemm_dw.hip b/factorizer_amd/csrc/gemm_dw.hip
--- a/factorizer_amd/csrc/gemm_dw.hip
+++ b/factorizer_amd/csrc/gemm_dw.hip
@@ -1,6 +1,7 @@
 #include "gemm_bx.h"
 #include "gemm_shared.h"
 #include "finish.h"
+#include "outproj_fac.h"
 
 namespace fz {
 
@@ -22,8 +23,12 @@
 
 template <bool LNB, typename AT, typename... DropX>
 __global__ __launch_bounds__(256, 2) void gemm_dw_kernel(DwArgsT<AT> p, int ntiles, DropX... dx) {
-  constexpr bool DROP = sizeof...(DropX) > 0;
+  constexpr bool FAC = is_fac_v<DropX...>;
+  constexpr bool DROP = sizeof...(DropX) > 0 && !FAC;
   const DropArgs dr = drop_of(dx...);
+  const FacArgs fa = fac_of(dx...);
+  static_assert(!FAC || (!LNB && sizeof(AT) == 4), "factors: the out-projection pair, fp32 storage");
+  static_assert(kFacLds <= 32 * kTS, "the factor staging area lives in the wave's Qb rows");
   constexpr int NACC = 2;
   constexpr int kWave = 64 * kTS;
   constexpr bool BXB = sizeof(AT) == 2;
@@ -73,9 +78,14 @@
 
   int tile = blockIdx.x;
   float bv[16][NACC];
+  FacTile ft;
   auto fetch_tile = [&](int t) {
     const int bt = t / tiles_per_sample;
     const int64_t ct = ((int64_t)(t % tiles_per_sample) * 4 + wave) * (32 * NACC) + NACC * j;
+    if constexpr (FAC) {
+      const int64_t n0 = ((int64_t)(t % tiles_per_sample) * 4 + wave) * (32 * NACC);
+      fac_fetch(fa, bt, (unsigned)(n0 < p.V ? n0 : 0), lane, ft);
+    }
     const unsigned lo = (unsigned)h * (unsigned)p.V + (unsigned)(ct < p.V ? ct : 0);
     const AT* xb = p.g + (int64_t)bt * 32 * p.V;
 #pragma unroll
@@ -108,6 +118,13 @@
       vload<NACC>(sp + nc, mu);
       vload<NACC>(sp + p.V + nc, rs);
     }
+    if constexpr (FAC) {
+      float qv[16][NACC];
+      fac_build(fa, ft, Qb, lane, qv);
+#pragma unroll
+      for (int s = 0; s < 16; ++s)
+        *reinterpret_cast<float2*>(Qb + (2 * s + h) * kTS + 2 * j) = make_float2(col_ok ? qv[s][0] : 0.f, col_ok ? qv[s][1] : 0.f);
+    } else
 #pragma unroll
     for (int hf = 0; hf < 2; ++hf) {
       float xv[8][NACC];
@@ -320,7 +337,7 @@
 
 extern "C" int fz_gemm_dw_rows(int B, int64_t V);
 template <typename AT>
-static int gemm_dw_launch(const fz_gemm_dw_desc* d, fz_stream_t stream) {
+static int gemm_dw_launch(const fz_gemm_dw_desc* d, const fz_outproj_fac* fac, fz_stream_t stream) {
   DwArgsT<AT> a;
   a.g = (const AT*)d->g; a.q = (const AT*)d->q; a.w = d->w; a.ldw = d->ldw > 0 ? d->ldw : 32; a.stats = d->stats; a.ln_g = d->ln_g; a.gadd = (const AT*)d->gadd;
   a.y = (AT*)d->y; a.wpart = (float*)d->wpart; a.V = d->V; a.B = d->B;
@@ -328,7 +345,18 @@
   const int rows = fz_gemm_dw_rows(d->B, d->V);
   constexpr int lds = (1536 + 32 + 256 + 4 * 64 * kTS) * (int)sizeof(float);
   hipStream_t st = (hipStream_t)stream;
-  if (d->drop_m) {
+  if (fac) {
+    if constexpr (sizeof(AT) == 4) {
+      FacArgs fa;
+      const int rc = fac_args(fac, d->V, "fz_gemm_dw_fac", fa);
+      if (rc != FZ_OK) return rc;
+      auto kern = gemm_dw_kernel<false, AT, FacArgs>;
+      FZ_HIP_OK(hipFuncSetAttribute(reinterpret_cast<const void*>(kern), hipFuncAttributeMaxDynamicSharedMemorySize, lds));
+      hipLaunchKernelGGL(kern, dim3((unsigned)rows), dim3(256), lds, st, a, ntiles, fa);
+    } else {
+      return fail(FZ_E_UNSUPPORTED, "fz_gemm_dw_fac: fp32 storage only");
+    }
+  } else if (d->drop_m) {
     auto kern = gemm_dw_kernel<false, AT, DropArgs>;
     FZ_HIP_OK(hipFuncSetAttribute(reinterpret_cast<const void*>(kern), hipFuncAttributeMaxDynamicSharedMemorySize, lds));
     hipLaunchKernelGGL(kern, dim3((unsigned)rows), dim3(256), lds, st, a, ntiles, drop_args(d->drop_m, nullptr, nullptr, d->drop_s, 1.f, 1.f, d->V));
@@ -357,9 +385,11 @@
   return (int64_t)fz_gemm_dw_rows(B, V) * kDwRow * (int64_t)sizeof(float);
 }
 
-extern "C" int fz_gemm_dw(const fz_gemm_dw_desc* d, fz_stream_t stream) {
+static int gemm_dw_entry(const fz_gemm_dw_desc* d, const fz_outproj_fac* fac, fz_stream_t stream) {
   if (!d) return fail(FZ_E_ARG, "fz_gemm_dw: null descriptor");
-  if (!d->g || !d->q || !d->w || !d->y || !d->wpart || !d->gw) return fail(FZ_E_ARG, "fz_gemm_dw: null pointer");
+  if (fac && (d->q || d->ln || d->drop_m || d->act_dtype != FZ_STORE_F32 || d->C != 32))
+    return fail(FZ_E_UNSUPPORTED, "fz_gemm_dw_fac: needs q == NULL, no LayerNorm form, no dropout, fp32 storage, C == 32 (fz_outproj_factors_supported)");
+  if (!d->g || (!d->q && !fac) || !d->w || !d->y || !d->wpart || !d->gw) return fail(FZ_E_ARG, "fz_gemm_dw: null pointer");
   if (d->ln && (!d->stats || !d->ln_g || !d->ln_b || !d->gln)) return fail(FZ_E_ARG, "fz_gemm_dw: the LayerNorm form needs stats, gamma, beta, gln");
   if (!d->ln && d->gadd) return fail(FZ_E_UNSUPPORTED, "fz_gemm_dw: gadd only with the LayerNorm backward");
   if (d->drop_m && d->ln) return fail(FZ_E_UNSUPPORTED, "fz_gemm_dw: dropout on g only without the LayerNorm backward");
@@ -368,7 +398,14 @@
   if (d->ldgw != 0 && d->ldgw < 32) return fail(FZ_E_ARG, "fz_gemm_dw: ldgw must be 0 (= 32) or >= 32");
   if (d->ldw != 0 && d->ldw < 32) return fail(FZ_E_ARG, "fz_gemm_dw: ldw must be 0 (= 32) or >= 32");
   if (d->B < 1 || d->V < 1 || d->V % 4 != 0 || d->V > ((int64_t)1 << 27)) return fail(FZ_E_UNSUPPORTED, "fz_gemm_dw: needs B >= 1, V % 4 == 0, V <= 2^27");
-  if (d->act_dtype == FZ_STORE_F32) return gemm_dw_launch<float>(d, stream);
-  if (d->act_dtype == FZ_STORE_BF16) return gemm_dw_launch<bf16>(d, stream);
+  if (d->act_dtype == FZ_STORE_F32) return gemm_dw_launch<float>(d, fac, stream);
+  if (d->act_dtype == FZ_STORE_BF16) return gemm_dw_launch<bf16>(d, fac, stream);
   return fail(FZ_E_ARG, "fz_gemm_dw: act_dtype must be FZ_STORE_F32 or FZ_STORE_BF16");
 }
+
+extern "C" int fz_gemm_dw(const fz_gemm_dw_desc* d, fz_stream_t stream) { return gemm_dw_entry(d, nullptr, stream); }
+
+extern "C" int fz_gemm_dw_fac(const fz_gemm_dw_desc* d, const fz_outproj_fac* fac, fz_stream_t stream) {
+  if (!fac) return fail(FZ_E_ARG, "fz_gemm_dw_fac: null factor block");
+  return gemm_dw_entry(d, fac, stream);
+}
diff --git a/factorizer_amd/csrc/mlp_chain.h b/factorizer_amd/csrc/mlp_chain.h
--- a/factorizer_amd/csrc/mlp_chain.h
+++ b/factorizer_amd/csrc/mlp_chain.h
@@ -48,7 +48,8 @@
 static int knob_mlp_wgs(int dflt) { return knob_pos(FZ_KNOB("FZ_MLP_WGS"), dflt); }
 
 template <typename AT>
-int chain32_launch(const fz_mlp_desc* d, const fz_mlp_dropout* drop, const GemmArgsT<AT>& a, const ChainArgsT<AT>& c, fz_stream_t stream);
+int chain32_launch(const fz_mlp_desc* d, const fz_mlp_dropout* drop, const fz_outproj_fac* fac, const GemmArgsT<AT>& a, const ChainArgsT<AT>& c,
+                   fz_stream_t stream);
 template <typename AT>
 int chain64_launch(const fz_mlp_desc* d, const GemmArgsT<AT>& a, const ChainArgsT<AT>& c, fz_stream_t stream);
 template <typename AT>
diff --git a/factorizer_amd/csrc/mlp_chain.hip b/factorizer_amd/csrc/mlp_chain.hip
--- a/factorizer_amd/csrc/mlp_chain.hip
+++ b/factorizer_amd/csrc/mlp_chain.hip
@@ -16,6 +16,13 @@
   return 0;
 }
 
+extern "C" int fz_outproj_factors_supported(int C, int Hd, int D, int H, int W, int d, int pd, int ph, int pw, int R, int T, int Tgrad,
+                                            int nshift, const int* shifts, int act_dtype, int products, int dropout) {
+  if (C != 32 || Hd != 64 || act_dtype != FZ_STORE_F32 || dropout || nshift != 2) return 0;
+  if (!fz_nmf_cf_factors_supported(C, D, H, W, d, pd, ph, pw, R, T, Tgrad, nshift, shifts)) return 0;
+  return fz_mlp_pre_supported(C, Hd, (int64_t)D * H * W, products);
+}
+
 extern "C" int fz_mlp_supported(int C, int H, int64_t V) {
   const bool shape = (C == 32 && (H == 64 || H == 128)) || (C == 64 && H == 128);
   return (shape && V > 0 && (V % 4) == 0 && V <= ((int64_t)1 << 27)) ? 1 : 0;
@@ -27,12 +34,12 @@
 }
 
 template <typename AT>
-static void forward_args(const fz_mlp_desc* d, int ldw, int ldwB, GemmArgsT<AT>& a, ChainArgsT<AT>& c) {
+static void forward_args(const fz_mlp_desc* d, bool fac, int ldw, int ldwB, GemmArgsT<AT>& a, ChainArgsT<AT>& c) {
   a.w = d->w1; a.w_t = 0; a.ldw = ldw;
   a.bias = d->b1; a.ln = 1; a.ln_g = d->ln_g; a.ln_b = d->ln_b; a.ln_eps = d->ln_eps; a.stats_out = d->stats;
   a.res = (const AT*)d->in; a.y = (AT*)d->out;
   c.wB = d->w2; c.wB_t = 0; c.ldwB = ldwB; c.biasB = d->b2; c.side = (AT*)d->z1;
-  if (d->pre_in) {
+  if (d->pre_in || fac) {
     c.preA = (const AT*)d->pre_in; c.preW = d->pre_w; c.preB = d->pre_b; c.preRes = (const AT*)d->pre_res; c.preOut = (AT*)d->pre_out;
     if (d->C == 64) a.res = (const AT*)d->pre_out;
     else { c.postW = d->post_w; c.postB = d->post_b; c.postOut = (AT*)d->post_out; c.postM = d->post_m; }
@@ -46,7 +53,7 @@
   c.wB = d->w1; c.wB_t = 1; c.ldwB = ldwB; c.side = side;
 }
 
-static int mlp_check(const fz_mlp_desc* d, const fz_mlp_dropout* dd, bool drop) {
+static int mlp_check(const fz_mlp_desc* d, const fz_mlp_dropout* dd, bool drop, bool fac) {
   if (!fz_mlp_supported(d->C, d->H, d->V)) return fail(FZ_E_UNSUPPORTED, "fz_mlp_chain: needs (C, H) in {(32, 64), (32, 128), (64, 128)}, V % 4 == 0");
   if (drop) {
     if (!fz_mlp_drop_supported(d->C, d->H, d->V, d->products) || d->mode != 0 || !d->pre_in)
@@ -56,7 +63,10 @@
   }
   if (d->C == 64 && d->mode == 2) return fail(FZ_E_UNSUPPORTED, "fz_mlp_chain: the fused weight gradients need C == 32, H == 64");
   if (d->B < 0) return fail(FZ_E_SHAPE, "fz_mlp_chain: negative batch");
-  const bool pre = d->pre_in != nullptr;
+  if (fac && (d->C != 32 || d->H != 64 || d->mode != 0 || d->act_dtype != FZ_STORE_F32 || drop || d->pre_in
+              || !fz_mlp_pre_supported(d->C, d->H, d->V, d->products)))
+    return fail(FZ_E_UNSUPPORTED, "fz_mlp_chain_fac: needs (C, H) = (32, 64), mode 0, fp32 storage, split-bf16 products, pre_in == NULL (fz_outproj_factors_supported)");
+  const bool pre = d->pre_in != nullptr || fac;
   if (pre && (d->mode != 0 || !d->pre_w || !d->pre_res || !d->pre_out))
     return fail(FZ_E_ARG, "fz_mlp_chain: pre_in needs mode 0, pre_w, pre_res, pre_out (see fz_mlp_pre_supported)");
   if (pre && !fz_mlp_pre_supported(d->C, d->H, d->V, d->products))
@@ -75,9 +85,9 @@
 }
 
 template <typename AT>
-static int mlp_launch(const fz_mlp_desc* d, const fz_mlp_dropout* dd, fz_stream_t stream) {
+static int mlp_launch(const fz_mlp_desc* d, const fz_mlp_dropout* dd, const fz_outproj_fac* fac, fz_stream_t stream) {
   const bool drop = dd && (dd->m0 || dd->m1 || dd->m2);
-  const int rc = mlp_check(d, dd, drop);
+  const int rc = mlp_check(d, dd, drop, fac != nullptr);
   if (rc != FZ_OK) return rc;
   if (d->B == 0) {
     if (d->mode == 2) {
@@ -93,23 +103,30 @@
   GemmArgsT<AT> a = {};
   ChainArgsT<AT> c = {};
   a.x[0] = (const AT*)d->in; a.nsrc = 1; a.c0 = d->C; a.Cin = d->C; a.Vin = d->V; a.M = d->H; a.K = d->C; a.Ncol = d->V; a.B = d->B;
-  if (d->mode == 0) forward_args(d, d->C, d->H, a, c);
+  if (d->mode == 0) forward_args(d, fac != nullptr, d->C, d->H, a, c);
   else backward_args(d, d->H, d->C, d->mode == 1 ? (AT*)d->gz1 : (AT*)nullptr, a, c);
   if (d->C == 64) return chain64_launch(d, a, c, stream);
   if (d->mode == 2) return chain_wg_launch(d, a, c, stream);
-  return chain32_launch(d, drop ? dd : nullptr, a, c, stream);
+  return chain32_launch(d, drop ? dd : nullptr, fac, a, c, stream);
 }
 
 extern "C" int fz_mlp_chain(const fz_mlp_desc* d, fz_stream_t stream) {
   if (!d) return fail(FZ_E_ARG, "fz_mlp_chain: null descriptor");
-  if (d->act_dtype == FZ_STORE_F32) return mlp_launch<float>(d, nullptr, stream);
-  if (d->act_dtype == FZ_STORE_BF16) return mlp_launch<bf16>(d, nullptr, stream);
+  if (d->act_dtype == FZ_STORE_F32) return mlp_launch<float>(d, nullptr, nullptr, stream);
+  if (d->act_dtype == FZ_STORE_BF16) return mlp_launch<bf16>(d, nullptr, nullptr, stream);
   return fail(FZ_E_ARG, "fz_mlp_chain: act_dtype must be FZ_STORE_F32 or FZ_STORE_BF16");
+}
+
+extern "C" int fz_mlp_chain_fac(const fz_mlp_desc* d, const fz_outproj_fac* fac, fz_stream_t stream) {
+  if (!d || !fac) return fail(FZ_E_ARG, "fz_mlp_chain_fac: null descriptor");
+  if (d->act_dtype == FZ_STORE_F32) return mlp_launch<float>(d, nullptr, fac, stream);
+  if (d->act_dtype == FZ_STORE_BF16) return mlp_launch<bf16>(d, nullptr, fac, stream);
+  return fail(FZ_E_ARG, "fz_mlp_chain_fac: act_dtype must be FZ_STORE_F32 or FZ_STORE_BF16");
 }
 
 extern "C" int fz_mlp_chain_drop(const fz_mlp_desc* d, const fz_mlp_dropout* drop, fz_stream_t stream) {
   if (!d || !drop) return fail(FZ_E_ARG, "fz_mlp_chain_drop: null descriptor");
-  if (d->act_dtype == FZ_STORE_F32) return mlp_launch<float>(d, drop, stream);
-  if (d->act_dtype == FZ_STORE_BF16) return mlp_launch<bf16>(d, drop, stream);
+  if (d->act_dtype == FZ_STORE_F32) return mlp_launch<float>(d, drop, nullptr, stream);
+  if (d->act_dtype == FZ_STORE_BF16) return mlp_launch<bf16>(d, drop, nullptr, stream);
   return fail(FZ_E_ARG, "fz_mlp_chain_drop: act_dtype must be FZ_STORE_F32 or FZ_STORE_BF16");
 }
diff --git a/factorizer_amd/csrc/mlp_chain32.hip b/factorizer_amd/csrc/mlp_chain32.hip
--- a/factorizer_amd/csrc/mlp_chain32.hip
+++ b/factorizer_amd/csrc/mlp_chain32.hip
@@ -1,11 +1,16 @@
 #include "mlp_chain.h"
+#include "outproj_fac.h"
 
 namespace fz {
 
 template <bool BWD, int NACC, int HB, typename AT = float, bool BX = false, bool PRE = false, typename... DropX>
 __global__ __launch_bounds__(256, (NACC == 2 && HB == 2 && !BWD && !BX) ? 3 : 2) void gemm_chain_kernel(GemmArgsT<AT> p, ChainArgsT<AT> c, int ntiles, DropX... dx) {
-  constexpr bool DROP = sizeof...(DropX) > 0;
+  constexpr bool FAC = is_fac_v<DropX...>;
+  constexpr bool DROP = sizeof...(DropX) > 0 && !FAC;
   const DropArgs dr = drop_of(dx...);
+  const FacArgs fa = fac_of(dx...);
+  static_assert(!FAC || (PRE && !BWD && NACC == 2 && sizeof(AT) == 4), "factors: the forward chain with the out-projection in front, fp32 storage");
+  static_assert(kFacLds <= 32 * 32 * NACC, "the factor staging area lives in the wave's stash rows");
   static_assert(!DROP || (PRE && !BWD && NACC == 2), "dropout: the forward chain with the out-projection in front");
   constexpr int NW = 4;
   constexpr int HID = 32 * HB, N1 = BX ? 1536 * HB : 16 * HB * 64;
@@ -108,13 +113,19 @@
   int tile = blockIdx.x;
   float bv[16][NACC];
   float xr[PRE ? 16 : 1][NACC];
+  FacTile ft;
   auto fetch_tile = [&](int t) {
     const int bt = t / tiles_per_sample;
     const int64_t ct = ((int64_t)(t % tiles_per_sample) * NW + wave) * (32 * NACC) + NACC * j;
     const unsigned lo = (unsigned)h * (unsigned)p.Ncol + (unsigned)(ct < p.Ncol ? ct : 0);
+    if constexpr (FAC) {
+      const int64_t n0 = ((int64_t)(t % tiles_per_sample) * NW + wave) * (32 * NACC);
+      fac_fetch(fa, bt, (unsigned)(n0 < p.Ncol ? n0 : 0), lane, ft);
+    } else {
     const AT* xb = (PRE ? c.preA : p.x[0]) + (int64_t)bt * 32 * p.Ncol;
 #pragma unroll
     for (int s = 0; s < 16; ++s) vload<NACC>(xb + (int64_t)(2 * s) * p.Ncol + lo, bv[s]);
+    }
     if constexpr (PRE) {
       const unsigned lr = (unsigned)(4 * h) * (unsigned)p.Ncol + (unsigned)(ct < p.Ncol ? ct : 0);
       const AT* rb0 = c.preRes + (int64_t)bt * 32 * p.Ncol;
@@ -133,6 +144,7 @@
     const int64_t nc = col_ok ? col_off : 0;
     const unsigned lane_row = (unsigned)(4 * h) * (unsigned)p.Ncol + (unsigned)nc;
     if constexpr (PRE) {
+      if constexpr (FAC) fac_build(fa, ft, &stash[wave][0][0], lane, bv);
       f32x16 acc0[NACC];
 #pragma unroll
       for (int q = 0; q < NACC; ++q)
@@ -381,10 +393,11 @@
 }
 
 template <typename AT>
-int chain32_launch(const fz_mlp_desc* d, const fz_mlp_dropout* drop, const GemmArgsT<AT>& a, const ChainArgsT<AT>& c, fz_stream_t stream) {
+int chain32_launch(const fz_mlp_desc* d, const fz_mlp_dropout* drop, const fz_outproj_fac* fac, const GemmArgsT<AT>& a, const ChainArgsT<AT>& c,
+                   fz_stream_t stream) {
   hipStream_t st = (hipStream_t)stream;
   const int ntiles = (int)fz_mlp_partials(d->B, d->V);
-  const bool bwd = d->mode != 0, pre = d->pre_in != nullptr;
+  const bool bwd = d->mode != 0, pre = d->pre_in != nullptr || fac;
   const bool bx = !bwd && d->H == 64 && products_split(d->products) && knob_chain_fwd_bx();
   const int wgs = knob_mlp_wgs(d->H == 128 || bx ? 512 : 768);
   const dim3 grid((unsigned)(ntiles < wgs ? ntiles : wgs)), block(256);
@@ -394,6 +407,16 @@
   } else if (d->H == 128) hipLaunchKernelGGL((gemm_chain_kernel<false, 2, 4>), grid, block, 0, st, a, c, ntiles);
   else if (!bx) hipLaunchKernelGGL((gemm_chain_kernel<false, 2, 2>), grid, block, 0, st, a, c, ntiles);
   else if (!pre) hipLaunchKernelGGL((gemm_chain_kernel<false, 2, 2, AT, true>), grid, block, 0, st, a, c, ntiles);
+  else if (fac) {
+    if constexpr (sizeof(AT) == 4) {
+      FacArgs fa;
+      const int rc = fac_args(fac, d->V, "fz_mlp_chain_fac", fa);
+      if (rc != FZ_OK) return rc;
+      hipLaunchKernelGGL((gemm_chain_kernel<false, 2, 2, AT, true, true, FacArgs>), grid, block, 0, st, a, c, ntiles, fa);
+    } else {
+      return fail(FZ_E_UNSUPPORTED, "fz_mlp_chain_fac: fp32 storage only");
+    }
+  }
   else if (!drop) hipLaunchKernelGGL((gemm_chain_kernel<false, 2, 2, AT, true, true>), grid, block, 0, st, a, c, ntiles);
   else
     hipLaunchKernelGGL((gemm_chain_kernel<false, 2, 2, AT, true, true, DropArgs>), grid, block, 0, st, a, c, ntiles,
@@ -401,7 +424,7 @@
   FZ_LAUNCH_CHECK();
   return FZ_OK;
 }
-template int chain32_launch<float>(const fz_mlp_desc*, const fz_mlp_dropout*, const GemmArgsT<float>&, const ChainArgsT<float>&, fz_stream_t);
-template int chain32_launch<bf16>(const fz_mlp_desc*, const fz_mlp_dropout*, const GemmArgsT<bf16>&, const ChainArgsT<bf16>&, fz_stream_t);
+template int chain32_launch<float>(const fz_mlp_desc*, const fz_mlp_dropout*, const fz_outproj_fac*, const GemmArgsT<float>&, const ChainArgsT<float>&, fz_stream_t);
+template int chain32_launch<bf16>(const fz_mlp_desc*, const fz_mlp_dropout*, const fz_outproj_fac*, const GemmArgsT<bf16>&, const ChainArgsT<bf16>&, fz_stream_t);
 
 }
diff --git a/factorizer_amd/csrc/nmf_cf.h b/factorizer_amd/csrc/nmf_cf.h
--- a/factorizer_amd/csrc/nmf_cf.h
+++ b/factorizer_amd/csrc/nmf_cf.h
@@ -1,6 +1,7 @@
 #pragma once
 #include <cstdlib>
 
+#include "cf_patch.h"
 #include "fz_common.h"
 #include "nmf_core.h"
 #include "nmf_gram.h"
@@ -284,6 +285,7 @@
 template <typename AT>
 int cf_fwd_launch(const AT* t, const float* u0, const float* v0, AT* out, float* vfac, float* ufac, const CfLaunch& a, int form,
                   int R, int T, int solver, float eps);
+int cf_factors_to_tensor_launch(const float* vf0, const float* uf0, const float* vf1, const float* uf1, float* out, const CfLaunch& a);
 template <typename AT>
 int cf_bwd_launch(const AT* t, const float* u0, const float* v0, const AT* ga, AT* gt, const CfLaunch& a, int relu_gate, int R,
                   int T, int G, int solver, float eps);
diff --git a/factorizer_amd/csrc/nmf_cf.hip b/factorizer_amd/csrc/nmf_cf.hip
--- a/factorizer_amd/csrc/nmf_cf.hip
+++ b/factorizer_amd/csrc/nmf_cf.hip
@@ -147,6 +147,23 @@
                         "fz_nmf_cf_fwd_from_factors: bad act_dtype");
 }
 
+extern "C" int fz_nmf_cf_factors_to_tensor(const float* vfac0, const float* ufac0, const float* vfac1, const float* ufac1, void* out,
+                                           int B, int C, int D, int H, int W, const int* shift0, const int* shift1, int act_dtype,
+                                           fz_stream_t stream) {
+  if (act_dtype == FZ_STORE_BF16) return fail(FZ_E_UNSUPPORTED, "fz_nmf_cf_factors_to_tensor: fp32 storage only");
+  if (act_dtype != FZ_STORE_F32) return fail(FZ_E_ARG, "fz_nmf_cf_factors_to_tensor: bad act_dtype");
+  CfLaunch a;
+  const int rc = cf_prepare(a, B, C, D, H, W, shift0, shift1, 0, 2, stream, [&](const CfGeom& q) {
+    if (!vfac0 || !ufac0 || !vfac1 || !ufac1 || !out || !shift1)
+      return fail(FZ_E_ARG, "fz_nmf_cf_factors_to_tensor: null pointer (vfac0, ufac0, vfac1, ufac1, out or shift1)");
+    if (W % 64) return fail(FZ_E_UNSUPPORTED, "fz_nmf_cf_factors_to_tensor: W must be a multiple of 64");
+    if ((q.s2 % 4) || (q.ps2 % 4)) return fail(FZ_E_UNSUPPORTED, "fz_nmf_cf_factors_to_tensor: W-axis shift must be a multiple of 4");
+    return (int)FZ_OK;
+  });
+  if (rc != FZ_OK || a.nmat == 0) return rc;
+  return cf_factors_to_tensor_launch(vfac0, ufac0, vfac1, ufac1, (float*)out, a);
+}
+
 extern "C" int fz_nmf_cf_bwd_factors_supported(int C, int D, int H, int W, int d, int pd, int ph, int pw, int R, int T, int Tgrad,
                                                int solver, int relu_gate, int nshift, const int* shifts) {
   if (FZ_KNOB("FZ_CF_BWD_FACTORS").set && FZ_KNOB("FZ_CF_BWD_FACTORS").val == 0) return 0;
diff --git a/factorizer_amd/csrc/nmf_cf_fwd.hip b/factorizer_amd/csrc/nmf_cf_fwd.hip
--- a/factorizer_amd/csrc/nmf_cf_fwd.hip
+++ b/factorizer_amd/csrc/nmf_cf_fwd.hip
@@ -180,4 +180,37 @@
 template int cf_fwd_launch<float>(const float*, const float*, const float*, float*, float*, float*, const CfLaunch&, int, int, int, int, float);
 template int cf_fwd_launch<bf16>(const bf16*, const float*, const float*, bf16*, float*, float*, const CfLaunch&, int, int, int, int, float);
 
-}
+__global__ __launch_bounds__(256) void nmf_cf_factors_to_tensor_kernel(const float* __restrict__ vf0, const float* __restrict__ uf0,
+                                                                       const float* __restrict__ vf1, const float* __restrict__ uf1,
+                                                                       float* __restrict__ out, CfGeom q, int64_t nchunk) {
+  const int64_t i = (int64_t)blockIdx.x * 256 + threadIdx.x;
+  if (i >= nchunk) return;
+  const unsigned vol = (unsigned)(q.D * q.H * q.W), per = vol >> 2;
+  const int64_t bh = i / per;
+  const unsigned vox = (unsigned)(i % per) << 2;
+  const int w = (int)(vox % (unsigned)q.W), hh = (int)((vox / (unsigned)q.W) % (unsigned)q.H), d = (int)(vox / (unsigned)(q.W * q.H));
+  const int64_t npatch = (int64_t)q.G0 * q.G1 * q.G2;
+  const float* up0 = uf0 + ((bh * npatch + cf_voxel_patch(d, hh, w, q.D, q.H, q.W, q.s0, q.s1, q.s2)) << 3);
+  const float* up1 = uf1 + ((bh * npatch + cf_voxel_patch(d, hh, w, q.D, q.H, q.W, q.ps0, q.ps1, q.ps2)) << 3);
+  const float4 v0 = ld4(vf0 + bh * vol + vox), v1 = ld4(vf1 + bh * vol + vox);
+  const float4 a0 = ld4(up0), b0 = ld4(up0 + 4), a1 = ld4(up1), b1 = ld4(up1 + 4);
+  const float u0[8] = {a0.x, a0.y, a0.z, a0.w, b0.x, b0.y, b0.z, b0.w};
+  const float u1[8] = {a1.x, a1.y, a1.z, a1.w, b1.x, b1.y, b1.z, b1.w};
+#pragma unroll
+  for (int dd = 0; dd < 8; ++dd)
+    st4(out + (bh * 8 + dd) * vol + vox,
+        make_float4(cf_two_window_value(u0[dd], v0.x, u1[dd], v1.x), cf_two_window_value(u0[dd], v0.y, u1[dd], v1.y),
+                    cf_two_window_value(u0[dd], v0.z, u1[dd], v1.z), cf_two_window_value(u0[dd], v0.w, u1[dd], v1.w)));
+}
+
+int cf_factors_to_tensor_launch(const float* vf0, const float* uf0, const float* vf1, const float* uf1, float* out, const CfLaunch& a) {
+  const CfGeom& q = a.q;
+  const int64_t nchunk = (int64_t)q.B * q.h * ((int64_t)q.D * q.H * q.W / 4);
+  if (nchunk == 0) return FZ_OK;
+  hipLaunchKernelGGL(nmf_cf_factors_to_tensor_kernel, dim3((unsigned)((nchunk + 255) / 256)), dim3(256), 0, a.st, vf0, uf0, vf1, uf1,
+                     out, q, nchunk);
+  FZ_LAUNCH_CHECK();
+  return FZ_OK;
+}
+
+}
diff --git a/factorizer_amd/csrc/outproj_fac.h b/factorizer_amd/csrc/outproj_fac.h
--- /dev/null
+++ b/factorizer_amd/csrc/outproj_fac.h
@@ -0,0 +1,112 @@
+#pragma once
+#include <string>
+#include <type_traits>
+
+#include "cf_patch.h"
+#include "gemm_shared.h"
+
+namespace fz {
+
+struct FacArgs {
+  const float* v[2];
+  const float* u[2];
+  int D, H, W;
+  int s[2][3];
+};
+template <class... X>
+constexpr bool is_fac_v = (std::is_same<X, FacArgs>::value || ... || false);
+__device__ __forceinline__ DropArgs drop_of(const FacArgs&) { return DropArgs{}; }
+__device__ __forceinline__ FacArgs fac_of() { return FacArgs{}; }
+__device__ __forceinline__ FacArgs fac_of(const DropArgs&) { return FacArgs{}; }
+__device__ __forceinline__ FacArgs fac_of(const FacArgs& f) { return f; }
+
+static int fac_args(const fz_outproj_fac* d, int64_t V, const char* who, FacArgs& f) {
+  auto bad = [&](int code, const char* what) { return fail(code, (std::string(who) + ": " + what).c_str()); };
+  if (!d->v[0] || !d->v[1] || !d->u[0] || !d->u[1]) return bad(FZ_E_ARG, "null factor pointer (v[0..1], u[0..1])");
+  const int D = d->dims[0], H = d->dims[1], W = d->dims[2];
+  if (d->heads != 4) return bad(FZ_E_UNSUPPORTED, "needs heads == 4 (C = 32, head_dim 8)");
+  if (D < 8 || H < 8 || W < 64 || (D % 8) || (H % 8) || (W % 64) || (int64_t)D * H * W != V)
+    return bad(FZ_E_UNSUPPORTED, "needs dims multiples of 8, W % 64 == 0, D H W == V");
+  f.D = D; f.H = H; f.W = W;
+  const int S[3] = {D, H, W};
+  for (int w = 0; w < 2; ++w) {
+    f.v[w] = d->v[w]; f.u[w] = d->u[w];
+    for (int i = 0; i < 3; ++i) {
+      int s = d->shift[3 * w + i] % S[i];
+      f.s[w][i] = s < 0 ? s + S[i] : s;
+    }
+    if (f.s[w][2] % 4) return bad(FZ_E_UNSUPPORTED, "needs W-axis shifts that are multiples of 4");
+  }
+  return FZ_OK;
+}
+
+constexpr int kFacRow = 36;
+constexpr int kFacWin = 9 * kFacRow;
+constexpr int kFacLds = 2 * kFacWin;
+
+struct FacTile {
+  float4 ur[3];
+  float2 vv[2][4];
+};
+
+__device__ __forceinline__ void fac_fetch(const FacArgs& f, int b, unsigned n0, int lane, FacTile& t) {
+  const unsigned vol = (unsigned)(f.D * f.H * f.W);
+  const int w0 = (int)(n0 % (unsigned)f.W), hh = (int)((n0 / (unsigned)f.W) % (unsigned)f.H), d = (int)(n0 / (unsigned)(f.W * f.H));
+  const int G1 = f.H >> 3, G2 = f.W >> 3;
+  const unsigned npatch = (unsigned)((f.D >> 3) * G1 * G2);
+#pragma unroll
+  for (int k = 0; k < 3; ++k) {
+    const int id = lane + 64 * k;
+    if (id < 144) {
+      const int win = id >= 72, rem = id - 72 * win, i = rem >> 3, head = (rem >> 1) & 3, half = rem & 1;
+      const unsigned row = cf_voxel_patch(d, hh, w0, f.D, f.H, f.W, f.s[win][0], f.s[win][1], f.s[win][2]);
+      const int g2 = (int)(row % (unsigned)G2);
+      int g2i = g2 + i; if (g2i >= G2) g2i -= G2;
+      const int64_t patch = (int64_t)(b * 4 + head) * npatch + (row - (unsigned)g2 + (unsigned)g2i);
+      t.ur[k] = *reinterpret_cast<const float4*>(f.u[win] + (patch << 3) + 4 * half);
+    } else {
+      t.ur[k] = make_float4(0.f, 0.f, 0.f, 0.f);
+    }
+  }
+  const unsigned vo = n0 + 2u * (unsigned)(lane & 31);
+#pragma unroll
+  for (int win = 0; win < 2; ++win)
+#pragma unroll
+    for (int head = 0; head < 4; ++head)
+      t.vv[win][head] = *reinterpret_cast<const float2*>(f.v[win] + (int64_t)(b * 4 + head) * vol + vo);
+}
+
+__device__ __forceinline__ void fac_build(const FacArgs& f, const FacTile& t, float* S, int lane, float (&bv)[16][2]) {
+  const int j = lane & 31, h = lane >> 5;
+#pragma unroll
+  for (int k = 0; k < 3; ++k) {
+    const int id = lane + 64 * k;
+    if (id < 144) {
+      const int win = id >= 72, rem = id - 72 * win, i = rem >> 3, head = (rem >> 1) & 3, half = rem & 1;
+      float* dst = S + win * kFacWin + i * kFacRow + head * 4 + half * 2;
+      *reinterpret_cast<float2*>(dst) = make_float2(t.ur[k].x, t.ur[k].z);
+      *reinterpret_cast<float2*>(dst + 16) = make_float2(t.ur[k].y, t.ur[k].w);
+    }
+  }
+  __builtin_amdgcn_fence(__ATOMIC_ACQ_REL, "wavefront");
+  float u[2][16];
+#pragma unroll
+  for (int win = 0; win < 2; ++win) {
+    const int i = ((f.s[win][2] & 7) + 2 * j) >> 3;
+    const float* src = S + win * kFacWin + i * kFacRow + h * 16;
+#pragma unroll
+    for (int c = 0; c < 4; ++c) {
+      const float4 x = *reinterpret_cast<const float4*>(src + 4 * c);
+      u[win][4 * c + 0] = x.x; u[win][4 * c + 1] = x.y; u[win][4 * c + 2] = x.z; u[win][4 * c + 3] = x.w;
+    }
+  }
+  __builtin_amdgcn_fence(__ATOMIC_ACQ_REL, "wavefront");
+#pragma unroll
+  for (int s = 0; s < 16; ++s) {
+    const float2 a = t.vv[0][s >> 2], b = t.vv[1][s >> 2];
+    bv[s][0] = cf_two_window_value(u[0][s], a.x, u[1][s], b.x);
+    bv[s][1] = cf_two_window_value(u[0][s], a.y, u[1][s], b.y);
+  }
+}
+
+}
diff --git a/factorizer_amd/functional.py b/factorizer_amd/functional.py
--- a/factorizer_amd/functional.py
+++ b/factorizer_amd/functional.py
@@ -385,6 +385,51 @@
         ok = geo._factors_ok[k] = bool(N.lib().fz_nmf_cf_bwd_factors_supported(
             geo.C, *geo.spatial, geo.d, *geo.patch, *k[1:4], N.SOLVER_ID[solver], int(k[5]), geo.nshift, geo._carr))
     return ok
+
+
+_OUTPROJ_FACTORS = os.environ.get("FZ_OUTPROJ_FACTORS", "1") != "0"
+
+
+def outproj_factors_supported(geo: Geometry, Hd, R, T, G, act_dtype, dropout) -> bool:
+    if not _OUTPROJ_FACTORS or len(geo.spatial) != 3:
+        return False
+    k = ("outproj", int(Hd), int(R), int(T), int(G), int(act_dtype), N.products(), bool(dropout))
+    ok = geo._factors_ok.get(k)
+    if ok is None:
+        ok = geo._factors_ok[k] = bool(N.lib().fz_outproj_factors_supported(
+            geo.C, k[1], *geo.spatial, geo.d, *geo.patch, *k[2:5], geo.nshift, geo._carr, k[5], k[6], int(k[7])))
+    return ok
+
+
+def core_factors(t, u0, v0, geo: Geometry, T, solver, eps):
+    t, u0, v0 = t.contiguous(), u0.contiguous(), v0.contiguous()
+    B = t.shape[0]
+    nt = t.element_size() * t.numel()
+    launch, sp, shifts = _core_launches(t, geo, N.act_dtype(t))
+    nf = 4 * (t.numel() // 8)
+    fac = []
+    with _dev_guard(t):
+        for w in range(2):
+            vfac = torch.empty((B, geo.h, *geo.spatial), device=t.device, dtype=torch.float32)
+            ufac = torch.empty((B * geo.h * geo.G, 8), device=t.device, dtype=torch.float32)
+            N.set_tile_order(w)
+            launch("fz_nmf_cf_fwd_store_factors", "nmf_cf_fwd_" + sp, nt + nf, t.data_ptr(), u0.data_ptr(), v0.data_ptr(),
+                   vfac.data_ptr(), ufac.data_ptr(), B, geo.C, *geo.spatial, shifts[w], u0.shape[1], T, N.SOLVER_ID[solver], eps)
+            fac += [vfac, ufac]
+        N.set_tile_order(0)
+    return tuple(fac)
+
+
+def factors_to_tensor(fac, geo: Geometry, like):
+    out = torch.empty_like(like)
+    B = like.shape[0]
+    s0, s1 = [(N._i * 3)(*s) for s in geo.shifts3]
+    with _dev_guard(like):
+        rc = _timed("nmf_cf_factors_to_tensor", like.element_size() * like.numel() * 5 // 4,
+                    lambda: N.lib().fz_nmf_cf_factors_to_tensor(*(f.data_ptr() for f in fac), out.data_ptr(), B, geo.C, *geo.spatial,
+                                                                s0, s1, N.act_dtype(like), N.stream_ptr(like)))
+    N.check(rc, "fz_nmf_cf_factors_to_tensor")
+    return out
 
 
 def nmf_pcf_supported(geo: Geometry, R, T, G) -> bool:
diff --git a/factorizer_amd/pointwise.py b/factorizer_amd/pointwise.py
--- a/factorizer_amd/pointwise.py
+++ b/factorizer_amd/pointwise.py
@@ -170,7 +170,10 @@
     return C == 32 and V % 4 == 0 and V <= (1 << 27) and os.environ.get("FZ_DW_FUSED", "1") != "0"
 
 
-def _gemm_dw(g, w2, q, ln=None, stats=None, gadd=None, want_bias=False, name="dgrad_wgrad", gw_out=None, gb_out=None, drop=None):
+def _gemm_dw(g, w2, q, ln=None, stats=None, gadd=None, want_bias=False, name="dgrad_wgrad", gw_out=None, gb_out=None, drop=None,
+             fac=None):
+    if fac is not None:
+        q = g
     B, C = q.shape[:2]
     V = _vox(q)
     dev = q.device
@@ -179,7 +182,8 @@
     gb = (gb_out if gb_out is not None else torch.empty(C, dtype=torch.float32, device=dev)) if want_bias else None
     wpart = torch.empty(N.lib().fz_gemm_dw_workspace_bytes(B, V) // 4, dtype=torch.float32, device=dev)
     d = N.GemmDwDesc()
-    d.g, d.q, d.w, d.y = g.data_ptr(), q.data_ptr(), w2.data_ptr(), y.data_ptr()
+    d.g, d.q, d.w, d.y = g.data_ptr(), q.data_ptr() if fac is None else None, w2.data_ptr(), y.data_ptr()
+    df = N.outproj_fac(*fac) if fac is not None else None
     d.wpart, d.gw, d.gb = wpart.data_ptr(), gw.data_ptr(), _p(gb)
     d.B, d.C, d.V, d.act_dtype = B, C, V, N.act_dtype(q)
     d.ldgw = gw.stride(0)
@@ -190,9 +194,11 @@
     if ln is not None:
         gpar = torch.empty(64, dtype=torch.float32, device=dev)
         d.ln, d.stats, d.ln_g, d.ln_b, d.gadd, d.gln = 1, stats.data_ptr(), ln[0].data_ptr(), ln[1].data_ptr(), _p(gadd), gpar.data_ptr()
-    nbytes = q.element_size() * (3 * q.numel() + (gadd.numel() if gadd is not None else 0))
+    nbytes = q.element_size() * ((3 * q.numel() if fac is None else 2 * q.numel() + q.numel() // 4) + (gadd.numel() if gadd is not None else 0))
     with torch.cuda.device(dev), _finish_scope(wpart, gw, gb, gpar):
-        rc = Fn._timed(f"{name}_{C}", nbytes, lambda: N.lib().fz_gemm_dw(ctypes.byref(d), N.stream_ptr(q)),
+        rc = Fn._timed(f"{name}_{C}", nbytes,
+                       lambda: (N.lib().fz_gemm_dw(ctypes.byref(d), N.stream_ptr(q)) if df is None
+                                else N.lib().fz_gemm_dw_fac(ctypes.byref(d), ctypes.byref(df), N.stream_ptr(q))),
                        cols=B * V, flops=4 * B * V * C * C)
         N.check(rc, "fz_gemm_dw")
     if ln is not None:
@@ -235,7 +241,7 @@
     return d
 
 
-def _mlp_chain_fwd(timed, like, ln_w, ln_b, eps, w12, b1, w22, b2, inp=None, pre=None, head=None, drop=None):
+def _mlp_chain_fwd(timed, like, ln_w, ln_b, eps, w12, b1, w22, b2, inp=None, pre=None, head=None, drop=None, fac=None):
     B, C = like.shape[:2]
     V = _vox(like)
     Hd = w12.shape[0]
@@ -246,18 +252,26 @@
     if pre is not None:
         a, wout2, bout, x = pre
         x1 = torch.empty_like(like)
-        d.pre_in, d.pre_w, d.pre_b, d.pre_res, d.pre_out = a.data_ptr(), wout2.data_ptr(), _p(bout), x.data_ptr(), x1.data_ptr()
+        d.pre_in, d.pre_w, d.pre_b, d.pre_res, d.pre_out = _p(a), wout2.data_ptr(), _p(bout), x.data_ptr(), x1.data_ptr()
     if head is not None:
         hw, hb = head
         logits = new(hw.shape[0])
         d.post_w, d.post_b, d.post_out, d.post_m = hw.data_ptr(), _p(hb), logits.data_ptr(), hw.shape[0]
     dd = _mlp_dropout(drop) if drop is not None else None
+    df = N.outproj_fac(*fac) if fac is not None else None
+    if dd is not None and df is not None:
+        raise N.NativeError("fz_mlp_chain: no dropout form of the chain on the core's factors")
     key, nbytes, flops = timed
+
+    def run():
+        if df is not None:
+            return N.lib().fz_mlp_chain_fac(ctypes.byref(d), ctypes.byref(df), N.stream_ptr(like))
+        if dd is not None:
+            return N.lib().fz_mlp_chain_drop(ctypes.byref(d), ctypes.byref(dd), N.stream_ptr(like))
+        return N.lib().fz_mlp_chain(ctypes.byref(d), N.stream_ptr(like))
+
     with torch.cuda.device(like.device):
-        rc = Fn._timed(key, nbytes,
-                       lambda: (N.lib().fz_mlp_chain(ctypes.byref(d), N.stream_ptr(like)) if dd is None
-                                else N.lib().fz_mlp_chain_drop(ctypes.byref(d), ctypes.byref(dd), N.stream_ptr(like))),
-                       cols=B * V, flops=flops)
+        rc = Fn._timed(key, nbytes, run, cols=B * V, flops=flops)
     N.check(rc, "fz_mlp_chain")
     return x1, x2, z1, st, logits
 
@@ -278,13 +292,21 @@
     return _OUTPROJ_MLP and _mlp_chain_ok(C, Hd, V) and bool(N.lib().fz_mlp_pre_supported(C, Hd, V, N.products()))
 
 
-def _outproj_mlp_fwd_chain(a, wout2, bout, x, ln_w, ln_b, eps, w12, b1, w22, b2, head=None, drop=None):
-    B, C = a.shape[:2]
-    V = _vox(a)
+def _outproj_factors_ok(x, geo, Hd, R, T, G, drop):
+    C, V = x.shape[1], _vox(x)
+    return (drop is None and isinstance(geo, Fn.Geometry) and _outproj_mlp_ok(C, Hd, V) and _dw_fused_ok(C, V)
+            and Fn.outproj_factors_supported(geo, Hd, R, T, G, N.act_dtype(x), False))
+
+
+def _outproj_mlp_fwd_chain(a, wout2, bout, x, ln_w, ln_b, eps, w12, b1, w22, b2, head=None, drop=None, fac=None):
+    B, C = x.shape[:2]
+    V = _vox(x)
     Hd = w12.shape[0]
     nlogits = B * head[0].shape[0] * V if head is not None else 0
-    timed = (f"outproj_mlp_chain_fwd_{C}", a.element_size() * (4 * a.numel() + B * Hd * V + nlogits), 4 * B * V * C * Hd + 2 * B * V * C * C)
-    x1, x2, z1, st, logits = _mlp_chain_fwd(timed, a, ln_w, ln_b, eps, w12, b1, w22, b2, pre=(a, wout2, bout, x), head=head, drop=drop)
+    na = x.numel() if fac is None else x.numel() // 4
+    timed = (f"outproj_mlp_chain_fwd_{C}", x.element_size() * (3 * x.numel() + na + B * Hd * V + nlogits), 4 * B * V * C * Hd + 2 * B * V * C * C)
+    x1, x2, z1, st, logits = _mlp_chain_fwd(timed, x, ln_w, ln_b, eps, w12, b1, w22, b2, pre=(a, wout2, bout, x), head=head, drop=drop,
+                                            fac=fac)
     if head is not None:
         return x1, x2, z1, st, logits
     return x1, x2, z1, st
@@ -1303,8 +1325,11 @@
             st1 = _ln_stats(B, V, x.device)
             _gemm([x], win2, t, B=B, Cin=C, Vin=V, M=C, K=C, Ncol=V, ln=(n1w, n1b, cfg["eps1"]), stats_out=st1,
                   eact=ACT["relu"], name="ln_linear")
-        m = None
-        if cfg["core"]:
+        m = fac = None
+        R = u0c.shape[1]
+        if cfg["core"] and _outproj_factors_ok(x, geo, Hd, R, T, G, drop):
+            a, fac = None, (Fn.core_factors(t, u0c, v0c, geo, T, solver, neps), geo)
+        elif cfg["core"]:
             a = Fn.FactCoreFn.forward(_Ctx(), t, u0c, v0c, geo, T, G, solver, neps, True)
         else:
             m = Fn._swm_fwd_raw(t, geo)
@@ -1313,9 +1338,10 @@
             del ym
         logits = None
         tail = (a, wout2, bout, x, n2w, n2b, cfg["eps2"], w12, b1, w22, b2)
-        if (_mlp_drop_ok if drop is not None else _outproj_mlp_ok)(C, Hd, V) and a.is_contiguous():
+        if (_mlp_drop_ok if drop is not None else _outproj_mlp_ok)(C, Hd, V) and (fac is not None or a.is_contiguous()):
             head = (head_w.reshape(head_w.shape[0], C), head_b) if head_w is not None and drop is None else None
-            x1, x2, z1, st2, *logits = _outproj_mlp_fwd_chain(*tail, head=head, drop=(bits, drop) if drop is not None else None)
+            x1, x2, z1, st2, *logits = _outproj_mlp_fwd_chain(*tail, head=head, drop=(bits, drop) if drop is not None else None,
+                                                              **({"fac": fac} if fac is not None else {}))
             logits = logits[0] if logits else None
         elif drop is None and _mlp_chain_ok(C, Hd, V):
             x1 = new(C)
@@ -1323,7 +1349,8 @@
             x2, z1, st2 = _mlp_fwd_chain(x1, n2w, n2b, cfg["eps2"], w12, b1, w22, b2)
         else:
             x1, x2, z1, st2 = _block_tail_fwd(*tail, drop, bits)
-        ctx.save_for_backward(x, st1, t, a, x1, st2, z1, m, n1w, n1b, win2, u0c, v0c, wout2, n2w, n2b, w12, w22, *bits)
+        ctx.save_for_backward(x, st1, t, a, x1, st2, z1, m, n1w, n1b, win2, u0c, v0c, wout2, n2w, n2b, w12, w22, *bits,
+                              *(fac[0] if fac is not None else ()))
         ctx.cfg = cfg
         ctx.shapes = (win.shape, wout.shape, w1.shape, w2.shape)
         ctx.prm = tuple(weakref.ref(t) for t in (win, wout, bout, w1, b1, w2, b2))
@@ -1340,6 +1367,7 @@
     @_bwd
     def backward(ctx, g2, _g_logits=None):
         x, st1, t, a, x1, st2, z1, m, n1w, n1b, win2, u0c, v0c, wout2, n2w, n2b, w12, w22, *bits = ctx.saved_tensors
+        bits, fac = bits[:3], (tuple(bits[3:]), ctx.cfg["geo"]) if len(bits) > 3 else None
         cfg = ctx.cfg
         drop = cfg.get("drop")
         if g2 is None:
@@ -1403,8 +1431,11 @@
                 go = Fn.dropout_apply(N.DROP_RES, m0, p0, gx1)
         dw = _dw_fused_ok(C, V)
         if dw:
-            ga, gwo, gbo, _, _ = _gemm_dw(go, wout2, a, want_bias=True, name="dgrad_wgrad", drop=go_drop)
+            ga, gwo, gbo, _, _ = _gemm_dw(go, wout2, a, want_bias=True, name="dgrad_wgrad", drop=go_drop,
+                                          **({"fac": fac} if fac is not None else {}))
         else:
+            if fac is not None:
+                a = Fn.factors_to_tensor(*fac, x)
             ga = torch.empty_like(a)
             _gemm([go], wout2, ga, B=B, Cin=C, Vin=V, M=C, K=C, Ncol=V, w_t=True, ldw=C, name="linear_dgrad")
             gwo = _GB.out_like(wout2)
diff --git a/include/factorizer_hip.h b/include/factorizer_hip.h
--- a/include/factorizer_hip.h
+++ b/include/factorizer_hip.h
@@ -83,6 +83,11 @@
 
 int fz_nmf_cf_factors_supported(int C, int D, int H, int W, int d, int pd, int ph, int pw, int R, int T, int Tgrad,
                                 int nshift, const int* shifts);
+int fz_nmf_cf_factors_to_tensor(const float* vfac0, const float* ufac0, const float* vfac1, const float* ufac1, void* out,
+                                int B, int C, int D, int H, int W, const int* shift0, const int* shift1, int act_dtype,
+                                fz_stream_t stream);
+int fz_outproj_factors_supported(int C, int Hd, int D, int H, int W, int d, int pd, int ph, int pw, int R, int T, int Tgrad,
+                                 int nshift, const int* shifts, int act_dtype, int products, int dropout);
 int fz_nmf_cf_fwd_store_factors(const void* t, const float* u0, const float* v0, float* vfac, float* ufac, int B,
                                 int C, int D, int H, int W, const int* shift, int R, int T, int solver, float eps,
                                 int act_dtype, fz_stream_t stream);
@@ -242,6 +247,16 @@
 int64_t fz_gemm_dw_workspace_bytes(int B, int64_t V);
 int fz_gemm_dw(const fz_gemm_dw_desc* desc, fz_stream_t stream);
 
+typedef struct fz_outproj_fac {
+  const float* v[2];
+  const float* u[2];
+  int dims[3];
+  int heads;
+  int shift[6];
+} fz_outproj_fac;
+int fz_mlp_chain_fac(const fz_mlp_desc* desc, const fz_outproj_fac* fac, fz_stream_t stream);
+int fz_gemm_dw_fac(const fz_gemm_dw_desc* desc, const fz_outproj_fac* fac, fz_stream_t stream);
+
 int fz_head_bwd_rows(void);
 int64_t fz_head_bwd_workspace_bytes(void);
 int fz_head_bwd(const void* gy, const void* x, const float* w, void* gx, float* part, int B, int M, int C, int64_t V,
```
